# kkahatapitiya/Coarse-Fine-Networks

Measured on AMD Instinct MI355X. Metric: clips/sec (fwd+bwd+SGD) x3d_fine X3D-M T=256x224x224, higher is better.
Workload: dtype f32; 1 GPU; x3d_fine X3D-M train step (fwd+loss+bwd+SGD), 8x3x256x224x224 clips per GPU, random-init weights; clips_per_gpu=8, frames=256, parallelism=dp1, launch=eager

## Files before the change

coarse-fine-networks_amd/cfn_hip/ops.py:

```python
import torch
from torch.autograd import Function
from torch.autograd.function import once_differentiable

import ctypes
import threading

from . import call, call_try, check, query, ACT_NONE, ACT_RELU, ACT_SWISH, ACT_SIGMOID


_scratch_epoch = [0]


class _ZeroArena(object):
    CHUNK = 1 << 20

    def __init__(self):
        self.buf, self.off, self.epoch = {}, {}, _scratch_epoch[0]

    def take(self, numel, dev):
        if self.epoch != _scratch_epoch[0]:
            self.buf, self.off, self.epoch = {}, {}, _scratch_epoch[0]
        numel_al = (numel + 1) & ~1
        key = (dev.type, dev.index)
        if key not in self.buf or self.off[key] + numel_al > self.buf[key].numel():
            self.buf[key] = torch.zeros(max(self.CHUNK, numel_al), dtype=torch.float64, device=dev)
            self.off[key] = 0
        o = self.off[key]
        self.off[key] = o + numel_al
        return self.buf[key][o:o + numel]


class _GradCast(object):

    def __init__(self):
        self._reset()
        self.last_total = 0

    def _reset(self):
        self.cur, self.live, self.scheduled, self.seen, self.task = {}, [], False, set(), None

    def begin(self):
        tid = torch._C._current_graph_task_id()
        if tid != self.task:
            if self.live:
                self.flush()
            self._reset()
            self.task = tid

    def first_use(self, w):
        if id(w) in self.seen:
            return False
        self.seen.add(id(w))
        return True

    def take(self, numel, shape, dev):
        al = (numel + 3) & ~3
        key = (dev.type, dev.index)
        ch = self.cur.get(key)
        if ch is None or ch['off'] + al > ch['f64'].numel():
            size = max(int(self.last_total * 1.05) + 1024, al, 1 << 16)
            ch = {'f64': torch.zeros(size, dtype=torch.float64, device=dev),
                  'f32': torch.empty(size, dtype=torch.float32, device=dev), 'off': 0, 'done': 0}
            self.cur[key] = ch
            self.live.append(ch)
        o = ch['off']
        ch['off'] = o + al
        if not self.scheduled:
            torch.autograd.Variable._execution_engine.queue_callback(self._end_of_backward)
            self.scheduled = True
        return ch['f64'][o:o + numel], ch['f32'][o:o + numel].view(shape)

    def flush(self):
        for ch in self.live:
            if ch['off'] > ch['done']:
                ch['f32'][ch['done']:ch['off']].copy_(ch['f64'][ch['done']:ch['off']])
                ch['done'] = ch['off']

    def _end_of_backward(self):
        self.flush()
        self.last_total = max(sum(ch['off'] for ch in self.live), 1)
        self._reset()


class _PerThread(threading.local):

    def __init__(self):
        self.arena = _ZeroArena()
        self.gradcast = _GradCast()


_tls = _PerThread()
LAZY_GRAD_CAST = True


def _f64(n, c, dev):
    return _tls.arena.take(n * c, dev).view(n, c)


def _f64pair(n, c, dev):
    t = _tls.arena.take(2 * n * c, dev).view(2, n, c)
    return t, t[0], t[1]


def reset_scratch():
    _scratch_epoch[0] += 1


def flush_grad_casts():
    _tls.gradcast.flush()


def allow_lazy_grad_cast(params, ok=True):
    for p in params:
        p._cfn_lazy_grad_ok = bool(ok)


def _lazy_ok(w):
    if not LAZY_GRAD_CAST or w is None or not w.is_leaf or w.grad is not None or torch.is_grad_enabled():
        return False
    if not getattr(w, '_cfn_lazy_grad_ok', False):
        return False
    if w._backward_hooks:
        return False
    hooks = getattr(w, '_post_accumulate_grad_hooks', None)
    if hooks:
        from .dist import _BucketHook
        if not all(isinstance(h, _BucketHook) for h in hooks.values()):
            return False
    return True


def _lazy_ok_probe(w):
    with torch.no_grad():
        return _lazy_ok(w)


def _grad_owner(w):
    if w is not None and not w.is_leaf and w._is_view():
        base = w._base
        if base is not None and base.is_leaf and base.numel() == w.numel() and w.is_contiguous() and base.is_contiguous():
            return base
    return w


def _gw_buffers(w, rows, cols, dev):
    gc = _tls.gradcast
    owner = _grad_owner(w)
    if _lazy_ok(owner):
        gc.begin()
        if gc.first_use(owner):
            g64, g32 = gc.take(rows * cols, tuple(w.shape), dev)
            return g64.view(rows, cols), (lambda: g32)
        gc.flush()
    g64 = _f64(rows, cols, dev)
    return g64, (lambda: g64.float().view(tuple(w.shape)))


def _opt(t):
    return None if t is None else t.contiguous()


def _coef(t, rows=None, cols=None):
    if t is None:
        return None
    if rows is not None and t.numel() != rows * cols:
        raise RuntimeError('per-sample coefficients of %d x %d channels expected, got a tensor of shape %s' % (rows, cols, tuple(t.shape)))
    return t.to(torch.float64).contiguous()


class ShortcutToken(object):

    def __init__(self):
        self.acc, self.acc_stride, self.main_done = None, 1, False


class TailLink(object):

    def __init__(self):
        self.y_scale = self.res_scale = None
        self.done = False


def _bf(t):
    return t is not None and t.dtype in (torch.bfloat16, torch.float16)


def subsample_hw(x, s):
    N, C, T, H, W = x.shape
    out = torch.empty(N, C, T, (H - 1) // s + 1, (W - 1) // s + 1, dtype=x.dtype, device=x.device)
    call('cfn_subsample_hw' + _sfx(x), x, out, N * C * T, H, W, s)
    return out


class _PwConv(Function):

    @staticmethod
    def forward(ctx, x, A, B, w, act, stride, want_stats, token, role, tail=None, tail_role=None):
        x = check(x).contiguous()
        N, Cin, T, H, W = x.shape
        Cout = w.shape[0]
        Ho, Wo = (H - 1) // stride + 1, (W - 1) // stride + 1
        y = torch.empty(N, Cout, T, Ho, Wo, dtype=x.dtype, device=x.device)
        s = q = None
        if want_stats:
            s, q = _f64(N, Cout, x.device), _f64(N, Cout, x.device)
        w2 = w.reshape(Cout, Cin).contiguous()
        A, B = _coef(A, N, Cin), _coef(B, N, Cin)
        xs = None
        if _bf(x):
            xs = subsample_hw(x, stride) if stride > 1 else x
            call('cfn_pwconv_fwd' + _sfx(x), xs, A, B, act, w2, y, s, q, N, Cin, Cout, T * Ho * Wo)
        else:
            call('cfn_pwconv_fwd', x, A, B, act, w2, y, s, q, N, Cin, Cout, T, H, W, stride)
        ctx.save_for_backward(x, A, B, w2, y, xs if stride > 1 else None)
        ctx.meta = (act, stride, tuple(w.shape))
        ctx.wparam = w
        ctx.token, ctx.role = token, role
        ctx.tail, ctx.tail_role = tail, tail_role
        if not want_stats:
            return y, None, None
        return y, s, q

    @staticmethod
    @once_differentiable
    def backward(ctx, gy, gs, gq):
        x, A, B, w2, y, xs = ctx.saved_tensors
        act, stride, wshape = ctx.meta
        token, role = ctx.token, ctx.role
        N, Cin, T, H, W = x.shape
        Cout = w2.shape[0]
        gy = torch.zeros_like(y) if gy is None else gy.contiguous()
        gs, gq = _opt(gs), _opt(gq)
        gsc = None
        if ctx.tail is not None and ctx.tail.done:
            gsc = ctx.tail.y_scale if ctx.tail_role == 'y' else ctx.tail.res_scale
        if _bf(x):
            return _PwConv._backward_bf16(ctx, gy, gs, gq, gsc)
        gx = gA = gB = gw = None
        g64 = fin = None
        fused = False
        if ctx.needs_input_grad[0] or (A is not None and ctx.needs_input_grad[1]):
            if token is not None and role == 'short' and stride > 1 and not token.main_done:
                Ho, Wo = y.shape[3], y.shape[4]
                da = torch.empty(N, Cin, T, Ho, Wo, dtype=torch.float32, device=x.device)
                if ctx.needs_input_grad[3]:
                    g64, fin = _gw_buffers(ctx.wparam, Cout, Cin, x.device)
                    fused = call_try('cfn_pwconv_short_bwd', gy, y, gs, gq, gsc, w2, x, A, B, act, da, g64, N, Cin, Cout, T, H, W,
                                     stride)
                if not fused:
                    call('cfn_pwconv_bwd_data_acc', gy, y, gs, gq, w2, None, None, None, ACT_NONE, da, None, None, N, Cin, Cout, T,
                         Ho, Wo, 1, None, 1, gsc)
                token.acc, token.acc_stride = da, stride
            else:
                gx = torch.zeros_like(x) if stride != 1 else torch.empty_like(x)
                ab = a64 = b64 = None
                if A is not None:
                    ab, a64, b64 = _f64pair(N, Cin, x.device)
                acc, acc_stride = None, 1
                if token is not None and role == 'main':
                    if token.acc is not None:
                        acc, acc_stride, token.acc = token.acc, token.acc_stride, None
                    else:
                        token.main_done = True
                if stride == 1 and ctx.needs_input_grad[3]:
                    g64, fin = _gw_buffers(ctx.wparam, Cout, Cin, x.device)
                    fused = call_try('cfn_pwconv_bwd_fused', gy, y, gs, gq, w2, x, A, B, act, gx, a64, b64, g64, N, Cin, Cout,
                                     T, H, W, acc, acc_stride, gsc)
                if not fused:
                    call('cfn_pwconv_bwd_data_acc', gy, y, gs, gq, w2, x, A, B, act, gx, a64, b64, N, Cin, Cout, T, H, W, stride,
                         acc, acc_stride, gsc)
                if A is not None:
                    gA, gB = ab[0], ab[1]
        if ctx.needs_input_grad[3]:
            if g64 is None:
                g64, fin = _gw_buffers(ctx.wparam, Cout, Cin, x.device)
            if not fused:
                call('cfn_pwconv_bwd_weight', gy, y, gs, gq, x, A, B, act, g64, N, Cin, Cout, T, H, W, stride, gsc)
            gw = fin()
        return gx, gA, gB, gw, None, None, None, None, None, None, None

    @staticmethod
    def _backward_bf16(ctx, gy, gs, gq, gsc):
        x, A, B, w2, y, xs = ctx.saved_tensors
        act, stride, wshape = ctx.meta
        token, role = ctx.token, ctx.role
        N, Cin, T, H, W = x.shape
        Cout = w2.shape[0]
        Ho, Wo = y.shape[3], y.shape[4]
        xin = xs if stride > 1 else x
        gx = gA = gB = gw = None
        if ctx.needs_input_grad[0] or (A is not None and ctx.needs_input_grad[1]):
            if token is not None and role == 'short' and stride > 1 and not token.main_done:
                da = torch.empty(N, Cin, T, Ho, Wo, dtype=x.dtype, device=x.device)
                call('cfn_pwconv_bwd_data' + _sfx(gy), gy, y, gs, gq, w2, None, None, None, ACT_NONE, da, None, None, N, Cin, Cout, T,
                     Ho, Wo, None, 1, gsc)
                token.acc, token.acc_stride = da, stride
            else:
                ab = a64 = b64 = None
                if A is not None:
                    ab, a64, b64 = _f64pair(N, Cin, x.device)
                acc, acc_stride = None, 1
                if token is not None and role == 'main':
                    if token.acc is not None:
                        acc, acc_stride, token.acc = token.acc, token.acc_stride, None
                    else:
                        token.main_done = True
                gxc = torch.empty_like(xin)
                call('cfn_pwconv_bwd_data' + _sfx(gy), gy, y, gs, gq, w2, xin, A, B, act, gxc, a64, b64, N, Cin, Cout, T, Ho, Wo,
                     acc, acc_stride, gsc)
                if stride > 1:
                    gx = torch.zeros_like(x)
                    gx[:, :, :, ::stride, ::stride] = gxc
                else:
                    gx = gxc
                if A is not None:
                    gA, gB = ab[0], ab[1]
        if ctx.needs_input_grad[3]:
            g64, fin = _gw_buffers(ctx.wparam, Cout, Cin, x.device)
            call('cfn_pwconv_bwd_weight' + _sfx(gy), gy, y, gs, gq, xin, A, B, act, g64, N, Cin, Cout, T * Ho * Wo, gsc)
            gw = fin()
        return gx, gA, gB, gw, None, None, None, None, None, None, None


def pwconv(x, w, A=None, B=None, act=ACT_NONE, stride=1, stats=True, token=None, role=None, tail=None, tail_role=None):
    N, Cin, T, H, W = x.shape
    Ho, Wo = (H - 1) // stride + 1, (W - 1) // stride + 1
    es = x.element_size()
    lim = (1 << 31) if es == 4 else (1 << 30)
    span = max(Cin * H * W, w.shape[0] * H * W, w.shape[0] * Ho * Wo, Cin * Ho * Wo) * es
    needs_grad = torch.is_grad_enabled() and any(t is not None and t.requires_grad for t in (x, w, A, B))
    if span * T < lim or needs_grad or T == 1:
        return _PwConv.apply(x, A, B, w, act, stride, stats, token, role, tail, tail_role)
    step = max((lim - 1) // span, 1)
    odd_plane = es == 2 and (Ho * Wo) % 2 == 1
    if odd_plane:
        if 2 * span >= lim:
            raise RuntimeError('pwconv: two frames of %d x %d x %d bf16 elements exceed the 1 GiB buffer range the frame-range '
                               'chunking has to respect (odd plane: frames travel in pairs)' % (max(Cin, w.shape[0]), H, W))
        step = max(step & ~1, 2)
    y = torch.empty(N, w.shape[0], T, Ho, Wo, dtype=x.dtype, device=x.device)
    s = q = None
    t0 = 0
    while t0 < T:
        t1 = min(t0 + step, T)
        if odd_plane and (t1 - t0) % 2 and t1 - t0 > 1:
            t1 -= 1
        pad = odd_plane and (t1 - t0) % 2 == 1
        xc = x[:, :, t0:t1].contiguous()
        if pad:
            xc = torch.cat([xc, torch.zeros_like(xc)], 2)
        yc, sc, qc = _PwConv.apply(xc, A, B, w, act, stride, False if pad else stats, None, None)
        if pad:
            yc = yc[:, :, :1]
            if stats:
                sc, qc = yc.double().sum((2, 3, 4)), (yc.double() ** 2).sum((2, 3, 4))
        y[:, :, t0:t1] = yc
        if stats:
            s, q = (sc, qc) if s is None else (s + sc, q + qc)
        t0 = t1
    return y, s, q


def _sfx(t):
    return '_bf16' if t.dtype == torch.bfloat16 else ('_f16' if t.dtype == torch.float16 else '')


class _DwConv3d(Function):

    @staticmethod
    def forward(ctx, x, A, B, w, act, stride, want_stats):
        x = check(x).contiguous()
        N, C, T, H, W = x.shape
        Ho, Wo = (H + 2 - 3) // stride + 1, (W + 2 - 3) // stride + 1
        y = torch.empty(N, C, T, Ho, Wo, dtype=x.dtype, device=x.device)
        s = q = None
        if want_stats:
            s, q = _f64(N, C, x.device), _f64(N, C, x.device)
        w2 = w.reshape(C, 27).contiguous()
        A, B = _coef(A, N, C), _coef(B, N, C)
        call('cfn_dwconv3d_fwd' + _sfx(x), x, A, B, act, w2, y, s, q, N, C, T, H, W, stride)
        ctx.save_for_backward(x, A, B, w2, y)
        ctx.meta = (act, stride, tuple(w.shape))
        ctx.wparam = w
        if not want_stats:
            return y, None, None
        return y, s, q

    @staticmethod
    @once_differentiable
    def backward(ctx, gy, gs, gq):
        x, A, B, w2, y = ctx.saved_tensors
        act, stride, wshape = ctx.meta
        N, C, T, H, W = x.shape
        gy = torch.zeros_like(y) if gy is None else gy.contiguous()
        gs, gq = _opt(gs), _opt(gq)
        gx = gA = gB = gw = None
        want_x = ctx.needs_input_grad[0] or (A is not None and ctx.needs_input_grad[1])
        want_w = ctx.needs_input_grad[3]
        ab = a64 = b64 = g64 = fin = None
        if want_x:
            gx = torch.empty_like(x)
            if A is not None:
                ab, a64, b64 = _f64pair(N, C, x.device)
        if want_w:
            g64, fin = _gw_buffers(ctx.wparam, C, 27, x.device)
        sfx = _sfx(x)
        fused = want_x and want_w and stride == 1 and call_try('cfn_dwconv3d_bwd_fused' + sfx, gy, y, gs, gq, w2, x, A, B, act,
                                                             gx, a64, b64, g64, N, C, T, H, W)
        if not fused and want_x and want_w and stride == 2:
            fused = call_try('cfn_dwconv3d_bwd_fused_s2' + sfx, gy, y, gs, gq, w2, x, A, B, act, gx, a64, b64, g64, N, C, T, H, W)
        if not fused:
            if want_x:
                call('cfn_dwconv3d_bwd_data' + sfx, gy, y, gs, gq, w2, x, A, B, act, gx, a64, b64, N, C, T, H, W, stride)
            if want_w:
                call('cfn_dwconv3d_bwd_weight' + sfx, gy, y, gs, gq, x, A, B, act, g64, N, C, T, H, W, stride)
        if want_x and A is not None:
            gA, gB = ab[0], ab[1]
        if want_w:
            gw = fin()
        return gx, gA, gB, gw, None, None, None


def dwconv3d(x, w, A=None, B=None, act=ACT_NONE, stride=1, stats=True):
    return _DwConv3d.apply(x, A, B, w, act, stride, stats)


class _DwConvT5(Function):

    @staticmethod
    def forward(ctx, x, w, want_stats, out_dtype=None):
        x = check(x, torch.float32).contiguous()
        N, C, T, H, W = x.shape
        y = torch.empty_like(x, dtype=out_dtype or x.dtype)
        s = q = None
        if want_stats:
            s, q = _f64(N, C, x.device), _f64(N, C, x.device)
        w2 = w.reshape(C, 5).contiguous()
        call('cfn_dwconv_t5_fwd' + _sfx(y), x, w2, y, s, q, N, C, T, H * W)
        ctx.save_for_backward(x, w2, y)
        ctx.wshape = tuple(w.shape)
        ctx.wparam = w
        if not want_stats:
            return y, None, None
        return y, s, q

    @staticmethod
    @once_differentiable
    def backward(ctx, gy, gs, gq):
        x, w2, y = ctx.saved_tensors
        N, C, T, H, W = x.shape
        gy = torch.zeros_like(y) if gy is None else gy.contiguous()
        gs, gq = _opt(gs), _opt(gq)
        gx = gw = None
        want_x, want_w = ctx.needs_input_grad[0], ctx.needs_input_grad[1]
        if want_x:
            gx = torch.empty_like(x)
        if want_w:
            g64, fin = _gw_buffers(ctx.wparam, C, 5, x.device)
        fused = want_x and want_w and call_try('cfn_dwconv_t5_bwd_fused' + _sfx(y), gy, y, gs, gq, w2, x, gx, g64, N, C, T, H * W)
        if not fused:
            if want_x:
                call('cfn_dwconv_t5_bwd_data' + _sfx(y), gy, y, gs, gq, w2, gx, N, C, T, H * W)
            if want_w:
                call('cfn_dwconv_t5_bwd_weight' + _sfx(y), gy, y, gs, gq, x, g64, N, C, T, H * W)
        if want_w:
            gw = fin()
        return gx, gw, None, None


def dwconv_t5(x, w, stats=True, out_dtype=None):
    return _DwConvT5.apply(x, w, stats, out_dtype)


class _StemConv(Function):

    @staticmethod
    def forward(ctx, x, w):
        x = check(x).contiguous()
        N, Ci, T, H, W = x.shape
        Co = w.shape[0]
        Ho, Wo = (H + 2 - 3) // 2 + 1, (W + 2 - 3) // 2 + 1
        y = torch.empty(N, Co, T, Ho, Wo, dtype=torch.float32, device=x.device)
        w2 = w.reshape(Co, Ci * 9).contiguous()
        call('cfn_stem_conv_fwd', x, w2, y, N, Ci, Co, T, H, W)
        ctx.save_for_backward(x)
        ctx.wshape = tuple(w.shape)
        ctx.wparam = w
        return y

    @staticmethod
    @once_differentiable
    def backward(ctx, gy):
        (x,) = ctx.saved_tensors
        N, Ci, T, H, W = x.shape
        Co = ctx.wshape[0]
        gw = None
        if ctx.needs_input_grad[1]:
            g64, fin = _gw_buffers(ctx.wparam, Co, Ci * 9, x.device)
            call('cfn_stem_conv_bwd_weight', gy.contiguous(), x, g64, N, Ci, Co, T, H, W)
            gw = fin()
        return None, gw


def stem_conv(x, w):
    return _StemConv.apply(x, w)


from .u8clips import clip_lut


def _u8_args(frames, lengths, lut):
    if frames.dtype != torch.uint8 or frames.dim() != 5 or frames.shape[4] != 3:
        raise RuntimeError('uint8 frames of shape (N, T, H, W, 3) expected, got %s %s' % (frames.dtype, tuple(frames.shape)))
    if lut.dtype != torch.float32 or lut.numel() != 3 * 256:
        raise RuntimeError('a (3, 256) fp32 table expected (ops.clip_lut), got %s %s' % (lut.dtype, tuple(lut.shape)))
    if lengths is not None:
        if lengths.numel() != frames.shape[0]:
            raise RuntimeError('one length per clip expected: %d clips, lengths %s' % (frames.shape[0], tuple(lengths.shape)))
        lengths = lengths.to(torch.int32).contiguous()
    return frames.contiguous(), lengths, lut.contiguous()


def clip_u8_to_f32(frames, lut, lengths=None):
    frames, lengths, lut = _u8_args(frames, lengths, lut)
    N, T, H, W, _ = frames.shape
    x = torch.empty(N, 3, T, H, W, dtype=torch.float32, device=frames.device)
    call('cfn_clip_u8_to_f32', frames, lut, lengths, x, N, T, H, W)
    return x


class _StemConvU8(Function):

    @staticmethod
    def forward(ctx, frames, lengths, lut, w):
        frames, lengths, lut = _u8_args(frames, lengths, lut)
        N, T, H, W, Ci = frames.shape
        Co = w.shape[0]
        Ho, Wo = (H + 2 - 3) // 2 + 1, (W + 2 - 3) // 2 + 1
        y = torch.empty(N, Co, T, Ho, Wo, dtype=torch.float32, device=frames.device)
        w2 = w.reshape(Co, Ci * 9).contiguous()
        if not call_try('cfn_stem_conv_u8_fwd', frames, lut, lengths, w2, y, N, Ci, Co, T, H, W):
            call('cfn_stem_conv_fwd', clip_u8_to_f32(frames, lut, lengths), w2, y, N, Ci, Co, T, H, W)
        ctx.save_for_backward(frames, lengths, lut)
        ctx.wshape = tuple(w.shape)
        ctx.wparam = w
        return y

    @staticmethod
    @once_differentiable
    def backward(ctx, gy):
        frames, lengths, lut = ctx.saved_tensors
        N, T, H, W, Ci = frames.shape
        Co = ctx.wshape[0]
        gw = None
        if ctx.needs_input_grad[3]:
            g64, fin = _gw_buffers(ctx.wparam, Co, Ci * 9, frames.device)
            gy = gy.contiguous()
            if not call_try('cfn_stem_conv_u8_bwd_weight', gy, frames, lut, lengths, g64, N, Ci, Co, T, H, W):
                call('cfn_stem_conv_bwd_weight', gy, clip_u8_to_f32(frames, lut, lengths), g64, N, Ci, Co, T, H, W)
            gw = fin()
        return None, None, None, gw


def stem_conv_u8(frames, lengths, lut, w):
    return _StemConvU8.apply(frames, lengths, lut, w)


from . import u8aug

_AUG_TABLES = {}
_AUG_TABLES_MAX = 256


def aug_tables(box, size, device):
    cs = tuple(int(v) for v in box.detach().reshape(-1, 4)[:, 2].cpu().tolist())
    device = torch.device(device)
    key = (cs, int(size), device.type, device.index)
    hit = _AUG_TABLES.get(key)
    if hit is None:
        if any(c <= 0 or c > 4 * int(size) for c in cs):
            raise RuntimeError('crop_resize_flip_u8: crop extents %s into %d: 1 <= c <= 4 * size expected (the kernel takes tables of up '
                               'to %d taps; there is no CPU fallback)' % (sorted(set(cs)), size, u8aug.MAX_TAPS))
        bounds, coef = u8aug.batch_tables(cs, size)
        hit = (bounds.to(device), coef.to(device))
        if len(_AUG_TABLES) >= _AUG_TABLES_MAX:
            _AUG_TABLES.clear()
        _AUG_TABLES[key] = hit
    return hit


def crop_resize_flip_u8(frames, lengths, box, size, out=None, tables=None):
    if frames.dtype != torch.uint8 or frames.dim() != 5 or frames.shape[4] != 3:
        raise RuntimeError('uint8 frames of shape (N, T, Hs, Ws, 3) expected, got %s %s' % (frames.dtype, tuple(frames.shape)))
    N, T, Hs, Ws, _ = frames.shape
    S = int(size)
    if box.numel() != 4 * N:
        raise RuntimeError('one box (x1, y1, c, flip) per clip expected: %d clips, box %s' % (N, tuple(box.shape)))
    if lengths is not None:
        if lengths.numel() != N:
            raise RuntimeError('one length per clip expected: %d clips, lengths %s' % (N, tuple(lengths.shape)))
        lengths = lengths.to(torch.int32).contiguous()
    bounds, coef = tables if tables is not None else aug_tables(box, S, frames.device)
    if tuple(bounds.shape) != (N, S, 2) or coef.dim() != 3 or tuple(coef.shape[:2]) != (N, S):
        raise RuntimeError('tables of %d clips into %d expected, got bounds %s coef %s' % (N, S, tuple(bounds.shape), tuple(coef.shape)))
    box = box.reshape(N, 4).to(device=frames.device, dtype=torch.int32).contiguous()
    if out is None:
        out = torch.empty(N, T, S, S, 3, dtype=torch.uint8, device=frames.device)
    elif out.dtype != torch.uint8 or tuple(out.shape) != (N, T, S, S, 3) or not out.is_contiguous():
        raise RuntimeError('out: a contiguous uint8 tensor of shape %s expected, got %s %s' % ((N, T, S, S, 3), out.dtype, tuple(out.shape)))
    if not call_try('cfn_crop_resize_flip_u8', frames.contiguous(), lengths, box, bounds.contiguous(), coef.contiguous(), out, N, T, Hs, Ws,
                    S, int(coef.shape[2])):
        raise RuntimeError('crop_resize_flip_u8: %d taps into size %d is beyond what the kernel was built for (c <= 4 * size, size <= 312 '
                           'at 9 taps); there is no CPU fallback' % (int(coef.shape[2]), S))
    return out


AP_SORT_TILE = 8192
AP_FLAG_NONBINARY, AP_FLAG_OVERFLOW = 1, 2


def _ap_stores(scores, targets, count, what):
    for name, x in (('scores', scores), ('targets', targets), ('count', count)):
        if not torch.is_tensor(x) or not x.is_cuda:
            raise RuntimeError('%s: %s must be a device tensor; there is no CPU path' % (what, name))
    if scores.dtype != torch.float32 or scores.dim() != 2 or targets.dtype != torch.uint8 or tuple(targets.shape) != tuple(scores.shape):
        raise RuntimeError('%s: class-major stores expected, scores (K, cap) fp32 and targets (K, cap) uint8; got %s %s, %s %s'
                           % (what, scores.dtype, tuple(scores.shape), targets.dtype, tuple(targets.shape)))
    if count.dtype != torch.int32 or count.numel() != 1:
        raise RuntimeError('%s: count must be one int32 on the device, got %s %s' % (what, count.dtype, tuple(count.shape)))
    if scores.shape[0] < 1 or scores.shape[1] < 1:
        raise RuntimeError('%s: empty stores %s' % (what, tuple(scores.shape)))
    return int(scores.shape[0]), int(scores.shape[1])


def ap_append(probs, labels, valid, scores, targets, count, flags):
    K, cap = _ap_stores(scores, targets, count, 'ap_append')
    for name, x in (('probs', probs), ('labels', labels), ('flags', flags)):
        if not torch.is_tensor(x) or not x.is_cuda:
            raise RuntimeError('ap_append: %s must be a device tensor; there is no CPU path' % name)
    if probs.dim() != 3 or probs.shape[1] != K or tuple(labels.shape) != tuple(probs.shape):
        raise RuntimeError('ap_append: probs and labels (B, %d, TL) expected, got %s and %s' % (K, tuple(probs.shape), tuple(labels.shape)))
    if flags.dtype != torch.int32 or flags.numel() != 1:
        raise RuntimeError('ap_append: flags must be one int32 on the device')
    B, _, TL = probs.shape
    if valid is not None:
        if valid.numel() != B:
            raise RuntimeError('ap_append: one valid length per video expected: %d videos, valid %s' % (B, tuple(valid.shape)))
        valid = valid.to(torch.int32).contiguous()
    call('cfn_ap_append', probs.float().contiguous(), labels.float().contiguous(), valid, scores, targets, count, flags, B, K, TL, cap)


def ap_sort(scores, targets, count, out=None):
    K, cap = _ap_stores(scores, targets, count, 'ap_sort')
    if out is None:
        out = (torch.empty_like(scores), torch.empty_like(targets), torch.empty(K, cap, dtype=torch.int32, device=scores.device),
               torch.empty_like(targets))
    ss, st, tk, tt = out
    for x, ref, dt in ((ss, scores, torch.float32), (st, targets, torch.uint8), (tk, scores, torch.int32), (tt, targets, torch.uint8)):
        if tuple(x.shape) != tuple(ref.shape) or x.dtype != dt or x.device != ref.device:
            raise RuntimeError('ap_sort: out buffers of shape %s (fp32, uint8, int32, uint8) on %s expected' % (tuple(ref.shape), ref.device))
    call('cfn_ap_sort', scores, targets, count, ss, st, tk, tt, K, cap)
    return ss, st


def ap_reduce(sorted_targets, count):
    if not sorted_targets.is_cuda or not count.is_cuda:
        raise RuntimeError('ap_reduce: device tensors only; there is no CPU path')
    if sorted_targets.dtype != torch.uint8 or sorted_targets.dim() != 2 or count.dtype != torch.int32 or count.numel() != 1:
        raise RuntimeError('ap_reduce: sorted targets (K, cap) uint8 and one int32 count expected')
    K, cap = sorted_targets.shape
    ap = torch.empty(K, dtype=torch.float32, device=sorted_targets.device)
    call('cfn_ap_reduce', sorted_targets, count, ap, K, cap)
    return ap


def average_precision(scores, targets, count, out=None):
    _, st = ap_sort(scores, targets, count, out=out)
    return ap_reduce(st, count)


class _BnFold(Function):

    @staticmethod
    def forward(ctx, s, q, gamma, beta, w1, b1, w2, b2, bufs, cfg):
        training, N, C, S, count, eps, momentum, pool_count = cfg
        run_mean, run_var, nbt = bufs
        dev = run_mean.device
        Wd = w1.shape[0] if w1 is not None else 0
        Se = S if training else 1
        A = torch.empty(N, C, dtype=torch.float64, device=dev)
        B = torch.empty_like(A)
        mean = torch.empty(Se, C, dtype=torch.float64, device=dev)
        rstd = torch.empty_like(mean)
        A0 = B0 = gate = hbuf = pooled = None
        w1c = w2c = None
        if Wd:
            A0, B0, gate, pooled = (torch.empty(N, C, dtype=torch.float32, device=dev) for _ in range(4))
            hbuf = torch.empty(N, Wd, dtype=torch.float32, device=dev)
            w1c, w2c = w1.reshape(Wd, C).contiguous(), w2.reshape(C, Wd).contiguous()
        s, q = _opt(s), _opt(q)
        call('cfn_bn_fold_fwd', s, q, gamma, beta, run_mean, run_var, nbt if training else None, int(training), N, C, S,
             float(count), float(eps), float(momentum), w1c, b1, w2c, b2, Wd, float(pool_count), A, B, mean, rstd,
             A0, B0, gate, hbuf, pooled)
        ctx.save_for_backward(s, gamma, mean, rstd, A0, B0, gate, hbuf, pooled, w1c, w2c)
        ctx.cfg = (training, N, C, S, Wd, count, pool_count, None if w1 is None else tuple(w1.shape),
                   None if w2 is None else tuple(w2.shape))
        return A, B

    @staticmethod
    @once_differentiable
    def backward(ctx, gA, gB):
        s, gamma, mean, rstd, A0, B0, gate, hbuf, pooled, w1c, w2c = ctx.saved_tensors
        training, N, C, S, Wd, count, pool_count, w1s, w2s = ctx.cfg
        dev = mean.device
        gA = torch.zeros(N, C, dtype=torch.float64, device=dev) if gA is None else gA.contiguous()
        gB = torch.zeros(N, C, dtype=torch.float64, device=dev) if gB is None else gB.contiguous()
        gs = gq = None
        if training:
            gs = torch.empty(N, C, dtype=torch.float64, device=dev)
            gq = torch.empty_like(gs)
        elif Wd:
            gs = torch.empty(N, C, dtype=torch.float64, device=dev)
        gg = gbt = None
        if gamma is not None:
            gg, gbt = torch.empty(C, device=dev), torch.empty(C, device=dev)
        gw1 = gb1 = gw2 = gb2 = tA = tB = None
        if Wd:
            gw1, gb1 = torch.empty(Wd, C, device=dev), torch.empty(Wd, device=dev)
            gw2, gb2 = torch.empty(C, Wd, device=dev), torch.empty(C, device=dev)
            tA, tB = (torch.empty(N, C, dtype=torch.float64, device=dev) for _ in range(2))
        call('cfn_bn_fold_bwd', gA, gB, s, gamma, mean, rstd, A0, B0, gate, hbuf, pooled, w1c, w2c, int(training), N, C, S,
             Wd, float(count), float(pool_count), gs, gq, gg, gbt, gw1, gb1, gw2, gb2, tA, tB)
        if Wd:
            gw1, gw2 = gw1.view(w1s), gw2.view(w2s)
        return gs, gq, gg, gbt, gw1, gb1, gw2, gb2, None, None


def bn_fold(s, q, gamma, beta, bufs, training, N, C, S, count, eps, momentum, se=None, pool_count=1.0):
    w1, b1, w2, b2 = se if se is not None else (None, None, None, None)
    return _BnFold.apply(s, q, gamma, beta, w1, b1, w2, b2, bufs, (training, N, C, S, count, eps, momentum, pool_count))


class _BnAddRelu(Function):

    @staticmethod
    def forward(ctx, y, A, B, res, Ar, Br, split, link):
        y, res = check(y).contiguous(), check(res).contiguous()
        N, C = y.shape[:2]
        vol = y[0, 0].numel()
        if tuple(res.shape) != tuple(y.shape):
            raise RuntimeError('bn_add_relu: residual %s does not match y %s' % (tuple(res.shape), tuple(y.shape)))
        out = torch.empty_like(y)
        A, B, Ar, Br = _coef(A, N, C), _coef(B, N, C), _coef(Ar, N, C), _coef(Br, N, C)
        mask = None
        sfx = _sfx(y)
        if link is not None:
            words = query('cfn_bn_add_relu_mask_words' + sfx, N * C, vol)
            if words > 0:
                mask = torch.empty(words, dtype=torch.int32, device=y.device)
        call('cfn_bn_add_relu_fwd' + sfx, y, A, B, res, Ar, Br, out, mask, N * C, vol)
        ctx.link, ctx.has_mask = link, mask is not None
        ctx.save_for_backward(y, A, res, Ar, mask if mask is not None else out)
        if not split:
            return out
        alias = torch.empty(0, dtype=out.dtype, device=out.device).set_(out.untyped_storage(), out.storage_offset(),
                                                                         out.shape, out.stride())
        return out, alias

    @staticmethod
    @once_differentiable
    def backward(ctx, gout, gout2=None):
        y, A, res, Ar, out = ctx.saved_tensors
        N, C = y.shape[:2]
        vol = y[0, 0].numel()
        if gout is None:
            gout, gout2 = gout2, None
        if gout is None:
            gout = torch.zeros_like(y)
        gout2 = None if gout2 is None else gout2.contiguous()
        t3 = _tls.arena.take(3 * N * C, y.device).view(3, N, C)
        gA, gB = t3[0], t3[1]
        gAr = t3[2] if Ar is not None else None
        gBr = gB if Ar is not None else None
        link = ctx.link
        if link is not None:
            g = torch.empty_like(y)
            mask = out if ctx.has_mask else None
            call('cfn_bn_add_relu_bwd_g' + _sfx(y), gout.contiguous(), gout2, None if ctx.has_mask else out, mask, y,
                 res if Ar is not None else None, g, gA, gB, gAr, N * C, vol)
            link.y_scale, link.res_scale, link.done = A.detach(), (None if Ar is None else Ar.detach()), True
            g2 = torch.empty(0, dtype=g.dtype, device=g.device).set_(g.untyped_storage(), g.storage_offset(), g.shape, g.stride())
            return g, gA, gB, g2, gAr, gBr, None, None
        if _bf(y):
            g = torch.empty_like(y)
            call('cfn_bn_add_relu_bwd_g' + _sfx(y), gout.contiguous(), gout2, out, None, y, res if Ar is not None else None, g, gA, gB,
                 gAr, N * C, vol)
            shp = (N, C) + (1,) * (y.dim() - 2)
            gres = g if Ar is None else (g.float() * Ar.float().view(shp)).to(y.dtype)
            return (g.float() * A.float().view(shp)).to(y.dtype), gA, gB, gres, gAr, gBr, None, None
        gy, gres = torch.empty_like(y), torch.empty_like(res)
        call('cfn_bn_add_relu_bwd', gout.contiguous(), gout2, out, y, A, res, Ar, gy, gres, gA, gB, gAr, N * C, vol)
        return gy, gA, gB, gres, gAr, gBr, None, None


def bn_add_relu(y, A, B, res, Ar=None, Br=None, split=False, link=None):
    return _BnAddRelu.apply(y, A, B, res, Ar, Br, split, link)


class _AffineAct(Function):
    @staticmethod
    def forward(ctx, x, A, B, act):
        x = check(x).contiguous()
        N, C = x.shape[:2]
        out = torch.empty_like(x)
        A, B = _coef(A, N, C), _coef(B, N, C)
        call('cfn_affine_act_fwd', x, A, B, act, out, N * C, x[0, 0].numel())
        ctx.save_for_backward(x, A, B)
        ctx.act = act
        return out

    @staticmethod
    @once_differentiable
    def backward(ctx, gout):
        x, A, B = ctx.saved_tensors
        N, C = x.shape[:2]
        gx = torch.empty_like(x)
        a64, b64 = _f64(N, C, x.device), _f64(N, C, x.device)
        call('cfn_affine_act_bwd', gout.contiguous(), x, A, B, ctx.act, gx, a64, b64, N * C, x[0, 0].numel())
        return gx, a64, b64, None


def affine_act(x, A, B, act=ACT_NONE):
    return _AffineAct.apply(x, A, B, act)


class _ChannelStats(Function):

    @staticmethod
    def forward(ctx, x):
        x = check(x).contiguous()
        N, C = x.shape[:2]
        s, q = _f64(N, C, x.device), _f64(N, C, x.device)
        call('cfn_channel_stats', x, s, q, N * C, x[0, 0].numel())
        ctx.save_for_backward(x)
        return s, q

    @staticmethod
    @once_differentiable
    def backward(ctx, gs, gq):
        (x,) = ctx.saved_tensors
        N, C = x.shape[:2]
        gx = torch.zeros_like(x)
        shp = (N, C) + (1,) * (x.dim() - 2)
        if gs is not None:
            gx = gx + gs.float().view(shp)
        if gq is not None:
            gx = gx + 2.0 * gq.float().view(shp) * x
        return gx


def channel_stats(x):
    return _ChannelStats.apply(x)


class _PoolHW(Function):

    @staticmethod
    def forward(ctx, x, A, B, act, OH, OW):
        x = check(x).contiguous()
        N, C, T, H, W = x.shape
        out = torch.empty(N, C, T, OH, OW, dtype=torch.float32, device=x.device)
        A, B = _coef(A, N, C), _coef(B, N, C)
        call('cfn_pool_hw_fwd' + _sfx(x), x, A, B, act, out, N * C, T, H, W, OH, OW)
        ctx.save_for_backward(x, A, B)
        ctx.meta = (act, OH, OW)
        return out

    @staticmethod
    @once_differentiable
    def backward(ctx, gout):
        x, A, B = ctx.saved_tensors
        act, OH, OW = ctx.meta
        N, C, T, H, W = x.shape
        gx = torch.empty_like(x)
        a64 = b64 = None
        if A is not None:
            a64, b64 = _f64(N, C, x.device), _f64(N, C, x.device)
        call('cfn_pool_hw_bwd' + _sfx(x), gout.contiguous(), x, A, B, act, gx, a64, b64, N * C, T, H, W, OH, OW)
        if A is None:
            return gx, None, None, None, None, None
        return gx, a64, b64, None, None, None


def pool_hw(x, OH, OW, A=None, B=None, act=ACT_NONE):
    return _PoolHW.apply(x, A, B, act, OH, OW)


class _Film(Function):

    @staticmethod
    def forward(ctx, x, m, c, f):
        x, m, c = check(x).contiguous(), check(m).contiguous(), check(c).contiguous()
        N, C, T, H, W = x.shape
        want = (N, C, T, H // f if f > 0 else -1, W // f if f > 0 else -1)
        if f <= 0 or H % f or W % f or tuple(m.shape) != want or tuple(c.shape) != want:
            raise RuntimeError('film: coefficients %s / %s do not tile x %s with %d x %d blocks (expected %s)'
                               % (tuple(m.shape), tuple(c.shape), tuple(x.shape), f, f, want))
        out = torch.empty_like(x)
        call('cfn_film_fwd', x, m, c, out, N * C, T, H, W, f)
        ctx.save_for_backward(x, m)
        ctx.f = f
        return out

    @staticmethod
    @once_differentiable
    def backward(ctx, g):
        x, m = ctx.saved_tensors
        N, C, T, H, W = x.shape
        gx, gm, gc = torch.empty_like(x), torch.empty_like(m), torch.empty_like(m)
        call('cfn_film_bwd', g.contiguous(), x, m, gx, gm, gc, N * C, T, H, W, ctx.f)
        return gx, gm, gc, None


def film(x, m, c, f):
    return _Film.apply(x, m, c, f)


class _TimeSample(Function):

    @staticmethod
    def forward(ctx, x, cdf):
        x, cdf = check(x).contiguous(), check(cdf).contiguous()
        B, C, Tin = x.shape[:3]
        K = cdf.shape[1]
        P = x[0, 0, 0].numel()
        out = torch.empty((B, C, K) + tuple(x.shape[3:]), dtype=torch.float32, device=x.device)
        call('cfn_time_sample_fwd', x, cdf, out, B, C, Tin, K, P)
        ctx.save_for_backward(x, cdf)
        return out

    @staticmethod
    @once_differentiable
    def backward(ctx, g):
        x, cdf = ctx.saved_tensors
        B, C, Tin = x.shape[:3]
        K = cdf.shape[1]
        P = x[0, 0, 0].numel()
        gx = torch.empty_like(x) if ctx.needs_input_grad[0] else None
        g64 = torch.zeros(B, K, dtype=torch.float64, device=x.device) if ctx.needs_input_grad[1] else None
        call('cfn_time_sample_bwd', g.contiguous(), x, cdf, gx, g64, B, C, Tin, K, P)
        return gx, (g64.float() if g64 is not None else None)


def time_sample(x, cdf):
    return _TimeSample.apply(x, cdf)


class _TimePool(Function):

    @staticmethod
    def forward(ctx, x, mode, R):
        x = check(x, torch.float32).contiguous()
        B, C, T = x.shape[:3]
        P = x[0, 0, 0].numel()
        out = torch.empty((B, C, T // R) + tuple(x.shape[3:]), dtype=torch.float32, device=x.device)
        call('cfn_time_pool_fwd', x, out, mode, B * C, T, R, P)
        ctx.save_for_backward(x)
        ctx.meta = (mode, R)
        return out

    @staticmethod
    @once_differentiable
    def backward(ctx, g):
        (x,) = ctx.saved_tensors
        mode, R = ctx.meta
        B, C, T = x.shape[:3]
        gx = torch.empty_like(x)
        call('cfn_time_pool_bwd', g.contiguous(), x, gx, mode, B * C, T, R, x[0, 0, 0].numel())
        return gx, None, None


def time_pool(x, mode, R=4):
    return _TimePool.apply(x, {'avg': 0, 'max': 1}[mode], R)


def grid_time_index(cdf, Tin):
    cdf = check(cdf).contiguous()
    i0 = torch.empty(cdf.shape, dtype=torch.int32, device=cdf.device)
    w1 = torch.empty(cdf.shape, dtype=torch.float32, device=cdf.device)
    call('cfn_grid_time_index', cdf, cdf.numel(), Tin, i0, w1)
    return i0, w1


class _Interp1d(Function):
    @staticmethod
    def forward(ctx, x, y, xnew):
        x, y, xnew = check(x).contiguous(), check(y).contiguous(), check(xnew).contiguous()
        B = max(x.shape[0], y.shape[0], xnew.shape[0])
        N, Pq = x.shape[1], xnew.shape[1]
        rows = (int(x.shape[0] > 1), int(y.shape[0] > 1), int(xnew.shape[0] > 1))
        ynew = torch.empty(B, Pq, dtype=torch.float32, device=x.device)
        ind = torch.empty(B, Pq, dtype=torch.int64, device=x.device)
        call('cfn_interp1d_fwd', x, y, xnew, ynew, ind, B, N, Pq, *rows)
        ctx.save_for_backward(x, y, xnew, ind)
        ctx.rows = rows
        ctx.mark_non_differentiable(ind)
        return ynew, ind

    @staticmethod
    @once_differentiable
    def backward(ctx, g, _gind):
        x, y, xnew, ind = ctx.saved_tensors
        B, Pq = ind.shape
        N = x.shape[1]
        gx = torch.zeros_like(x) if ctx.needs_input_grad[0] else None
        gy = torch.zeros_like(y) if ctx.needs_input_grad[1] else None
        gq = torch.zeros_like(xnew) if ctx.needs_input_grad[2] else None
        call('cfn_interp1d_bwd', g.contiguous(), x, y, xnew, ind, gx, gy, gq, B, N, Pq, *ctx.rows)
        return gx, gy, gq


def interp1d(x, y, xnew):
    return _Interp1d.apply(x, y, xnew)


class _TimeResize(Function):

    @staticmethod
    def forward(ctx, x, L, align_corners):
        x = check(x).contiguous()
        BC = x.shape[0] * x.shape[1]
        Kin = x.shape[2]
        P = x[0, 0, 0].numel()
        out = torch.empty(tuple(x.shape[:2]) + (L,) + tuple(x.shape[3:]), dtype=torch.float32, device=x.device)
        call('cfn_time_resize_fwd', x, out, BC, Kin, L, P, int(bool(align_corners)))
        ctx.meta = (tuple(x.shape), L, int(bool(align_corners)))
        return out

    @staticmethod
    @once_differentiable
    def backward(ctx, g):
        shape, L, ac = ctx.meta
        gx = torch.empty(shape, dtype=torch.float32, device=g.device)
        P = 1
        for d in shape[3:]:
            P *= d
        call('cfn_time_resize_bwd', g.contiguous(), gx, shape[0] * shape[1], shape[2], L, P, ac)
        return gx, None, None


def time_resize(x, L, align_corners=True):
    return _TimeResize.apply(x, L, align_corners)


def _detloss_args(logits, labels, masks, crops):
    for name, v in (('logits', logits), ('labels', labels), ('masks', masks)):
        if not v.is_cuda or v.dtype != torch.float32:
            raise RuntimeError('detection_loss: %s must be a device fp32 tensor, got %s on %s (there is no CPU path)' % (name, v.dtype, v.device))
        if v.device != logits.device:
            raise RuntimeError('detection_loss: %s lives on %s, the logits on %s' % (name, v.device, logits.device))
    crops = int(crops)
    if logits.dim() != 3 or labels.dim() != 3 or masks.dim() != 2 or crops < 1:
        raise RuntimeError('detection_loss: logits (B*crops, C, T), labels (B, C, TL), masks (B, TL), crops >= 1')
    B, C, TL = labels.shape
    if logits.shape[0] != B * crops or logits.shape[1] != C or tuple(masks.shape) != (B, TL) or 0 in logits.shape or 0 in labels.shape:
        raise RuntimeError('detection_loss: logits %s, labels %s, masks %s do not belong together at %d crop(s)'
                           % (tuple(logits.shape), tuple(labels.shape), tuple(masks.shape), crops))
    return logits.contiguous(), labels.contiguous(), masks.contiguous(), B, C, logits.shape[2], TL


def detection_loss_fwd(logits, labels, masks, align_corners=True, crops=1, norm=None, world=1.0, want_probs=True):
    logits, labels, masks, B, C, T, TL = _detloss_args(logits, labels, masks, crops)
    dev = logits.device
    if norm is not None:
        if not norm.is_cuda or norm.device != dev or norm.numel() != 1:
            raise RuntimeError('detection_loss: norm must be a one-element tensor on the device of the logits')
        norm = norm.detach().to(torch.float32).reshape(1)
    cls = torch.empty((), dtype=torch.float32, device=dev)
    loc = torch.empty((), dtype=torch.float32, device=dev)
    probs = torch.empty(B, C, TL, dtype=torch.float32, device=dev) if want_probs else None
    jstar = torch.empty(B * C, dtype=torch.int32, device=dev)
    ymax = torch.empty(B * C, dtype=torch.float32, device=dev)
    rows = torch.empty(2 * B * C, dtype=torch.float64, device=dev)
    norm_used = torch.empty(1, dtype=torch.float64, device=dev)
    call('cfn_detloss_fwd', logits, labels, masks, norm, float(world), probs, cls, loc, jstar, ymax, rows, norm_used, B, C, T, TL, int(crops),
         int(bool(align_corners)))
    return cls, loc, probs, jstar, ymax, norm_used


def detection_loss_bwd(g_cls, g_loc, logits, labels, masks, jstar, ymax, norm_used, align_corners=True, crops=1, world=1.0):
    logits, labels, masks, B, C, T, TL = _detloss_args(logits, labels, masks, crops)
    if jstar.numel() != B * C or ymax.numel() != B * C or norm_used.numel() != 1:
        raise RuntimeError('detection_loss_bwd: jstar / ymax / norm_used are not the ones the forward returned for these shapes')
    g_cls, g_loc = (g.detach().to(torch.float32).reshape(1) for g in (g_cls, g_loc))
    gx = torch.empty_like(logits)
    call('cfn_detloss_bwd', g_cls, g_loc, logits, labels, masks, jstar.contiguous(), ymax.contiguous(), norm_used, float(world), gx, B, C, T, TL,
         int(crops), int(bool(align_corners)))
    return gx


class _DetectionLoss(Function):

    @staticmethod
    def forward(ctx, logits, labels, masks, align_corners, crops, norm, world, want_probs):
        cls, loc, probs, jstar, ymax, norm_used = detection_loss_fwd(logits, labels, masks, align_corners, crops, norm, world, want_probs)
        ctx.save_for_backward(logits, labels, masks, jstar, ymax, norm_used)
        ctx.meta = (bool(align_corners), int(crops), float(world))
        if probs is not None:
            ctx.mark_non_differentiable(probs)
# ... 305 lines not shown
```

coarse-fine-networks_amd/csrc/pw_common.h:

```cpp
#pragma once
#include "cfn_common.h"

typedef float __attribute__((ext_vector_type(16))) f16v;
typedef float __attribute__((ext_vector_type(4))) f4v;

enum { PW_FWD = 0, PW_DGRAD = 1 };
#define PW_KC 32
#define PW_RED_PITCH 33

struct PwArgs {
    const float* src;
    const float* src2;
    const double* pa;
    const double* pb;
    const double* gs;
    const double* gq;
    const double* gsc;
    const float* w;
    float* dst;
    const float* ex;
    const double* ea;
    const double* eb;
    const float* acc; int acc_s, acc_Ho, acc_Wo;
    double* s1;
    double* s2;
    int N, M, K, Q, Pin, Hi, Wi, Ho, Wo, stride, act;
    int Cin;
    int mtiles, nstrips, tpb, kres, Kpad;
    int stem, Cimg, kT, kH, kW, sT, sH, sW, pT, pH, pW, Ti, To;
};

#define PW_UNIT 8
#define PW_KRES_MAX 512

__device__ __forceinline__ float pw_bload(__amdgpu_buffer_rsrc_t r, int voff, int soff) {
    return __builtin_bit_cast(float, __builtin_amdgcn_raw_buffer_load_b32(r, voff, soff, 0));
}


int pwd_try_launch(PwArgs& a, int mode, bool stats, hipStream_t st);

int pws_try_launch(PwArgs& a, int mode, bool stats, hipStream_t st);
int pwk_try_launch(PwArgs& a, int mode, bool stats, hipStream_t st);
int pwt_try_launch(PwArgs& a, int mode, bool stats, hipStream_t st);
int pws_terms_now();
int pws_wgrad_try_launch(const float* gy, const float* y, const double* gs, const double* gq, const double* gsc, const float* x,
                         const double* pa, const double* pb, int act, double* gw, int N, int M, int K, int Q, hipStream_t st);

int pwss_wgrad_try_bf16(const uint16_t* gy, const uint16_t* y, const double* gs, const double* gq, const double* gsc, const uint16_t* x,
                        const double* pa, const double* pb, int act, double* gw, int N, int M, int K, int Q, hipStream_t st);

int pwd_wgrad_try_launch(const float* gy, const float* y, const double* gs, const double* gq, const double* gsc, const float* x,
                         const double* pa, const double* pb, int act, double* gw, int N, int M, int K, int Q, hipStream_t st);
int pwd_wgrad_try_strided(const float* gy, const float* y, const double* gs, const double* gq, const double* gsc, const float* x,
                          const double* pa, const double* pb, int act, double* gw, int N, int M, int K, int T, int Hi, int Wi,
                          int stride, hipStream_t st);
int pwd_wgrad_try_dense(const float* gy, const float* y, const double* gs, const double* gq, const float* x, const double* pa,
                        const double* pb, int act, double* gw, int N, int M, int Cimg, int T, int Hi, int Wi, const int* g,
                        hipStream_t st);

int stem_fwd_try_launch(const float* x, const float* w, float* y, int N, int Cimg, int Cout, int T, int Hi, int Wi, hipStream_t st);
int stem_wgrad_try_launch(const float* gy, const float* x, double* gw, int N, int Cimg, int Cout, int T, int Hi, int Wi, hipStream_t st, bool probe);

int sal_fwd_try_launch(const float* x, const double* A, const double* B, int act, const float* w, float* y, double* sum,
                       double* sumsq, int N, int Cin, int Cout, int T, int Hi, int Wi, const int* g, hipStream_t st);
int pwfs_try_launch(const float* gy, const float* y, const double* gsum, const double* gsumsq, const float* w, const float* x, const double* A,
                    const double* B, int act, float* gx, double* gA, double* gB, double* gw, int N, int Cin, int Cout, int T, int Hi, int Wi,
                    const float* acc, int acc_stride, const double* gscale, hipStream_t st);
int salb_fwd_try_launch(const float* x, const double* A, const double* B, int act, const float* w, float* y, double* sum,
                        double* sumsq, int N, int Cin, int Cout, int T, int Hi, int Wi, const int* g, hipStream_t st);
int sal_wgrad_try_launch(const float* gy, const float* y, const double* gs, const double* gq, const float* x, const double* A,
                         const double* B, int act, double* gw, int N, int Cin, int Cout, int T, int Hi, int Wi, const int* g,
                         hipStream_t st);
```

coarse-fine-networks_amd/csrc/pwfused.hip:

```cpp
#include "cfn_common.h"
#include <stdlib.h>

#include "pw_common.h"

typedef float __attribute__((ext_vector_type(4))) pf4;

#define PF_PT 64
#define PF_PITCH 65

struct PfArgs {
    const float* gy; const float* y; const double* gs; const double* gq; const double* gsc;
    const float* w;
    const float* x; const double* pa; const double* pb;
    float* gx; double* gA; double* gB; double* gw;
    const float* acc; int acc_s, acc_Ho, acc_Wo, Hi, Wi, T;
    int N, M, K, Q, nstrips, stages;
};

template <int MTW, int NTW, int ACT>
__global__ __launch_bounds__(256, ACT < 0 ? 3 : 2) void pw_bwd_fused_kernel(const PfArgs a) {
    extern __shared__ __attribute__((aligned(16))) float smem[];
    constexpr bool EPI = ACT >= 0;
    constexpr int ACTV = EPI ? ACT : CFN_ACT_NONE;
    constexpr int BM = 32 * MTW, BN = 32 * NTW;
    constexpr int NG = BM / 16, NX = BN / 16;
    constexpr int NT16 = BN / 16, KS = BM / 4;
    const int tid = threadIdx.x, wave = tid >> 6, lane = tid & 63, half = lane >> 5, col = lane & 31;
    const int m16 = lane & 15, kq = lane >> 4;
    unsigned L = cfn_xcd_remap(blockIdx.x, gridDim.x);
    const int strip = L % a.nstrips;
    const int n = L / a.nstrips;
    const int M = a.M, K = a.K, Q = a.Q;

    constexpr int IMG = (BM + BN) * PF_PITCH;
    float* img0 = smem;
    float* sCg = smem + 2 * IMG;
    float* sCz = sCg + 2 * BM;
    float* sCx = sCz + BM;
    float* sSt = sCx + 2 * BN;
    for (int m = tid; m < BM; m += 256) {
        const bool ok = m < M;
        sCg[2 * m] = (ok && a.gs) ? (float)a.gs[(long)n * M + m] : 0.0f;
        sCg[2 * m + 1] = (ok && a.gq && a.y) ? 2.0f * (float)a.gq[(long)n * M + m] : 0.0f;
        sCz[m] = (ok && a.gsc) ? (float)a.gsc[(long)n * M + m] : 1.0f;
    }
    for (int k = tid; k < BN; k += 256) {
        const bool ok = EPI && k < K;
        sCx[2 * k] = ok ? (float)a.pa[(long)n * K + k] : 1.0f;
        sCx[2 * k + 1] = ok ? (float)a.pb[(long)n * K + k] : 0.0f;
    }
    float wq[NT16][KS];
#pragma unroll
    for (int t = 0; t < NT16; ++t)
#pragma unroll
        for (int s = 0; s < KS; ++s) {
            const int ci = t * 16 + m16, co = 4 * s + kq;
            wq[t][s] = (ci < K && co < M) ? a.w[(long)co * K + ci] : 0.0f;
        }
    float ca[NTW], cb[NTW];
#pragma unroll
    for (int j = 0; j < NTW; ++j) {
        const int k = j * 32 + col;
        const bool ok = EPI && k < K;
        ca[j] = ok ? (float)a.pa[(long)n * K + k] : 1.0f;
        cb[j] = ok ? (float)a.pb[(long)n * K + k] : 0.0f;
    }
    f16v acc[MTW][NTW];
#pragma unroll
    for (int i = 0; i < MTW; ++i)
#pragma unroll
        for (int j = 0; j < NTW; ++j)
#pragma unroll
            for (int r = 0; r < 16; ++r) acc[i][j][r] = 0.0f;
    float sa[NT16][4], sb[NT16][4];
#pragma unroll
    for (int t = 0; t < NT16; ++t)
#pragma unroll
        for (int r = 0; r < 4; ++r) { sa[t][r] = 0.0f; sb[t][r] = 0.0f; }
    __syncthreads();

    const int lrow = tid >> 4, c4 = (tid & 15) * 4;
    constexpr int OOB = 0x7ffffff0;
    __amdgpu_buffer_rsrc_t rg = cfn_rsrc(const_cast<float*>(a.gy + (long)n * M * Q), (unsigned)((long)M * Q * 4));
    __amdgpu_buffer_rsrc_t ry = cfn_rsrc(const_cast<float*>((a.y ? a.y : a.gy) + (long)n * M * Q), a.y ? (unsigned)((long)M * Q * 4) : 0u);
    __amdgpu_buffer_rsrc_t rx = cfn_rsrc(const_cast<float*>(a.x + (long)n * K * Q), (unsigned)((long)K * Q * 4));
    __amdgpu_buffer_rsrc_t rd = cfn_rsrc(a.gx + (long)n * K * Q, (unsigned)((long)K * Q * 4));
    pf4 pg[NG], py[NG], px[NX];
    int vog[NG], vox[NX];
#pragma unroll
    for (int it = 0; it < NG; ++it) vog[it] = (it * 16 + lrow) < M ? ((it * 16 + lrow) * Q + c4) * 4 : OOB;
#pragma unroll
    for (int it = 0; it < NX; ++it) vox[it] = (it * 16 + lrow) < K ? ((it * 16 + lrow) * Q + c4) * 4 : OOB;
    auto prefetch = [&](int q0) {
        const bool inq = q0 + c4 < Q;
#pragma unroll
        for (int it = 0; it < NG; ++it) {
            const int vo = inq ? vog[it] : OOB;
            pg[it] = __builtin_bit_cast(pf4, __builtin_amdgcn_raw_buffer_load_b128(rg, vo, q0 * 4, 0));
            py[it] = __builtin_bit_cast(pf4, __builtin_amdgcn_raw_buffer_load_b128(ry, vo, q0 * 4, 0));
        }
#pragma unroll
        for (int it = 0; it < NX; ++it)
            px[it] = __builtin_bit_cast(pf4, __builtin_amdgcn_raw_buffer_load_b128(rx, inq ? vox[it] : OOB, q0 * 4, 0));
    };
    auto stage = [&](int q0, float* sG, float* sX) {
        const bool inq = q0 + c4 < Q;
#pragma unroll
        for (int it = 0; it < NG; ++it) {
            const int row = it * 16 + lrow;
            const float cs = cfn_settle(sCg[2 * row]), cq = cfn_settle(sCg[2 * row + 1]), cz = cfn_settle(sCz[row]);
            const bool ok = inq && (row < M);
            float* d = sG + row * PF_PITCH + c4;
            d[0] = ok ? fmaf(py[it].x, cq, fmaf(pg[it].x, cz, cs)) : 0.0f;
            d[1] = ok ? fmaf(py[it].y, cq, fmaf(pg[it].y, cz, cs)) : 0.0f;
            d[2] = ok ? fmaf(py[it].z, cq, fmaf(pg[it].z, cz, cs)) : 0.0f;
            d[3] = ok ? fmaf(py[it].w, cq, fmaf(pg[it].w, cz, cs)) : 0.0f;
        }
#pragma unroll
        for (int it = 0; it < NX; ++it) {
            const int row = it * 16 + lrow;
            float* d = sX + row * PF_PITCH + c4;
            d[0] = px[it].x; d[1] = px[it].y; d[2] = px[it].z; d[3] = px[it].w;
        }
    };

    const int qbeg = strip * a.stages * PF_PT;
    const int nst = min(a.stages, (Q - qbeg + PF_PT - 1) / PF_PT);
    if (nst > 0) {
        prefetch(qbeg);
        stage(qbeg, img0, img0 + BM * PF_PITCH);
        if (nst > 1) prefetch(qbeg + PF_PT);
    }
    __syncthreads();
    const int pbase = wave * (PF_PT / 4);
    const int hw = a.Hi * a.Wi;
    const int acc_pitch4 = a.T * a.acc_Ho * a.acc_Wo * 4;
    __amdgpu_buffer_rsrc_t racc = cfn_rsrc(const_cast<float*>(a.acc ? a.acc + (long)n * K * (acc_pitch4 / 4) : a.gy), a.acc ? (unsigned)((long)K * acc_pitch4) : 0u);
    for (int st = 0; st < nst; ++st) {
        const int q0 = qbeg + st * PF_PT;
        float* cur = img0 + (st & 1) * IMG;
        float* nxt = img0 + ((st + 1) & 1) * IMG;
        if (st + 1 < nst) {
            stage(q0 + PF_PT, nxt, nxt + BM * PF_PITCH);
            if (st + 2 < nst) prefetch(q0 + 2 * PF_PT);
        }
        const float* sG = cur;
        const float* sX = cur + BM * PF_PITCH;
#pragma unroll
        for (int s = 0; s < PF_PT / 8; ++s) {
            const int p = pbase + 2 * s + half;
            float av[MTW], bv[NTW];
#pragma unroll
            for (int i = 0; i < MTW; ++i) av[i] = sG[(i * 32 + col) * PF_PITCH + p];
#pragma unroll
            for (int j = 0; j < NTW; ++j) {
                const float xr = sX[(j * 32 + col) * PF_PITCH + p];
                bv[j] = EPI ? cfn_act<ACTV>(fmaf(xr, ca[j], cb[j])) : xr;
            }
#pragma unroll
            for (int i = 0; i < MTW; ++i)
#pragma unroll
                for (int j = 0; j < NTW; ++j) acc[i][j] = __builtin_amdgcn_mfma_f32_32x32x2f32(av[i], bv[j], acc[i][j], 0, 0, 0);
        }
        pf4 da[NT16];
#pragma unroll
        for (int t = 0; t < NT16; ++t) da[t] = (pf4){0.f, 0.f, 0.f, 0.f};
#pragma unroll
        for (int s = 0; s < KS; ++s) {
            const float b = sG[(4 * s + kq) * PF_PITCH + pbase + m16];
#pragma unroll
            for (int t = 0; t < NT16; ++t) da[t] = __builtin_amdgcn_mfma_f32_16x16x4f32(wq[t][s], b, da[t], 0, 0, 0);
        }
        const int q = q0 + pbase + m16;
        const bool qv = q < Q;
        int aoff = OOB;
        if (a.acc && qv) {
            const int tq = q / hw, rq = q - tq * hw;
            const int hq = rq / a.Wi, wq_ = rq - hq * a.Wi;
            if (hq % a.acc_s == 0 && wq_ % a.acc_s == 0) aoff = (((tq * a.acc_Ho + hq / a.acc_s) * a.acc_Wo + wq_ / a.acc_s)) * 4;
        }
        float av4[NT16][4];
#pragma unroll
        for (int t = 0; t < NT16; ++t)
#pragma unroll
            for (int r = 0; r < 4; ++r) av4[t][r] = 0.0f;
        if (a.acc) {
            const unsigned arow = (unsigned)aoff + (unsigned)(4 * kq) * (unsigned)acc_pitch4;
#pragma unroll
            for (int t = 0; t < NT16; ++t)
#pragma unroll
                for (int r = 0; r < 4; ++r)
                    av4[t][r] = __builtin_bit_cast(float, __builtin_amdgcn_raw_buffer_load_b32(
                        racc, (int)(aoff == OOB ? (unsigned)OOB : arow + (unsigned)r * (unsigned)acc_pitch4), t * 16 * acc_pitch4, 0));
        }
#pragma unroll
        for (int t = 0; t < NT16; ++t) {
#pragma unroll
            for (int r = 0; r < 4; ++r) {
                const int ci = t * 16 + 4 * kq + r;
                const bool ok = qv && ci < K;
                float v = da[t][r] + av4[t][r];
                if (EPI) {
                    const float xr = sX[ci * PF_PITCH + pbase + m16];
                    const float pa = sCx[2 * ci], pb = sCx[2 * ci + 1];
                    const float dz = ok ? v * cfn_act_grad<ACTV>(fmaf(xr, pa, pb)) : 0.0f;
                    sa[t][r] = fmaf(dz, xr, sa[t][r]);
                    sb[t][r] += dz;
                    v = dz * pa;
                }
                __builtin_amdgcn_raw_buffer_store_b32(__builtin_bit_cast(unsigned, v), rd, ok ? (ci * Q + pbase + m16) * 4 : OOB, q0 * 4, 0);
            }
        }
        __syncthreads();
    }

    if (EPI) {
#pragma unroll
        for (int t = 0; t < NT16; ++t)
#pragma unroll
            for (int r = 0; r < 4; ++r) {
                float u = sa[t][r], v = sb[t][r];
#pragma unroll
                for (int o = 1; o < 16; o <<= 1) { u += __shfl_xor(u, o, 64); v += __shfl_xor(v, o, 64); }
                if (m16 == 0) {
                    const int ci = t * 16 + 4 * kq + r;
                    sSt[(wave * BN + ci) * 2] = u;
                    sSt[(wave * BN + ci) * 2 + 1] = v;
                }
            }
    }
    constexpr int CWP = BN + 1;
    float* cw = smem + wave * (BM * CWP);
#pragma unroll
    for (int i = 0; i < MTW; ++i)
#pragma unroll
        for (int j = 0; j < NTW; ++j)
#pragma unroll
            for (int r = 0; r < 16; ++r) {
                const int ml = i * 32 + (r & 3) + 8 * (r >> 2) + 4 * half;
                cw[ml * CWP + j * 32 + col] = acc[i][j][r];
            }
    __syncthreads();
    for (int e = tid; e < BM * BN; e += 256) {
        const int ml = e / BN, kl = e - ml * BN;
        const int o = ml * CWP + kl;
        const float v = (smem[o] + smem[BM * CWP + o]) + (smem[2 * BM * CWP + o] + smem[3 * BM * CWP + o]);
        if (ml < M && kl < K) cfn_add64(&a.gw[(long)ml * K + kl], (double)v);
    }
    if (EPI && tid < K) {
        const float u = (sSt[2 * tid] + sSt[(BN + tid) * 2]) + (sSt[(2 * BN + tid) * 2] + sSt[(3 * BN + tid) * 2]);
        const float v = (sSt[2 * tid + 1] + sSt[(BN + tid) * 2 + 1]) + (sSt[(2 * BN + tid) * 2 + 1] + sSt[(3 * BN + tid) * 2 + 1]);
        cfn_add64(&a.gA[(long)n * K + tid], (double)u);
        cfn_add64(&a.gB[(long)n * K + tid], (double)v);
    }
}

template <int MTW, int NTW>
static int pf_launch(const PfArgs& a, int act, bool epi, unsigned blocks, hipStream_t st) {
    constexpr int BM = 32 * MTW, BN = 32 * NTW;
    size_t lds = ((size_t)2 * (BM + BN) * PF_PITCH + 3 * BM + 10 * BN) * sizeof(float);
    const size_t lds_cw = (size_t)4 * BM * (BN + 1) * sizeof(float);
    if (lds_cw > lds) lds = lds_cw;
#define CFN_PF_GO(ACTV)                                                                                         \
    do {                                                                                                        \
        auto k = pw_bwd_fused_kernel<MTW, NTW, ACTV>;                                                           \
        if (lds > 48 * 1024) (void)hipFuncSetAttribute((const void*)k, hipFuncAttributeMaxDynamicSharedMemorySize, (int)lds); \
        hipLaunchKernelGGL(k, dim3(blocks), dim3(256), lds, st, a);                                             \
    } while (0)
    if (!epi) CFN_PF_GO(-1);
    else if (act == CFN_ACT_RELU) CFN_PF_GO(CFN_ACT_RELU);
    else if (act == CFN_ACT_SWISH) CFN_PF_GO(CFN_ACT_SWISH);
    else CFN_PF_GO(CFN_ACT_NONE);
#undef CFN_PF_GO
    return cfn_check_launch("pwconv_bwd_fused");
}

extern "C" int cfn_pwconv_bwd_fused(const float* gy, const float* y, const double* gsum, const double* gsumsq, const float* w,
                                    const float* x, const double* A, const double* B, int act, float* gx, double* gA, double* gB,
                                    double* gw, int N, int Cin, int Cout, int T, int Hi, int Wi, const float* acc, int acc_stride,
                                    const double* gscale, void* stream) {
    CFN_REQUIRE(gy && w && x && gx && gw, "cfn_pwconv_bwd_fused: null tensor");
    CFN_REQUIRE((A == nullptr) == (B == nullptr), "cfn_pwconv_bwd_fused: A/B mismatch");
    CFN_REQUIRE(A == nullptr || (gA && gB), "cfn_pwconv_bwd_fused: prologue needs gA, gB");
    CFN_REQUIRE(gsumsq == nullptr || y != nullptr, "cfn_pwconv_bwd_fused: gsumsq needs y");
    CFN_REQUIRE(acc == nullptr || acc_stride >= 1, "cfn_pwconv_bwd_fused: bad acc_stride");
    {
        const int rs = pwfs_try_launch(gy, y, gsum, gsumsq, w, x, A, B, act, gx, gA, gB, gw, N, Cin, Cout, T, Hi, Wi, acc, acc_stride, gscale, (hipStream_t)stream);
        if (rs != -1) return rs;
    }
    const long Ql = (long)T * Hi * Wi;
    if (Cin > 64 || Cout > 64 || (Cin > 32 && Cout > 32) || Ql % 4 != 0 || Ql >= (1L << 30)) return -1;
    if ((long)Cout * Ql * 4 >= 0x7ffffff0L || (long)Cin * Ql * 4 >= 0x7ffffff0L) return -1;
    if (A && act != CFN_ACT_NONE && act != CFN_ACT_RELU && act != CFN_ACT_SWISH) return -1;
    if ((((uintptr_t)gy | (uintptr_t)x | (uintptr_t)(y ? y : gy)) & 15) != 0) return -1;
    PfArgs a = {};
    a.gy = gy; a.y = gsumsq ? y : nullptr; a.gs = gsum; a.gq = gsumsq; a.gsc = gscale; a.w = w; a.x = x; a.pa = A; a.pb = B;
    a.gx = gx; a.gA = gA; a.gB = gB; a.gw = gw;
    a.acc = acc; a.acc_s = acc ? acc_stride : 1; a.Hi = Hi; a.Wi = Wi; a.T = T;
    a.acc_Ho = (Hi - 1) / a.acc_s + 1; a.acc_Wo = (Wi - 1) / a.acc_s + 1;
    a.N = N; a.M = Cout; a.K = Cin; a.Q = (int)Ql;
    const long nst = cfn_cdiv(Ql, PF_PT);
    const bool epi = A != nullptr;
    long want = (epi ? 1024 : 1536) / N;
    if (want < 1) want = 1;
    long stages = cfn_cdiv(nst, want);
    if (stages < 4) stages = 4;
    a.stages = (int)stages;
    a.nstrips = (int)cfn_cdiv(nst, stages);
    const unsigned blocks = (unsigned)((long)N * a.nstrips);
    hipStream_t st = (hipStream_t)stream;
    CfnProfScope prof(CFN_K_PWCONV_BWD, st, 4.0 * N * ((double)Cout * Ql * (a.y ? 2 : 1) + (double)Cin * Ql * 2));
    if (Cout > 32) return pf_launch<2, 1>(a, act, epi, blocks, st);
    if (Cin > 32) return pf_launch<1, 2>(a, act, epi, blocks, st);
    return pf_launch<1, 1>(a, act, epi, blocks, st);
}
```

coarse-fine-networks_amd/csrc/pwfuseds.hip:

```cpp
#include "cfn_common.h"
#include <stdlib.h>
#include <map>
#include <mutex>

#include "pw_common.h"

typedef float __attribute__((ext_vector_type(4))) pf4;
typedef __bf16 pfs_bf8 __attribute__((ext_vector_type(8)));
typedef __bf16 pfs_bf2 __attribute__((ext_vector_type(2)));
typedef float pfs_f2 __attribute__((ext_vector_type(2)));
typedef unsigned pfs_u4 __attribute__((ext_vector_type(4)));

#define PFS_PT 64
#define PFS_PITCH 65

__device__ __forceinline__ float pfs_lo(unsigned u) { return __builtin_bit_cast(float, u << 16); }
__device__ __forceinline__ float pfs_hi(unsigned u) { return __builtin_bit_cast(float, u & 0xffff0000u); }
__device__ __forceinline__ unsigned pfs_pack(float lo, float hi) {
    const pfs_bf2 b = __builtin_convertvector((pfs_f2){lo, hi}, pfs_bf2);
    return __builtin_bit_cast(unsigned, b);
}
__device__ __forceinline__ void pfs_split3(float v0, float v1, unsigned (&p)[3]) {
    p[0] = pfs_pack(v0, v1);
    v0 -= pfs_lo(p[0]); v1 -= pfs_hi(p[0]);
    p[1] = pfs_pack(v0, v1);
    v0 -= pfs_lo(p[1]); v1 -= pfs_hi(p[1]);
    p[2] = pfs_pack(v0, v1);
}
#define PFS_TERMS(F) F(2, 0) F(0, 2) F(1, 1) F(1, 0) F(0, 1) F(0, 0)

struct PfsArgs {
    const float* gy; const float* y; const double* gs; const double* gq; const double* gsc;
    const float* w;
    const float* x; const double* pa; const double* pb;
    float* gx; double* gA; double* gB; double* gw;
    const float* acc; int acc_s, acc_Ho, acc_Wo, Hi, Wi, T;
    int N, M, K, Q, nstrips, stages;
    int dbg;
};

template <int MTW, int NTW, int ACT>
__global__ __launch_bounds__(512, 1) void pw_bwd_fused_split_kernel(const PfsArgs a) {
    extern __shared__ __attribute__((aligned(16))) float smem[];
    constexpr bool EPI = ACT >= 0;
    constexpr int ACTV = EPI ? ACT : CFN_ACT_NONE;
    constexpr int BM = 32 * MTW, BN = 32 * NTW;
    constexpr int NG = BM / 16, NX = BN / 16;
    constexpr int NT16 = BN / 16, KS = BM / 32;
    constexpr bool ROWSPLIT = MTW >= NTW;
    constexpr int MI = ROWSPLIT ? MTW / 2 : MTW, NJ = ROWSPLIT ? NTW : NTW / 2;
    constexpr int BMP = BM + 8;
    const int tid = threadIdx.x, wave = cfn_uni((int)(tid >> 6)), lane = tid & 63, half = lane >> 5, col = lane & 31;
    const int m16 = lane & 15, kq = lane >> 4;
    unsigned L = cfn_xcd_remap(blockIdx.x, gridDim.x);
    const int strip = L % a.nstrips;
    const int n = L / a.nstrips;
    const int M = a.M, K = a.K, Q = a.Q;

    constexpr int IMG = (BM + BN) * PFS_PITCH;
    float* img0 = smem;
    float* sCx = smem + 2 * IMG + 3 * BM;
    float* sSt = sCx + 2 * BN;
    unsigned* sW = reinterpret_cast<unsigned*>(sSt + 8 * BN);
    for (int k = tid; k < BN; k += 512) {
        const bool ok = EPI && k < K;
        sCx[2 * k] = ok ? (float)a.pa[(long)n * K + k] : 1.0f;
        sCx[2 * k + 1] = ok ? (float)a.pb[(long)n * K + k] : 0.0f;
    }
    for (int e = tid; e < BN * (BM / 2); e += 512) {
        const int ci = e / (BM / 2), mp = e - ci * (BM / 2), co = 2 * mp;
        const float w0 = (ci < K && co < M) ? a.w[(long)co * K + ci] : 0.0f;
        const float w1 = (ci < K && co + 1 < M) ? a.w[(long)(co + 1) * K + ci] : 0.0f;
        unsigned p[3];
        pfs_split3(w0, w1, p);
#pragma unroll
        for (int s = 0; s < 3; ++s) sW[(s * BN + ci) * (BMP / 2) + mp] = p[s];
    }
    __syncthreads();

    const int lrow = 4 * ((tid & 255) >> 6) + ((lane >> 3) & 3), c4 = ((lane & 7) + 8 * (lane >> 5)) * 4;
    constexpr int OOB = 0x7ffffff0;
    __amdgpu_buffer_rsrc_t rg = cfn_rsrc(const_cast<float*>(a.gy + (long)n * M * Q), (unsigned)((long)M * Q * 4));
    __amdgpu_buffer_rsrc_t ry = cfn_rsrc(const_cast<float*>((a.y ? a.y : a.gy) + (long)n * M * Q), a.y ? (unsigned)((long)M * Q * 4) : 0u);
    __amdgpu_buffer_rsrc_t rx = cfn_rsrc(const_cast<float*>(a.x + (long)n * K * Q), (unsigned)((long)K * Q * 4));
    __amdgpu_buffer_rsrc_t rd = cfn_rsrc(a.gx + (long)n * K * Q, (unsigned)((long)K * Q * 4));
    pf4 pg[NG], py[NG], px[NX];
    int vog[NG], vox[NX];
    float rcs[NG], rcq[NG], rcz[NG];
#pragma unroll
    for (int it = 0; it < NG; ++it) {
        const int row = it * 16 + lrow;
        const bool ok = row < M;
        rcs[it] = (ok && a.gs) ? (float)a.gs[(long)n * M + row] : 0.0f;
        rcq[it] = (ok && a.gq && a.y) ? 2.0f * (float)a.gq[(long)n * M + row] : 0.0f;
        rcz[it] = (ok && a.gsc) ? (float)a.gsc[(long)n * M + row] : 1.0f;
    }
#pragma unroll
    for (int it = 0; it < NG; ++it) vog[it] = (it * 16 + lrow) < M ? ((it * 16 + lrow) * Q + c4) * 4 : OOB;
#pragma unroll
    for (int it = 0; it < NX; ++it) vox[it] = (it * 16 + lrow) < K ? ((it * 16 + lrow) * Q + c4) * 4 : OOB;
    auto prefetch = [&](int q0) {
        const bool inq = q0 + c4 < Q;
#pragma unroll
        for (int it = 0; it < NG; ++it) {
            const int vo = inq ? vog[it] : OOB;
            pg[it] = __builtin_bit_cast(pf4, __builtin_amdgcn_raw_buffer_load_b128(rg, vo, q0 * 4, 0));
            py[it] = __builtin_bit_cast(pf4, __builtin_amdgcn_raw_buffer_load_b128(ry, vo, q0 * 4, 0));
        }
#pragma unroll
        for (int it = 0; it < NX; ++it)
            px[it] = __builtin_bit_cast(pf4, __builtin_amdgcn_raw_buffer_load_b128(rx, inq ? vox[it] : OOB, q0 * 4, 0));
    };
    auto stage = [&](int q0, float* sG, float* sX) {
        const bool inq = q0 + c4 < Q;
#pragma unroll
        for (int it = 0; it < NG; ++it) {
            const int row = it * 16 + lrow;
            const float cs = rcs[it], cq = rcq[it], cz = rcz[it];
            const bool ok = inq && (row < M);
            float* d = sG + row * PFS_PITCH + c4;
            d[0] = ok ? fmaf(py[it].x, cq, fmaf(pg[it].x, cz, cs)) : 0.0f;
            d[1] = ok ? fmaf(py[it].y, cq, fmaf(pg[it].y, cz, cs)) : 0.0f;
            d[2] = ok ? fmaf(py[it].z, cq, fmaf(pg[it].z, cz, cs)) : 0.0f;
            d[3] = ok ? fmaf(py[it].w, cq, fmaf(pg[it].w, cz, cs)) : 0.0f;
        }
#pragma unroll
        for (int it = 0; it < NX; ++it) {
            const int row = it * 16 + lrow;
            float* d = sX + row * PFS_PITCH + c4;
            d[0] = px[it].x; d[1] = px[it].y; d[2] = px[it].z; d[3] = px[it].w;
        }
    };

    const int qbeg = strip * a.stages * PFS_PT;
    const int nst = min(a.stages, (Q - qbeg + PFS_PT - 1) / PFS_PT);
    if (nst > 0 && wave < 4) {
        prefetch(qbeg);
        stage(qbeg, img0, img0 + BM * PFS_PITCH);
        if (nst > 1) prefetch(qbeg + PFS_PT);
    }
    __syncthreads();
    const int pbase = (wave & 3) * (PFS_PT / 4);
    constexpr int CWP = 33, CWT = 32 * CWP;

    if (wave < 4) {
        const int th = wave & 1, ph = wave >> 1;
        const int i0 = ROWSPLIT ? th * MI : 0, j0 = ROWSPLIT ? 0 : th * NJ;
        float ca[NJ], cb[NJ];
#pragma unroll
        for (int j = 0; j < NJ; ++j) {
            const int k = (j0 + j) * 32 + col;
            const bool ok = EPI && k < K;
            ca[j] = ok ? (float)a.pa[(long)n * K + k] : 1.0f;
            cb[j] = ok ? (float)a.pb[(long)n * K + k] : 0.0f;
        }
        f16v acc[MI][NJ];
#pragma unroll
        for (int i = 0; i < MI; ++i)
#pragma unroll
            for (int j = 0; j < NJ; ++j)
#pragma unroll
                for (int r = 0; r < 16; ++r) acc[i][j][r] = 0.0f;
        for (int st = 0; st < nst; ++st) {
            const int q0 = qbeg + st * PFS_PT;
            float* cur = img0 + (st & 1) * IMG;
            float* nxt = img0 + ((st + 1) & 1) * IMG;
            if (st + 1 < nst) {
                stage(q0 + PFS_PT, nxt, nxt + BM * PFS_PITCH);
                if (st + 2 < nst) prefetch(q0 + 2 * PFS_PT);
            }
            const float* sG = cur;
            const float* sX = cur + BM * PFS_PITCH;
            if (!(a.dbg & 1))
#pragma unroll
            for (int kb = 0; kb < 2; ++kb) {
                const int p0 = 32 * ph + 16 * kb + 8 * half;
                pfs_u4 Bf[NJ][3];
#pragma unroll
                for (int j = 0; j < NJ; ++j) {
                    const float* r = sX + ((j0 + j) * 32 + col) * PFS_PITCH + p0;
#pragma unroll
                    for (int h = 0; h < 4; ++h) {
                        float x0 = r[2 * h], x1 = r[2 * h + 1];
                        if (EPI) { x0 = cfn_act<ACTV>(fmaf(x0, ca[j], cb[j])); x1 = cfn_act<ACTV>(fmaf(x1, ca[j], cb[j])); }
                        unsigned p[3];
                        pfs_split3(x0, x1, p);
#pragma unroll
                        for (int s = 0; s < 3; ++s) Bf[j][s][h] = p[s];
                    }
                }
#pragma unroll
                for (int i = 0; i < MI; ++i) {
                    const float* r = sG + ((i0 + i) * 32 + col) * PFS_PITCH + p0;
                    pfs_u4 Af[3];
#pragma unroll
                    for (int h = 0; h < 4; ++h) {
                        unsigned p[3];
                        pfs_split3(r[2 * h], r[2 * h + 1], p);
#pragma unroll
                        for (int s = 0; s < 3; ++s) Af[s][h] = p[s];
                    }
#define PFS_WG(SA, SB) acc[i][j] = __builtin_amdgcn_mfma_f32_32x32x16_bf16(__builtin_bit_cast(pfs_bf8, Af[SA]), __builtin_bit_cast(pfs_bf8, Bf[j][SB]), acc[i][j], 0, 0, 0);
#pragma unroll
                    for (int j = 0; j < NJ; ++j) { PFS_TERMS(PFS_WG) }
#undef PFS_WG
                }
            }
            __syncthreads();
        }
        __syncthreads();
        __syncthreads();
        float* cw = smem + wave * (MI * NJ * CWT);
#pragma unroll
        for (int i = 0; i < MI; ++i)
#pragma unroll
            for (int j = 0; j < NJ; ++j)
#pragma unroll
                for (int r = 0; r < 16; ++r) cw[(i * NJ + j) * CWT + ((r & 3) + 8 * (r >> 2) + 4 * half) * CWP + col] = acc[i][j][r];
    } else {
        float sa[NT16][4], sb[NT16][4];
#pragma unroll
        for (int t = 0; t < NT16; ++t)
#pragma unroll
            for (int r = 0; r < 4; ++r) { sa[t][r] = 0.0f; sb[t][r] = 0.0f; }
        const int hw = a.Hi * a.Wi;
        const int acc_pitch4 = a.T * a.acc_Ho * a.acc_Wo * 4;
        __amdgpu_buffer_rsrc_t racc = cfn_rsrc(const_cast<float*>(a.acc ? a.acc + (long)n * K * (acc_pitch4 / 4) : a.gy), a.acc ? (unsigned)((long)K * acc_pitch4) : 0u);
        for (int st = 0; st < nst; ++st) {
            const int q0 = qbeg + st * PFS_PT;
            float* cur = img0 + (st & 1) * IMG;
            const float* sG = cur;
            const float* sX = cur + BM * PFS_PITCH;
            pf4 da[NT16];
#pragma unroll
            for (int t = 0; t < NT16; ++t) da[t] = (pf4){0.f, 0.f, 0.f, 0.f};
            if (!(a.dbg & 2))
#pragma unroll
            for (int s = 0; s < KS; ++s) {
                const float* r = sG + (32 * s + 8 * kq) * PFS_PITCH + pbase + m16;
                pfs_u4 Gf[3];
#pragma unroll
                for (int h = 0; h < 4; ++h) {
                    unsigned p[3];
                    pfs_split3(r[(2 * h) * PFS_PITCH], r[(2 * h + 1) * PFS_PITCH], p);
#pragma unroll
                    for (int u = 0; u < 3; ++u) Gf[u][h] = p[u];
                }
#pragma unroll
                for (int t = 0; t < NT16; ++t) {
                    const unsigned* wr = sW + ((t * 16 + m16) * BMP + 32 * s + 8 * kq) / 2;
                    pfs_u4 Wf[3];
#pragma unroll
                    for (int u = 0; u < 3; ++u) Wf[u] = *reinterpret_cast<const pfs_u4*>(wr + u * BN * (BMP / 2));
#define PFS_DG(SA, SB) da[t] = __builtin_amdgcn_mfma_f32_16x16x32_bf16(__builtin_bit_cast(pfs_bf8, Wf[SA]), __builtin_bit_cast(pfs_bf8, Gf[SB]), da[t], 0, 0, 0);
                    PFS_TERMS(PFS_DG)
#undef PFS_DG
                    if (NT16 > 4 && (t & 1)) __builtin_amdgcn_sched_barrier(0);
                }
            }
            const int q = q0 + pbase + m16;
            const bool qv = q < Q;
            const int gvo = (qv && !(a.dbg & 8)) ? (4 * kq * Q + pbase + m16) * 4 : OOB;
            int aoff = OOB;
            if (a.acc && qv) {
                const int tq = q / hw, rq = q - tq * hw;
                const int hq = rq / a.Wi, wq_ = rq - hq * a.Wi;
                if (hq % a.acc_s == 0 && wq_ % a.acc_s == 0) aoff = (((tq * a.acc_Ho + hq / a.acc_s) * a.acc_Wo + wq_ / a.acc_s)) * 4;
            }
            const unsigned arow = (unsigned)aoff + (unsigned)(4 * kq) * (unsigned)acc_pitch4;
            constexpr bool AV_UPFRONT = NT16 <= 4;
            float av4[AV_UPFRONT ? NT16 : 1][4];
            if (AV_UPFRONT) {
#pragma unroll
                for (int t = 0; t < NT16; ++t)
#pragma unroll
                    for (int r = 0; r < 4; ++r) av4[AV_UPFRONT ? t : 0][r] = 0.0f;
                if (a.acc) {
#pragma unroll
                    for (int t = 0; t < NT16; ++t)
#pragma unroll
                        for (int r = 0; r < 4; ++r)
                            av4[AV_UPFRONT ? t : 0][r] = __builtin_bit_cast(float, __builtin_amdgcn_raw_buffer_load_b32(
                                racc, (int)(aoff == OOB ? (unsigned)OOB : arow + (unsigned)r * (unsigned)acc_pitch4), t * 16 * acc_pitch4, 0));
                }
            }
#pragma unroll
            for (int t = 0; t < NT16; ++t) {
#pragma unroll
                for (int r = 0; r < 4; ++r) {
                    const int ci = t * 16 + 4 * kq + r;
                    float v = da[t][r];
                    if (AV_UPFRONT) v += av4[AV_UPFRONT ? t : 0][r];
                    else if (a.acc)
                        v += __builtin_bit_cast(float, __builtin_amdgcn_raw_buffer_load_b32(
                            racc, (int)(aoff == OOB ? (unsigned)OOB : arow + (unsigned)r * (unsigned)acc_pitch4), t * 16 * acc_pitch4, 0));
                    if (EPI && !(a.dbg & 4)) {
                        const float xr = sX[ci * PFS_PITCH + pbase + m16];
                        const float2 pab = cfn_settle(*reinterpret_cast<const float2*>(sCx + 2 * ci));
                        const float pa = pab.x, pb = pab.y;
                        const float dz = v * cfn_act_grad<ACTV>(fmaf(xr, pa, pb));
                        sa[t][r] = fmaf(dz, xr, sa[t][r]);
                        sb[t][r] += dz;
                        v = dz * pa;
                    }
                    __builtin_amdgcn_raw_buffer_store_b32(__builtin_bit_cast(unsigned, v), rd, gvo, (q0 + (t * 16 + r) * Q) * 4, 0);
                }
                if (NT16 > 4) __builtin_amdgcn_sched_barrier(0);
            }
            __syncthreads();
        }
        if (EPI) {
#pragma unroll
            for (int t = 0; t < NT16; ++t)
#pragma unroll
                for (int r = 0; r < 4; ++r) {
                    float u = sa[t][r], v = sb[t][r];
#pragma unroll
                    for (int o = 1; o < 16; o <<= 1) { u += __shfl_xor(u, o, 64); v += __shfl_xor(v, o, 64); }
                    if (m16 == 0) {
                        const int ci = t * 16 + 4 * kq + r;
                        sSt[((wave & 3) * BN + ci) * 2] = u;
                        sSt[((wave & 3) * BN + ci) * 2 + 1] = v;
                    }
                }
        }
        __syncthreads();
        const int t2 = tid - 256;
        if (EPI && t2 < K) {
            const float u = (sSt[2 * t2] + sSt[(BN + t2) * 2]) + (sSt[(2 * BN + t2) * 2] + sSt[(3 * BN + t2) * 2]);
            const float v = (sSt[2 * t2 + 1] + sSt[(BN + t2) * 2 + 1]) + (sSt[(2 * BN + t2) * 2 + 1] + sSt[(3 * BN + t2) * 2 + 1]);
            cfn_add64(&a.gA[(long)n * K + t2], (double)u);
            cfn_add64(&a.gB[(long)n * K + t2], (double)v);
        }
        __syncthreads();
    }
    __syncthreads();
    constexpr int WT = MI * NJ;
    for (int e = tid; e < 2 * WT * 1024; e += 512) {
        const int th = e / (WT * 1024), tile = (e >> 10) % WT, ml = (e >> 5) & 31, kl = e & 31, o = tile * CWT + ml * CWP + kl;
        const float v = smem[th * (WT * CWT) + o] + smem[(2 + th) * (WT * CWT) + o];
        const int i = tile / NJ, j = tile - i * NJ;
        const int gm = ((ROWSPLIT ? th * MI : 0) + i) * 32 + ml, gk = ((ROWSPLIT ? 0 : th * NJ) + j) * 32 + kl;
        if (gm < M && gk < K) cfn_add64(&a.gw[(long)gm * K + gk], (double)v);
    }
}

template <int MTW, int NTW>
static int pfs_launch(const PfsArgs& a, int act, bool epi, unsigned blocks, hipStream_t st) {
    constexpr int BM = 32 * MTW, BN = 32 * NTW, BMP = BM + 8;
    size_t lds = ((size_t)2 * (BM + BN) * PFS_PITCH + 3 * BM + 10 * BN) * sizeof(float) + (size_t)3 * BN * BMP * 2;
    const size_t lds_cw = (size_t)4 * (MTW * NTW / 2) * 32 * 33 * sizeof(float);
    if (lds_cw > lds) lds = lds_cw;
#define CFN_PFS_GO(ACTV)                                                                                        \
    do {                                                                                                        \
        auto k = pw_bwd_fused_split_kernel<MTW, NTW, ACTV>;                                                     \
        (void)hipFuncSetAttribute((const void*)k, hipFuncAttributeMaxDynamicSharedMemorySize, (int)lds);        \
        hipLaunchKernelGGL(k, dim3(blocks), dim3(512), lds, st, a);                                             \
    } while (0)
    if (!epi) CFN_PFS_GO(-1);
    else if (act == CFN_ACT_RELU) CFN_PFS_GO(CFN_ACT_RELU);
    else if (act == CFN_ACT_SWISH) CFN_PFS_GO(CFN_ACT_SWISH);
    else CFN_PFS_GO(CFN_ACT_NONE);
#undef CFN_PFS_GO
    return cfn_check_launch("pwconv_bwd_fused (split bf16)");
}

#define PF3_PT 32
#define PF3_PITCH 33
#define PF3_TP 36

struct Pf3Args {
    const float* gy; const float* y; const double* gs; const double* gq; const double* gsc;
    const float* x; const unsigned* wsplit;
    float* gx; double* gw;
    const float* acc; int acc_s, acc_Ho, acc_Wo, Hi, Wi, T;
    int N, M, K, Q, nstrips, stages;
    int dbg;
};

template <int MT, int NT>
__global__ __launch_bounds__(256) void pf3_presplit_kernel(const float* w, int M, int K, unsigned* ws) {
    constexpr int BM = 32 * MT, BN = 32 * NT, BMP = BM + 8;
    const int e = blockIdx.x * 256 + threadIdx.x;
    if (e >= BN * (BMP / 2)) return;
    const int ci = e / (BMP / 2), mp = e - ci * (BMP / 2), co = 2 * mp;
    const float w0 = (ci < K && co < M) ? w[(long)co * K + ci] : 0.0f;
    const float w1 = (ci < K && co + 1 < M) ? w[(long)(co + 1) * K + ci] : 0.0f;
    unsigned p[3];
    pfs_split3(w0, w1, p);
#pragma unroll
    for (int s = 0; s < 3; ++s) ws[(s * BN + ci) * (BMP / 2) + mp] = p[s];
}

template <int MT, int NT>
__global__ __launch_bounds__(512, 1) void pw_bwd_fused_split3_kernel(const Pf3Args a) {
    extern __shared__ __attribute__((aligned(16))) float smem[];
    constexpr int BM = 32 * MT, BN = 32 * NT, BMP = BM + 8;
    constexpr int NG = BM / 32, NX = BN / 32;
    constexpr int NT16 = BN / 16, KS = BM / 32;
    constexpr int NR = (MT + 3) / 4;
    constexpr int NDW = NT16 / 2;
    static_assert(NT16 % 2 == 0 && NDW <= 3, "at most three data-gradient waves beside the staging wave");
    const int tid = threadIdx.x, wave = cfn_uni((int)(tid >> 6)), lane = tid & 63, half = lane >> 5, col = lane & 31;
    const int m16 = lane & 15, kq = lane >> 4;
    unsigned L = cfn_xcd_remap(blockIdx.x, gridDim.x);
    const int strip = L % a.nstrips;
    const int n = L / a.nstrips;
    const int M = a.M, K = a.K, Q = a.Q;
    constexpr int IMG = (BM + BN) * PF3_PITCH;
    float* img0 = smem;
    constexpr int OOB = 0x7ffffff0;
    const int qbeg = strip * a.stages * PF3_PT;
    const int nst = min(a.stages, (Q - qbeg + PF3_PT - 1) / PF3_PT);
    const int lrow = (tid & 255) >> 3, c4 = (tid & 7) * 4;

    if (wave < 4) {
        __amdgpu_buffer_rsrc_t rg = cfn_rsrc(const_cast<float*>(a.gy + (long)n * M * Q), (unsigned)((long)M * Q * 4));
        __amdgpu_buffer_rsrc_t ry = cfn_rsrc(const_cast<float*>((a.y ? a.y : a.gy) + (long)n * M * Q), a.y ? (unsigned)((long)M * Q * 4) : 0u);
        pf4 pg[NG], py[NG];
        int vog[NG];
        float rcs[NG], rcq[NG], rcz[NG];
#pragma unroll
        for (int it = 0; it < NG; ++it) {
            const int row = it * 32 + lrow;
            const bool ok = row < M;
            rcs[it] = (ok && a.gs) ? (float)a.gs[(long)n * M + row] : 0.0f;
            rcq[it] = (ok && a.gq && a.y) ? 2.0f * (float)a.gq[(long)n * M + row] : 0.0f;
            rcz[it] = (ok && a.gsc) ? (float)a.gsc[(long)n * M + row] : 1.0f;
            vog[it] = ok ? (row * Q + c4) * 4 : OOB;
        }
        auto prefetch = [&](int q0) {
            const bool inq = q0 + c4 < Q;
#pragma unroll
            for (int it = 0; it < NG; ++it) {
                const int vo = inq ? vog[it] : OOB;
                pg[it] = __builtin_bit_cast(pf4, __builtin_amdgcn_raw_buffer_load_b128(rg, vo, q0 * 4, 0));
                py[it] = __builtin_bit_cast(pf4, __builtin_amdgcn_raw_buffer_load_b128(ry, vo, q0 * 4, 0));
            }
        };
        auto stage = [&](int q0, float* sG) {
            const bool inq = q0 + c4 < Q;
#pragma unroll
            for (int it = 0; it < NG; ++it) {
                const int row = it * 32 + lrow;
                const float cs = rcs[it], cq = rcq[it], cz = rcz[it];
                const bool ok = inq && (row < M);
                float* d = sG + row * PF3_PITCH + c4;
                d[0] = ok ? fmaf(py[it].x, cq, fmaf(pg[it].x, cz, cs)) : 0.0f;
                d[1] = ok ? fmaf(py[it].y, cq, fmaf(pg[it].y, cz, cs)) : 0.0f;
                d[2] = ok ? fmaf(py[it].z, cq, fmaf(pg[it].z, cz, cs)) : 0.0f;
                d[3] = ok ? fmaf(py[it].w, cq, fmaf(pg[it].w, cz, cs)) : 0.0f;
            }
        };
        if (nst > 0) {
            prefetch(qbeg);
            stage(qbeg, img0);
            if (nst > 1) prefetch(qbeg + PF3_PT);
        }
        __syncthreads();
        f16v acc[NR][NT];
#pragma unroll
        for (int t = 0; t < NR; ++t)
#pragma unroll
            for (int j = 0; j < NT; ++j)
#pragma unroll
                for (int r = 0; r < 16; ++r) acc[t][j][r] = 0.0f;
        for (int st = 0; st < nst; ++st) {
            const int q0 = qbeg + st * PF3_PT;
            float* cur = img0 + (st & 1) * IMG;
            float* nxt = img0 + ((st + 1) & 1) * IMG;
            if (st + 1 < nst) {
                stage(q0 + PF3_PT, nxt);
                if (st + 2 < nst) prefetch(q0 + 2 * PF3_PT);
            }
            const float* sG = cur;
            const float* sX = cur + BM * PF3_PITCH;
            if (!(a.dbg & 1))
#pragma unroll
            for (int kb = 0; kb < 2; ++kb) {
                const int p0 = 16 * kb + 8 * half;
                pfs_u4 Af[NR][3];
#pragma unroll
                for (int t = 0; t < NR; ++t) {
                    const int i = wave + 4 * t;
                    if (i < MT) {
                        const float* r = sG + (i * 32 + col) * PF3_PITCH + p0;
#pragma unroll
                        for (int h = 0; h < 4; ++h) {
                            unsigned p[3];
                            pfs_split3(r[2 * h], r[2 * h + 1], p);
#pragma unroll
                            for (int s = 0; s < 3; ++s) Af[t][s][h] = p[s];
                        }
                    }
                }
#pragma unroll
                for (int j = 0; j < NT; ++j) {
                    pfs_u4 Bf[3];
                    const float* r = sX + (j * 32 + col) * PF3_PITCH + p0;
#pragma unroll
                    for (int h = 0; h < 4; ++h) {
                        unsigned p[3];
                        pfs_split3(r[2 * h], r[2 * h + 1], p);
#pragma unroll
                        for (int s = 0; s < 3; ++s) Bf[s][h] = p[s];
                    }
#define PF3_WG(SA, SB)                                                                                                                         \
                    _Pragma("unroll") for (int t = 0; t < NR; ++t)                                                                              \
                        if (wave + 4 * t < MT)                                                                                                  \
                            acc[t][j] = __builtin_amdgcn_mfma_f32_32x32x16_bf16(__builtin_bit_cast(pfs_bf8, Af[t][SA]), __builtin_bit_cast(pfs_bf8, Bf[SB]), acc[t][j], 0, 0, 0);
                    PFS_TERMS(PF3_WG)
#undef PF3_WG
                }
            }
            __syncthreads();
        }
#pragma unroll
        for (int t = 0; t < NR; ++t) {
            const int i = wave + 4 * t;
            if (i < MT) {
#pragma unroll
                for (int j = 0; j < NT; ++j)
#pragma unroll
                    for (int r = 0; r < 16; ++r) {
                        const int gm = i * 32 + (r & 3) + 8 * (r >> 2) + 4 * half, gk = j * 32 + col;
                        const float v = acc[t][j][r];
                        if (gm < M && gk < K) cfn_add64(&a.gw[(long)gm * K + gk], (double)v);
                    }
            }
        }
    } else if (wave < 4 + NDW) {
        const int d = wave - 4;
        __amdgpu_buffer_rsrc_t rd = cfn_rsrc(a.gx + (long)n * K * Q, (unsigned)((long)K * Q * 4));
        __amdgpu_buffer_rsrc_t rw = cfn_rsrc(const_cast<unsigned*>(a.wsplit), (unsigned)((size_t)3 * BN * (BMP / 2) * 4));
        const int wlane = ((m16 * BMP + 8 * kq) / 2) * 4;
        pfs_u4 Wr[2][KS][3];
#pragma unroll
        for (int t = 0; t < 2; ++t)
#pragma unroll
            for (int s = 0; s < KS; ++s)
#pragma unroll
                for (int u = 0; u < 3; ++u)
                    Wr[t][s][u] = __builtin_bit_cast(pfs_u4, __builtin_amdgcn_raw_buffer_load_b128(rw, wlane, (((u * BN + (2 * d + t) * 16) * BMP + 32 * s) / 2) * 4, 0));
        const int hw = a.Hi * a.Wi;
        const int acc_pitch4 = a.T * a.acc_Ho * a.acc_Wo * 4;
        __amdgpu_buffer_rsrc_t racc = cfn_rsrc(const_cast<float*>(a.acc ? a.acc + (long)n * K * (acc_pitch4 / 4) : a.gy), a.acc ? (unsigned)((long)K * acc_pitch4) : 0u);
        __syncthreads();
        for (int st = 0; st < nst; ++st) {
            const int q0 = qbeg + st * PF3_PT;
            const float* sG = img0 + (st & 1) * IMG;
            float av[2][2][4];
#pragma unroll
            for (int pb = 0; pb < 2; ++pb)
#pragma unroll
                for (int t = 0; t < 2; ++t)
#pragma unroll
                    for (int r = 0; r < 4; ++r) av[pb][t][r] = 0.0f;
            if (a.acc) {
#pragma unroll
                for (int pb = 0; pb < 2; ++pb) {
                    const int q = q0 + 16 * pb + m16;
                    int aoff = OOB;
                    if (q < Q) {
                        const int tq = q / hw, rq = q - tq * hw;
                        const int hq = rq / a.Wi, wq_ = rq - hq * a.Wi;
                        if (hq % a.acc_s == 0 && wq_ % a.acc_s == 0) aoff = (((tq * a.acc_Ho + hq / a.acc_s) * a.acc_Wo + wq_ / a.acc_s)) * 4;
                    }
                    const unsigned arow = (unsigned)aoff + (unsigned)(4 * kq) * (unsigned)acc_pitch4;
#pragma unroll
                    for (int t = 0; t < 2; ++t)
#pragma unroll
                        for (int r = 0; r < 4; ++r)
                            av[pb][t][r] = __builtin_bit_cast(float, __builtin_amdgcn_raw_buffer_load_b32(
                                racc, (int)(aoff == OOB ? (unsigned)OOB : arow + (unsigned)r * (unsigned)acc_pitch4), (2 * d + t) * 16 * acc_pitch4, 0));
                }
            }
            pf4 da[2][2];
#pragma unroll
            for (int pb = 0; pb < 2; ++pb)
#pragma unroll
                for (int t = 0; t < 2; ++t) da[pb][t] = (pf4){0.f, 0.f, 0.f, 0.f};
            if (!(a.dbg & 2))
#pragma unroll
            for (int s = 0; s < KS; ++s) {
#pragma unroll
                for (int pb = 0; pb < 2; ++pb) {
                    const float* r = sG + (32 * s + 8 * kq) * PF3_PITCH + 16 * pb + m16;
                    pfs_u4 Gf[3];
#pragma unroll
                    for (int h = 0; h < 4; ++h) {
                        unsigned p[3];
                        pfs_split3(r[(2 * h) * PF3_PITCH], r[(2 * h + 1) * PF3_PITCH], p);
#pragma unroll
                        for (int u = 0; u < 3; ++u) Gf[u][h] = p[u];
                    }
#define PF3_DG(SA, SB)                                                                                                                         \
                    _Pragma("unroll") for (int t = 0; t < 2; ++t)                                                                               \
                        da[pb][t] = __builtin_amdgcn_mfma_f32_16x16x32_bf16(__builtin_bit_cast(pfs_bf8, Wr[t][s][SA]), __builtin_bit_cast(pfs_bf8, Gf[SB]), da[pb][t], 0, 0, 0);
                    PFS_TERMS(PF3_DG)
#undef PF3_DG
                }
            }
            float* tile = smem + 2 * IMG + d * (32 * PF3_TP);
#pragma unroll
            for (int pb = 0; pb < 2; ++pb)
#pragma unroll
                for (int t = 0; t < 2; ++t)
#pragma unroll
                    for (int r = 0; r < 4; ++r) {
                        const float v = da[pb][t][r] + av[pb][t][r];
                        tile[(t * 16 + 4 * kq + r) * PF3_TP + 16 * pb + m16] = v;
                    }
            __builtin_amdgcn_fence(__ATOMIC_RELEASE, "wavefront");
            __builtin_amdgcn_wave_barrier();
            __builtin_amdgcn_fence(__ATOMIC_ACQUIRE, "wavefront");
            {
                const int seg = lane & 7, r0 = lane >> 3;
                const bool inq = q0 + 4 * seg < Q && !(a.dbg & 8);
#pragma unroll
                for (int ps = 0; ps < 4; ++ps) {
                    const int row = ps * 8 + r0;
                    const pf4 v = *reinterpret_cast<const pf4*>(tile + row * PF3_TP + 4 * seg);
                    __builtin_amdgcn_raw_buffer_store_b128(__builtin_bit_cast(pfs_u4, v), rd, inq ? (r0 * Q + 4 * seg) * 4 : OOB, (q0 + (32 * d + ps * 8) * Q) * 4, 0);
                }
            }
            __syncthreads();
        }
    } else if (wave < 7) {
        __syncthreads();
        for (int st = 0; st < nst; ++st) __syncthreads();
    } else {
        __amdgpu_buffer_rsrc_t rx = cfn_rsrc(const_cast<float*>(a.x + (long)n * K * Q), (unsigned)((long)K * Q * 4));
        constexpr int NP = BN / 8;
        const int xrow = lane >> 3;
        pf4 px[NP];
        int vox[NP];
#pragma unroll
        for (int it = 0; it < NP; ++it) vox[it] = (it * 8 + xrow) < K ? ((it * 8 + xrow) * Q + c4) * 4 : OOB;
        auto prefetch = [&](int q0) {
            const bool inq = q0 + c4 < Q;
#pragma unroll
            for (int it = 0; it < NP; ++it)
                px[it] = __builtin_bit_cast(pf4, __builtin_amdgcn_raw_buffer_load_b128(rx, inq ? vox[it] : OOB, q0 * 4, 0));
        };
        auto stage = [&](float* sX) {
#pragma unroll
            for (int it = 0; it < NP; ++it) {
                float* dd = sX + (it * 8 + xrow) * PF3_PITCH + c4;
                dd[0] = px[it].x; dd[1] = px[it].y; dd[2] = px[it].z; dd[3] = px[it].w;
            }
        };
        if (nst > 0) {
            prefetch(qbeg);
            stage(img0 + BM * PF3_PITCH);
            if (nst > 1) prefetch(qbeg + PF3_PT);
        }
        __syncthreads();
        for (int st = 0; st < nst; ++st) {
            const int q0 = qbeg + st * PF3_PT;
            float* nxt = img0 + ((st + 1) & 1) * IMG;
            if (st + 1 < nst) {
                stage(nxt + BM * PF3_PITCH);
                if (st + 2 < nst) prefetch(q0 + 2 * PF3_PT);
            }
            __syncthreads();
        }
    }
// ... 39 lines not shown
        __amdgpu_buffer_rsrc_t ry = cfn_rsrc(const_cast<float*>((a.y ? a.y : a.gy) + (long)n * M * Q), a.y ? (unsigned)((long)M * Q * 4) : 0u);
        __amdgpu_buffer_rsrc_t rx = cfn_rsrc(const_cast<float*>(a.x + (long)n * K * Q), (unsigned)((long)K * Q * 4));
        pf4 pg[NG], py[NG], px[NX];
        int vog[NG], vox[NX];
        float rcs[NG], rcq[NG], rcz[NG];
#pragma unroll
        for (int it = 0; it < NG; ++it) {
            const int row = it * 32 + lrow;
            const bool ok = row < M;
            rcs[it] = (ok && a.gs) ? (float)a.gs[(long)n * M + row] : 0.0f;
            rcq[it] = (ok && a.gq && a.y) ? 2.0f * (float)a.gq[(long)n * M + row] : 0.0f;
            rcz[it] = (ok && a.gsc) ? (float)a.gsc[(long)n * M + row] : 1.0f;
            vog[it] = ok ? (row * Q + c4) * 4 : OOB;
        }
#pragma unroll
        for (int it = 0; it < NX; ++it) vox[it] = (it * 32 + lrow) < K ? ((it * 32 + lrow) * Q + c4) * 4 : OOB;
        auto prefetch = [&](int q0) {
            const bool inq = q0 + c4 < Q;
#pragma unroll
            for (int it = 0; it < NG; ++it) {
                const int vo = inq ? vog[it] : OOB;
                pg[it] = __builtin_bit_cast(pf4, __builtin_amdgcn_raw_buffer_load_b128(rg, vo, q0 * 4, 0));
                py[it] = __builtin_bit_cast(pf4, __builtin_amdgcn_raw_buffer_load_b128(ry, vo, q0 * 4, 0));
            }
#pragma unroll
            for (int it = 0; it < NX; ++it)
                px[it] = __builtin_bit_cast(pf4, __builtin_amdgcn_raw_buffer_load_b128(rx, inq ? vox[it] : OOB, q0 * 4, 0));
        };
        auto stage = [&](int q0, float* sG, float* sX) {
            const bool inq = q0 + c4 < Q;
#pragma unroll
            for (int it = 0; it < NG; ++it) {
                const int row = it * 32 + lrow;
                const float cs = rcs[it], cq = rcq[it], cz = rcz[it];
                const bool ok = inq && (row < M);
                float* d = sG + row * PF3_PITCH + c4;
                d[0] = ok ? fmaf(py[it].x, cq, fmaf(pg[it].x, cz, cs)) : 0.0f;
                d[1] = ok ? fmaf(py[it].y, cq, fmaf(pg[it].y, cz, cs)) : 0.0f;
                d[2] = ok ? fmaf(py[it].z, cq, fmaf(pg[it].z, cz, cs)) : 0.0f;
                d[3] = ok ? fmaf(py[it].w, cq, fmaf(pg[it].w, cz, cs)) : 0.0f;
            }
#pragma unroll
            for (int it = 0; it < NX; ++it) {
                float* d = sX + (it * 32 + lrow) * PF3_PITCH + c4;
                d[0] = px[it].x; d[1] = px[it].y; d[2] = px[it].z; d[3] = px[it].w;
            }
        };
        if (nst > 0) {
            prefetch(qbeg);
            stage(qbeg, img0, img0 + BM * PF3_PITCH);
            if (nst > 1) prefetch(qbeg + PF3_PT);
        }
        float ca[NC], cb[NC];
#pragma unroll
        for (int c = 0; c < NC; ++c) {
            const int k = (wave + 4 * c) * 32 + col;
            const bool ok = k < K;
            ca[c] = ok ? (float)a.pa[(long)n * K + k] : 1.0f;
            cb[c] = ok ? (float)a.pb[(long)n * K + k] : 0.0f;
        }
        __syncthreads();
        f16v acc[NC][MT];
#pragma unroll
        for (int c = 0; c < NC; ++c)
#pragma unroll
            for (int i = 0; i < MT; ++i)
#pragma unroll
                for (int r = 0; r < 16; ++r) acc[c][i][r] = 0.0f;
        for (int st = 0; st < nst; ++st) {
            const int q0 = qbeg + st * PF3_PT;
            float* cur = img0 + (st & 1) * IMG;
            float* nxt = img0 + ((st + 1) & 1) * IMG;
            if (st + 1 < nst) {
                stage(q0 + PF3_PT, nxt, nxt + BM * PF3_PITCH);
                if (st + 2 < nst) prefetch(q0 + 2 * PF3_PT);
            }
            const float* sG = cur;
            const float* sX = cur + BM * PF3_PITCH;
#pragma unroll
            for (int kb = 0; kb < 2; ++kb) {
                const int p0 = 16 * kb + 8 * half;
                pfs_u4 Bf[NC][3];
#pragma unroll
                for (int c = 0; c < NC; ++c) {
                    const int j = wave + 4 * c;
                    if (j < NT) {
                        const float* r = sX + (j * 32 + col) * PF3_PITCH + p0;
#pragma unroll
                        for (int h = 0; h < 4; ++h) {
                            const float x0 = cfn_act<ACT>(fmaf(r[2 * h], ca[c], cb[c])), x1 = cfn_act<ACT>(fmaf(r[2 * h + 1], ca[c], cb[c]));
                            unsigned p[3];
                            pfs_split3(x0, x1, p);
#pragma unroll
                            for (int s = 0; s < 3; ++s) Bf[c][s][h] = p[s];
                        }
                    }
                }
#pragma unroll
                for (int i = 0; i < MT; ++i) {
                    pfs_u4 Af[3];
                    const float* r = sG + (i * 32 + col) * PF3_PITCH + p0;
#pragma unroll
                    for (int h = 0; h < 4; ++h) {
                        unsigned p[3];
                        pfs_split3(r[2 * h], r[2 * h + 1], p);
#pragma unroll
                        for (int s = 0; s < 3; ++s) Af[s][h] = p[s];
                    }
#define PF3E_WG(SA, SB)                                                                                                                        \
                    _Pragma("unroll") for (int c = 0; c < NC; ++c)                                                                              \
                        if (wave + 4 * c < NT)                                                                                                  \
                            acc[c][i] = __builtin_amdgcn_mfma_f32_32x32x16_bf16(__builtin_bit_cast(pfs_bf8, Af[SA]), __builtin_bit_cast(pfs_bf8, Bf[c][SB]), acc[c][i], 0, 0, 0);
                    PFS_TERMS(PF3E_WG)
#undef PF3E_WG
                }
            }
            __syncthreads();
        }
#pragma unroll
        for (int c = 0; c < NC; ++c) {
            const int j = wave + 4 * c;
            if (j < NT) {
#pragma unroll
                for (int i = 0; i < MT; ++i)
#pragma unroll
                    for (int r = 0; r < 16; ++r) {
                        const int gm = i * 32 + (r & 3) + 8 * (r >> 2) + 4 * half, gk = j * 32 + col;
                        const float v = acc[c][i][r];
                        if (gm < M && gk < K) cfn_add64(&a.gw[(long)gm * K + gk], (double)v);
                    }
            }
        }
    } else {
        const int d = wave - 4;
        const int tb = ND * d, tn = ND;
        __amdgpu_buffer_rsrc_t rd = cfn_rsrc(a.gx + (long)n * K * Q, (unsigned)((long)K * Q * 4));
        __amdgpu_buffer_rsrc_t rw = cfn_rsrc(const_cast<unsigned*>(a.wsplit), (unsigned)((size_t)3 * BN * (BMP / 2) * 4));
        const int wlane = ((m16 * BMP + 8 * kq) / 2) * 4;
        pfs_u4 Wr[ND][KS][3];
#pragma unroll
        for (int t = 0; t < ND; ++t)
#pragma unroll
            for (int s = 0; s < KS; ++s)
#pragma unroll
                for (int u = 0; u < 3; ++u)
                    Wr[t][s][u] = (t < tn && tb + t < NT16) ? __builtin_bit_cast(pfs_u4, __builtin_amdgcn_raw_buffer_load_b128(rw, wlane, cfn_uni((((u * BN + (tb + t) * 16) * BMP + 32 * s) / 2) * 4), 0))
                                                      : (pfs_u4){0u, 0u, 0u, 0u};
        float sa[ND][4], sb[ND][4];
#pragma unroll
        for (int t = 0; t < ND; ++t)
#pragma unroll
            for (int r = 0; r < 4; ++r) { sa[t][r] = 0.0f; sb[t][r] = 0.0f; }
        __syncthreads();
        for (int st = 0; st < nst; ++st) {
            const int q0 = qbeg + st * PF3_PT;
            const float* sG = img0 + (st & 1) * IMG;
            const float* sX = sG + BM * PF3_PITCH;
            pf4 da[2][ND];
#pragma unroll
            for (int pb = 0; pb < 2; ++pb)
#pragma unroll
                for (int t = 0; t < ND; ++t) da[pb][t] = (pf4){0.f, 0.f, 0.f, 0.f};
#pragma unroll
            for (int s = 0; s < KS; ++s) {
#pragma unroll
                for (int pb = 0; pb < 2; ++pb) {
                    const float* r = sG + (32 * s + 8 * kq) * PF3_PITCH + 16 * pb + m16;
                    pfs_u4 Gf[3];
#pragma unroll
                    for (int h = 0; h < 4; ++h) {
                        unsigned p[3];
                        pfs_split3(r[(2 * h) * PF3_PITCH], r[(2 * h + 1) * PF3_PITCH], p);
#pragma unroll
                        for (int u = 0; u < 3; ++u) Gf[u][h] = p[u];
                    }
#define PF3E_DG(SA, SB)                                                                                                                        \
                    _Pragma("unroll") for (int t = 0; t < ND; ++t)                                                                              \
                        da[pb][t] = __builtin_amdgcn_mfma_f32_16x16x32_bf16(__builtin_bit_cast(pfs_bf8, Wr[t][s][SA]), __builtin_bit_cast(pfs_bf8, Gf[SB]), da[pb][t], 0, 0, 0);
                    PFS_TERMS(PF3E_DG)
#undef PF3E_DG
                }
            }
#pragma unroll
            for (int pb = 0; pb < 2; ++pb) {
                const int q = q0 + 16 * pb + m16;
                const int gvo = q < Q ? (4 * kq * Q + 16 * pb + m16) * 4 : OOB;
#pragma unroll
                for (int t = 0; t < ND; ++t) {
#pragma unroll
                    for (int r = 0; r < 4; ++r) {
                        const int ci = (tb + t) * 16 + 4 * kq + r;
                        const float v = da[pb][t][r];
                        const float xr = sX[ci * PF3_PITCH + 16 * pb + m16];
                        const float2 pab = cfn_settle(*reinterpret_cast<const float2*>(sCx + 2 * ci));
                        const float dz = v * cfn_act_grad<ACT>(fmaf(xr, pab.x, pab.y));
                        sa[t][r] = fmaf(dz, xr, sa[t][r]);
                        sb[t][r] += dz;
                        const float o = dz * pab.x;
                        __builtin_amdgcn_raw_buffer_store_b32(__builtin_bit_cast(unsigned, o), rd, gvo, (q0 + ((tb + t) * 16 + r) * Q) * 4, 0);
                    }
                    __builtin_amdgcn_sched_barrier(0);
                }
            }
            __syncthreads();
        }
#pragma unroll
        for (int t = 0; t < ND; ++t)
#pragma unroll
            for (int r = 0; r < 4; ++r) {
                float u = sa[t][r], v = sb[t][r];
#pragma unroll
                for (int o = 1; o < 16; o <<= 1) { u += __shfl_xor(u, o, 64); v += __shfl_xor(v, o, 64); }
                const int ci = (tb + t) * 16 + 4 * kq + r;
                if (m16 == 0 && t < tn && ci < K) {
                    cfn_add64(&a.gA[(long)n * K + ci], (double)u);
                    cfn_add64(&a.gB[(long)n * K + ci], (double)v);
                }
            }
    }
}

static unsigned* pf3_workspace(size_t bytes, hipStream_t st) {
    static std::mutex mu;
    static std::map<std::pair<int, hipStream_t>, std::pair<unsigned*, size_t>> bufs;
    int dev = 0;
    if (hipGetDevice(&dev) != hipSuccess) { (void)hipGetLastError(); return nullptr; }
    std::lock_guard<std::mutex> lk(mu);
    auto& b = bufs[std::make_pair(dev, st)];
    if (b.second >= bytes) return b.first;
    hipStreamCaptureStatus cs = hipStreamCaptureStatusNone;
    if (hipStreamIsCapturing(st, &cs) != hipSuccess || cs != hipStreamCaptureStatusNone) return nullptr;
    unsigned* p = nullptr;
    if (hipMalloc(&p, bytes) != hipSuccess) { (void)hipGetLastError(); return nullptr; }
    b = {p, bytes};
    return p;
}

template <int NT>
static int pf3_launch(const float* gy, const float* y, const double* gsum, const double* gsumsq, const float* w, const float* x, float* gx, double* gw,
                      int N, int Cin, int Cout, int T, int Hi, int Wi, const float* acc, int acc_stride, const double* gscale, hipStream_t st) {
    constexpr int MT = 7, BM = 32 * MT, BN = 32 * NT, BMP = BM + 8;
    const long Ql = (long)T * Hi * Wi;
    const size_t wbytes = (size_t)3 * BN * (BMP / 2) * 4;
    unsigned* ws = pf3_workspace(wbytes, st);
    if (!ws) return -1;
    hipLaunchKernelGGL((pf3_presplit_kernel<MT, NT>), dim3((BN * (BMP / 2) + 255) / 256), dim3(256), 0, st, w, Cout, Cin, ws);
    Pf3Args a = {};
    a.gy = gy; a.y = gsumsq ? y : nullptr; a.gs = gsum; a.gq = gsumsq; a.gsc = gscale; a.x = x; a.wsplit = ws; a.gx = gx; a.gw = gw;
    a.acc = acc; a.acc_s = acc ? acc_stride : 1; a.Hi = Hi; a.Wi = Wi; a.T = T;
    a.acc_Ho = (Hi - 1) / a.acc_s + 1; a.acc_Wo = (Wi - 1) / a.acc_s + 1;
    a.N = N; a.M = Cout; a.K = Cin; a.Q = (int)Ql;
#ifdef CFN_PWFS_KNOCKOUTS
    { const char* e = getenv("CFN_PWFS_DBG"); a.dbg = e ? atoi(e) : 0; }
#endif
    const long nst = cfn_cdiv(Ql, PF3_PT);
    const long wgs = (long)N * nst > 256L * 100 ? 512 : 256;
    long want = wgs / N;
    if (want < 1) want = 1;
    long stages = cfn_cdiv(nst, want);
    if (stages < 4) stages = 4;
    a.stages = (int)stages;
    a.nstrips = (int)cfn_cdiv(nst, stages);
    const unsigned blocks = (unsigned)((long)N * a.nstrips);
    const size_t lds = ((size_t)2 * (BM + BN) * PF3_PITCH + 3 * 32 * PF3_TP) * sizeof(float);
    CfnProfScope prof(CFN_K_PWCONV_BWD, st, 4.0 * N * ((double)Cout * Ql * (a.y ? 2 : 1) + (double)Cin * Ql * 2));
    auto k = pw_bwd_fused_split3_kernel<MT, NT>;
    (void)hipFuncSetAttribute((const void*)k, hipFuncAttributeMaxDynamicSharedMemorySize, (int)lds);
    hipLaunchKernelGGL(k, dim3(blocks), dim3(512), lds, st, a);
    return cfn_check_launch("pwconv_bwd_fused (split bf16, layer 3)");
}

static int pf3e_try_launch(const float* gy, const float* y, const double* gsum, const double* gsumsq, const float* w, const float* x, const double* A, const double* B,
                           int act, float* gx, double* gA, double* gB, double* gw, int N, int Cin, int Cout, long Ql, const double* gscale, hipStream_t st) {
    constexpr int MT = 3, NT = 7, BM = 32 * MT, BN = 32 * NT, BMP = BM + 8;
    const size_t wbytes = (size_t)3 * BN * (BMP / 2) * 4;
    unsigned* ws = pf3_workspace(wbytes, st);
    if (!ws) return -1;
    hipLaunchKernelGGL((pf3_presplit_kernel<MT, NT>), dim3((BN * (BMP / 2) + 255) / 256), dim3(256), 0, st, w, Cout, Cin, ws);
    Pf3eArgs a = {};
    a.gy = gy; a.y = gsumsq ? y : nullptr; a.gs = gsum; a.gq = gsumsq; a.gsc = gscale; a.x = x; a.pa = A; a.pb = B; a.wsplit = ws;
    a.gx = gx; a.gA = gA; a.gB = gB; a.gw = gw;
    a.N = N; a.M = Cout; a.K = Cin; a.Q = (int)Ql;
    const long nst = cfn_cdiv(Ql, PF3_PT);
    long want = 256 / N;
    if (want < 1) want = 1;
    long stages = cfn_cdiv(nst, want);
    if (stages < 4) stages = 4;
    a.stages = (int)stages;
    a.nstrips = (int)cfn_cdiv(nst, stages);
    const unsigned blocks = (unsigned)((long)N * a.nstrips);
    const size_t lds = ((size_t)2 * (BM + BN) * PF3_PITCH + 2 * BN) * sizeof(float);
    CfnProfScope prof(CFN_K_PWCONV_BWD, st, 4.0 * N * ((double)Cout * Ql * (a.y ? 2 : 1) + (double)Cin * Ql * 2));
#define CFN_PF3E_GO(ACTV)                                                                                       \
    do {                                                                                                        \
        auto k = pw_bwd_fused_split3e_kernel<MT, NT, ACTV>;                                                     \
        (void)hipFuncSetAttribute((const void*)k, hipFuncAttributeMaxDynamicSharedMemorySize, (int)lds);        \
        hipLaunchKernelGGL(k, dim3(blocks), dim3(512), lds, st, a);                                             \
    } while (0)
    if (act == CFN_ACT_RELU) CFN_PF3E_GO(CFN_ACT_RELU);
    else if (act == CFN_ACT_SWISH) CFN_PF3E_GO(CFN_ACT_SWISH);
    else CFN_PF3E_GO(CFN_ACT_NONE);
#undef CFN_PF3E_GO
    return cfn_check_launch("pwconv_bwd_fused (split bf16, layer 3 conv3)");
}

int pwfs_try_launch(const float* gy, const float* y, const double* gsum, const double* gsumsq, const float* w, const float* x, const double* A,
                    const double* B, int act, float* gx, double* gA, double* gB, double* gw, int N, int Cin, int Cout, int T, int Hi, int Wi,
                    const float* acc, int acc_stride, const double* gscale, hipStream_t st) {
    const char* env_on = getenv("CFN_PWF_SPLIT");
    const int on = env_on ? atoi(env_on) : 1;
    if (!on || pws_terms_now() != 6) return -1;
    const bool wide_m = Cout > 64 && Cout <= 128 && Cin > 32 && Cin <= 64;
    const bool thin_k = Cout > 64 && Cout <= 128 && Cin >= 16 && Cin <= 32;
    const bool wide_k = Cin > 64 && Cin <= 128 && Cout > 32 && Cout <= 64;
    if (on >= 1 && A == nullptr && Cout > 192 && Cout <= 224 && Cin > 32 && Cin <= 96) {
        const long Ql3 = (long)T * Hi * Wi;
        if (Ql3 % 4 == 0 && Ql3 < (1L << 30) && (long)Cout * Ql3 * 4 < 0x7ffffff0L && ((((uintptr_t)gy | (uintptr_t)x | (uintptr_t)(y ? y : gy)) & 15) == 0) &&
            (acc == nullptr || acc_stride >= 1)) {
            if (Cin > 64) return pf3_launch<3>(gy, y, gsum, gsumsq, w, x, gx, gw, N, Cin, Cout, T, Hi, Wi, acc, acc_stride, gscale, st);
            return pf3_launch<2>(gy, y, gsum, gsumsq, w, x, gx, gw, N, Cin, Cout, T, Hi, Wi, acc, acc_stride, gscale, st);
        }
    }
    const char* env_l3e = getenv("CFN_PWF_L3E");
    const int l3e_on = env_l3e ? atoi(env_l3e) : 0;
    if (on >= 1 && l3e_on && A != nullptr && acc == nullptr && Cout > 64 && Cout <= 96 && Cin > 192 && Cin <= 224) {
        const long Ql3 = (long)T * Hi * Wi;
        if (Ql3 % 4 == 0 && Ql3 < (1L << 30) && (long)Cin * Ql3 * 4 < 0x7ffffff0L && ((((uintptr_t)gy | (uintptr_t)x | (uintptr_t)(y ? y : gy)) & 15) == 0) &&
            (act == CFN_ACT_NONE || act == CFN_ACT_RELU || act == CFN_ACT_SWISH))
            return pf3e_try_launch(gy, y, gsum, gsumsq, w, x, A, B, act, gx, gA, gB, gw, N, Cin, Cout, Ql3, gscale, st);
    }
    if (!wide_m && !wide_k && !thin_k) return -1;
    if (A != nullptr && on < 2) return -1;
    const long Ql = (long)T * Hi * Wi;
    if (Ql % 4 != 0 || Ql >= (1L << 30)) return -1;
    if ((long)Cout * Ql * 4 >= 0x7ffffff0L || (long)Cin * Ql * 4 >= 0x7ffffff0L) return -1;
    if (A && act != CFN_ACT_NONE && act != CFN_ACT_RELU && act != CFN_ACT_SWISH) return -1;
    if ((((uintptr_t)gy | (uintptr_t)x | (uintptr_t)(y ? y : gy)) & 15) != 0) return -1;
    PfsArgs a = {};
    a.gy = gy; a.y = gsumsq ? y : nullptr; a.gs = gsum; a.gq = gsumsq; a.gsc = gscale; a.w = w; a.x = x; a.pa = A; a.pb = B;
    a.gx = gx; a.gA = gA; a.gB = gB; a.gw = gw;
    a.acc = acc; a.acc_s = acc ? acc_stride : 1; a.Hi = Hi; a.Wi = Wi; a.T = T;
    a.acc_Ho = (Hi - 1) / a.acc_s + 1; a.acc_Wo = (Wi - 1) / a.acc_s + 1;
    a.N = N; a.M = Cout; a.K = Cin; a.Q = (int)Ql;
#ifdef CFN_PWFS_KNOCKOUTS
    { const char* e = getenv("CFN_PWFS_DBG"); a.dbg = e ? atoi(e) : 0; }
#endif
    const long nst = cfn_cdiv(Ql, PFS_PT);
    long want = 512 / N;
    if (want < 1) want = 1;
    long stages = cfn_cdiv(nst, want);
    if (stages < 4) stages = 4;
    a.stages = (int)stages;
    a.nstrips = (int)cfn_cdiv(nst, stages);
    const unsigned blocks = (unsigned)((long)N * a.nstrips);
    CfnProfScope prof(CFN_K_PWCONV_BWD, st, 4.0 * N * ((double)Cout * Ql * (a.y ? 2 : 1) + (double)Cin * Ql * 2));
    const bool epi = A != nullptr;
    if (wide_m) return pfs_launch<4, 2>(a, act, epi, blocks, st);
    if (thin_k) return pfs_launch<4, 1>(a, act, epi, blocks, st);
    return pfs_launch<2, 4>(a, act, epi, blocks, st);
}
```

coarse-fine-networks_amd/x3d_fine.py:

```python
import os

import torch
import torch.nn as nn
import torch.nn.functional as F

from cfn_hip import ops, ACT_NONE, ACT_RELU, ACT_SWISH
from cfn_hip.u8clips import U8Clips

USE_TORCH_OPS = os.environ.get('CFN_USE_TORCH_OPS', '0') == '1'


class Deferred(object):
    __slots__ = ('raw', 'A', 'B', 'act')

    def __init__(self, raw, A, B, act):
        self.raw, self.A, self.B, self.act = raw, A, B, act

    @property
    def shape(self):
        return self.raw.shape

    def materialize(self):
        return ops.affine_act(self.raw, self.A, self.B, self.act)


def _unpack(x):
    if isinstance(x, Deferred):
        return x.raw, x.A, x.B, x.act
    return x, None, None, ACT_NONE


class SubBatchNorm3d(nn.Module):

    def __init__(self, num_splits, **args):
        super(SubBatchNorm3d, self).__init__()
        self.num_splits = num_splits
        self.num_features = args['num_features']
        self.eps = args.get('eps', 1e-5)
        self.momentum = args.get('momentum', 0.1)
        if args.get('affine', True):
            self.affine = True
            self.weight = nn.Parameter(torch.ones(self.num_features))
            self.bias = nn.Parameter(torch.zeros(self.num_features))
        else:
            self.affine = False
        self.bn = nn.BatchNorm3d(self.num_features, eps=self.eps, momentum=self.momentum, affine=False)
        self.split_bn = nn.BatchNorm3d(self.num_features * self.num_splits, eps=self.eps, momentum=self.momentum,
                                       affine=False)

    def aggregate_stats(self):
        if self.split_bn.track_running_stats:
            n = self.num_splits
            means = self.split_bn.running_mean.view(n, -1)
            mean = means.sum(0) / n
            var = self.split_bn.running_var.view(n, -1).sum(0) / n + ((means - mean) ** 2).sum(0) / n
            self.bn.running_mean.data = mean.detach()
            self.bn.running_var.data = var.detach()

    def fold(self, s, q, count, n, se=None):
        if self.training:
            bufs = (self.split_bn.running_mean, self.split_bn.running_var, self.split_bn.num_batches_tracked)
        else:
            bufs = (self.bn.running_mean, self.bn.running_var, self.bn.num_batches_tracked)
        gamma, beta = (self.weight, self.bias) if self.affine else (None, None)
        return ops.bn_fold(s, q, gamma, beta, bufs, self.training, n, self.num_features, self.num_splits, count, self.eps,
                           self.momentum, se=se, pool_count=count)

    def fold_op(self, s, q, count, n, se=None):
        tr = self.training
        bn = self.split_bn if tr else self.bn
        gamma, beta = (self.weight, self.bias) if self.affine else (None, None)
        w1, b1, w2, b2 = se if se is not None else (None, None, None, None)
        out = torch.ops.cfn.bn_fold(s, q, gamma, beta, bn.running_mean, bn.running_var, bn.num_batches_tracked, tr, n,
                                    self.num_features, self.num_splits, float(count), self.eps, self.momentum, w1, b1, w2, b2, float(count))
        if tr:
            with torch.no_grad():
                bn.running_mean.copy_(out[9])
                bn.running_var.copy_(out[10])
                bn.num_batches_tracked.copy_(out[11])
        return out[0], out[1]

    def forward(self, x):
        n = x.shape[0]
        s = q = None
        if self.training:
            s, q = ops.channel_stats(x)
        A, B = self.fold(s, q, x[0, 0].numel(), n)
        return ops.affine_act(x, A, B, ACT_NONE)


class Swish(nn.Module):

    def forward(self, x):
        n, c = x.shape[:2]
        one = torch.ones(n, c, device=x.device)
        return ops.affine_act(x, one, torch.zeros_like(one), ACT_SWISH)


def conv3x3x3(in_planes, out_planes, stride=1, t_downsample=False):
    return nn.Conv3d(in_planes, out_planes, kernel_size=3, stride=stride if t_downsample else (1, stride, stride), padding=1,
                     bias=False, groups=in_planes)


def conv1x1x1(in_planes, out_planes, stride=1, t_downsample=False):
    return nn.Conv3d(in_planes, out_planes, kernel_size=1, stride=stride if t_downsample else (1, stride, stride), bias=False)


def _every(x, s):
    return x if s == 1 else x[:, :, ::s].contiguous()


def _count(y):
    return y.shape[2] * y.shape[3] * y.shape[4]


class Bottleneck(nn.Module):

    def __init__(self, in_planes, planes, stride=1, downsample=None, index=0, base_bn_splits=8, t_downsample=False):
        super(Bottleneck, self).__init__()
        self.index = index
        self.base_bn_splits = base_bn_splits
        self.conv1 = conv1x1x1(in_planes, planes[0])
        self.bn1 = SubBatchNorm3d(num_splits=base_bn_splits, num_features=planes[0], affine=True)
        self.conv2 = conv3x3x3(planes[0], planes[0], stride, t_downsample=t_downsample)
        self.bn2 = SubBatchNorm3d(num_splits=base_bn_splits, num_features=planes[0], affine=True)
        self.conv3 = conv1x1x1(planes[0], planes[1], t_downsample=t_downsample)
        self.bn3 = SubBatchNorm3d(num_splits=base_bn_splits, num_features=planes[1], affine=True)
        self.swish = Swish()
        self.relu = nn.ReLU(inplace=True)
        if self.index % 2 == 0:
            width = self.round_width(planes[0])
            self.global_pool = nn.AdaptiveAvgPool3d((1, 1, 1))
            self.fc1 = nn.Conv3d(planes[0], width, kernel_size=1, stride=1)
            self.fc2 = nn.Conv3d(width, planes[0], kernel_size=1, stride=1)
            self.sigmoid = nn.Sigmoid()
        self.downsample = downsample
        self.stride = stride
        self.t_stride = stride if t_downsample else 1
        self.split_out = False

    def round_width(self, width, multiplier=0.0625, min_width=8, divisor=8):
        if not multiplier:
            return width
        width *= multiplier
        min_width = min_width or divisor
        width_out = max(min_width, int(width + divisor / 2) // divisor * divisor)
        if width_out < 0.9 * width:
            width_out += divisor
        return int(width_out)

    def _forward_torch_ops(self, x):
        import cfn_hip.torchlib
        T = torch.ops.cfn
        if isinstance(x, tuple):
            x = x[0]
        if isinstance(x, Deferred):
            x = x.materialize()
        if self.t_stride != 1 or (self.downsample is not None and not isinstance(self.downsample, nn.Sequential)):
            raise NotImplementedError('CFN_USE_TORCH_OPS: t_downsample / shortcut type A run on the default path only')
        n = x.shape[0]
        has_se = self.index % 2 == 0
        y1, s1, q1 = T.pwconv(x, self.conv1.weight, None, None, ACT_NONE, 1)
        A1, B1 = self.bn1.fold_op(s1, q1, _count(y1), n)
        y2, s2, q2 = T.dwconv3d(y1, self.conv2.weight, A1, B1, ACT_RELU, self.stride)
        se = (self.fc1.weight, self.fc1.bias, self.fc2.weight, self.fc2.bias) if has_se else None
        A2, B2 = self.bn2.fold_op(s2, q2, _count(y2), n, se=se)
        y3, s3, q3 = T.pwconv(y2, self.conv3.weight, A2, B2, ACT_SWISH, 1)
        A3, B3 = self.bn3.fold_op(s3, q3, _count(y3), n)
        if self.downsample is not None:
            yd, sd, qd = T.pwconv(x, self.downsample[0].weight, None, None, ACT_NONE, self.stride)
            Ad, Bd = self.downsample[1].fold_op(sd, qd, _count(yd), n)
            return T.bn_add_relu(y3, A3, B3, yd, Ad, Bd)
        return T.bn_add_relu(y3, A3, B3, x)

    def forward(self, x):
        if USE_TORCH_OPS:
            return self._forward_torch_ops(x)
        x, x_res = x if isinstance(x, tuple) else (x, x)
        xr, xa, xb, xact = _unpack(x)
        n = xr.shape[0]
        tr = self.training
        has_se = self.index % 2 == 0

        ts = self.t_stride
        tok = ops.ShortcutToken() if (isinstance(self.downsample, nn.Sequential) and self.stride > 1 and ts == 1) else None
        y1, s1, q1 = ops.pwconv(xr, self.conv1.weight, xa, xb, xact, 1, stats=tr, token=tok, role='main')
        A1, B1 = self.bn1.fold(s1, q1, _count(y1), n)
        if ts == 1:
            y2, s2, q2 = ops.dwconv3d(y1, self.conv2.weight, A1, B1, ACT_RELU, self.stride, stats=tr or has_se)
        else:
            y2f, _, _ = ops.dwconv3d(y1, self.conv2.weight, A1, B1, ACT_RELU, self.stride, stats=False)
            y2 = _every(y2f, ts)
            s2, q2 = ops.channel_stats(y2) if (tr or has_se) else (None, None)
        se = (self.fc1.weight, self.fc1.bias, self.fc2.weight, self.fc2.bias) if has_se else None
        A2, B2 = self.bn2.fold(s2, q2, _count(y2), n, se=se)
        link = ops.TailLink() if torch.is_grad_enabled() else None
        y3, s3, q3 = ops.pwconv(y2, self.conv3.weight, A2, B2, ACT_SWISH, 1, stats=tr, tail=link, tail_role='y')
        A3, B3 = self.bn3.fold(s3, q3, _count(y3), n)

        if self.downsample is not None:
            if not isinstance(self.downsample, nn.Sequential):
                _, planes_out, s_ = self.downsample
                xm = x_res.materialize() if isinstance(x_res, Deferred) else x_res
                res = xm.detach()[:, :, ::s_, ::s_, ::s_]
                if planes_out > res.shape[1]:
                    res = torch.cat([res, res.new_zeros((res.shape[0], planes_out - res.shape[1]) + tuple(res.shape[2:]))], dim=1)
                return ops.bn_add_relu(y3, A3, B3, res.contiguous(), split=self.split_out, link=link)
            yd, sd, qd = ops.pwconv(_every(xr, ts), self.downsample[0].weight, xa, xb, xact, self.stride, stats=tr, token=tok, role='short',
                                    tail=link, tail_role='res')
            Ad, Bd = self.downsample[1].fold(sd, qd, _count(yd), n)
            return ops.bn_add_relu(y3, A3, B3, yd, Ad, Bd, split=self.split_out, link=link)
        res = x_res.materialize() if isinstance(x_res, Deferred) else x_res
        return ops.bn_add_relu(y3, A3, B3, res, split=self.split_out, link=link)


class ResNet(nn.Module):

    def __init__(self, block, layers, block_inplanes, n_input_channels=3, conv1_t_size=7, conv1_t_stride=1,
                 shortcut_type='B', widen_factor=1.0, dropout=0.5, n_classes=400, base_bn_splits=8, task='class',
                 extract_feat=False, global_tower=False, t_downsample=False, aux_losses=None, _skip_module_init=False,
                 act_dtype=None):
        if not _skip_module_init:
            super(ResNet, self).__init__()
        block_inplanes = [(int(x * widen_factor), int(y * widen_factor)) for x, y in block_inplanes]
        self.index = 0
        self.base_bn_splits = base_bn_splits
        self.task = task
        self.extract_feat = extract_feat
        self.global_tower = global_tower
        self.t_downsample = t_downsample
        self.act_dtype = {None: torch.float32, 'f32': torch.float32, 'fp32': torch.float32, torch.float32: torch.float32,
                          'bf16': torch.bfloat16, torch.bfloat16: torch.bfloat16,
                          'fp16': torch.float16, 'f16': torch.float16, torch.float16: torch.float16}[act_dtype]
        self.in_planes = block_inplanes[0][1]

        self.conv1_s = nn.Conv3d(n_input_channels, self.in_planes, kernel_size=(1, 3, 3), stride=(1, 2, 2),
                                 padding=(0, 1, 1), bias=False)
        self.conv1_t = nn.Conv3d(self.in_planes, self.in_planes, kernel_size=(5, 1, 1), stride=(1, 1, 1),
                                 padding=(2, 0, 0), bias=False, groups=self.in_planes)
        self.bn1 = SubBatchNorm3d(num_splits=base_bn_splits, num_features=self.in_planes, affine=True)
        self.relu = nn.ReLU(inplace=True)
        self.layer1 = self._make_layer(block, block_inplanes[0], layers[0], shortcut_type, stride=2)
        self.layer2 = self._make_layer(block, block_inplanes[1], layers[1], shortcut_type, stride=2)
        self.layer3 = self._make_layer(block, block_inplanes[2], layers[2], shortcut_type, stride=2)
        self.layer4 = self._make_layer(block, block_inplanes[3], layers[3], shortcut_type, stride=2)
        self.conv5 = nn.Conv3d(block_inplanes[3][1], block_inplanes[3][0], kernel_size=(1, 1, 1), stride=(1, 1, 1),
                               padding=(0, 0, 0), bias=False)
        self.bn5 = SubBatchNorm3d(num_splits=base_bn_splits, num_features=block_inplanes[3][0], affine=True)
        if task == 'class':
            self.avgpool = nn.AdaptiveAvgPool3d((1, 1, 1))
        elif task == 'loc':
            self.avgpool = nn.AdaptiveAvgPool3d((None, 1, 1))
        self.fc1 = nn.Conv3d(block_inplanes[3][0], 2048, bias=False, kernel_size=1, stride=1)
        self.fc2 = nn.Linear(2048, n_classes)
        self.dropout = nn.Dropout(dropout)

        for m in self.modules():
            if isinstance(m, nn.Conv3d):
                nn.init.kaiming_normal_(m.weight, mode='fan_out', nonlinearity='relu')

    def _make_layer(self, block, planes, blocks, shortcut_type, stride=1):
        downsample = None
        if stride != 1 or self.in_planes != planes[1]:
            if shortcut_type == 'A':
                downsample = ('A', planes[1], stride)
            else:
                downsample = nn.Sequential(
                    conv1x1x1(self.in_planes, planes[1], stride, t_downsample=self.t_downsample),
                    SubBatchNorm3d(num_splits=self.base_bn_splits, num_features=planes[1], affine=True))
        layers = [block(in_planes=self.in_planes, planes=planes, stride=stride, downsample=downsample,
                        index=self.index, base_bn_splits=self.base_bn_splits, t_downsample=self.t_downsample)]
        self.in_planes = planes[1]
        self.index += 1
        for _ in range(1, blocks):
            layers.append(block(self.in_planes, planes, index=self.index, base_bn_splits=self.base_bn_splits,
                                t_downsample=self.t_downsample))
            self.index += 1
        self.index = 0
        for blk in layers[:-1]:
            blk.split_out = True
        return nn.Sequential(*layers)

    def replace_logits(self, n_classes):
        self.fc2 = nn.Linear(2048, n_classes).to(self.fc1.weight.device)

    def update_bn_splits_long_cycle(self, long_cycle_bn_scale):
        for m in self.modules():
            if isinstance(m, SubBatchNorm3d):
                m.num_splits = self.base_bn_splits * long_cycle_bn_scale
                m.split_bn = nn.BatchNorm3d(num_features=m.num_features * m.num_splits, affine=False).to(m.weight.device)
        return self.base_bn_splits * long_cycle_bn_scale

    def aggregate_sub_bn_stats(self):
        count = 0
        for m in self.modules():
            if isinstance(m, SubBatchNorm3d):
                m.aggregate_stats()
                count += 1
        return count

    def set_input_norm(self, mean, std, norm_value=255):
        lut = ops.clip_lut(mean, std, norm_value).to(self.conv1_s.weight.device)
        self.register_buffer('input_lut', lut, persistent=False)
        return self

    def _conv1_s(self, x):
        if not isinstance(x, U8Clips):
            return ops.stem_conv(x, self.conv1_s.weight)
        lut = getattr(self, 'input_lut', None)
        if lut is None:
            raise RuntimeError('the model was handed uint8 frames (U8Clips) but does not know how to normalise them: call '
                               'set_input_norm(mean, std) first (e.g. CHARADES_MEAN / CHARADES_STD)')
        if x.frames.dim() != 5:
            raise RuntimeError('U8Clips of shape (N, T, H, W, 3) expected (flatten_crops() a collated batch), got %s'
                               % (tuple(x.frames.shape),))
        return ops.stem_conv_u8(x.frames, x.lengths, lut, self.conv1_s.weight)

    def _stem(self, x):
        y = self._conv1_s(x)
        y, s, q = ops.dwconv_t5(y, self.conv1_t.weight, stats=self.training, out_dtype=self.act_dtype)
        A, B = self.bn1.fold(s, q, _count(y), y.shape[0])
        return Deferred(y, A, B, ACT_RELU)

    def _head(self, x):
        n = x.shape[0]
        y5, s5, q5 = ops.pwconv(x, self.conv5.weight, stats=self.training)
        A5, B5 = self.bn5.fold(s5, q5, _count(y5), n)
        if self.task == 'class':
            pooled = ops.pool_hw(y5, 1, 1, A5, B5, ACT_RELU).mean(dim=2, keepdim=True)
        else:
            pooled = ops.pool_hw(y5, 1, 1, A5, B5, ACT_RELU)
        if self.extract_feat:
            return pooled
        f1, _, _ = ops.pwconv(pooled, self.fc1.weight, stats=False)
        one = torch.ones(n, f1.shape[1], device=f1.device)
        z = ops.affine_act(f1, one, torch.zeros_like(one), ACT_RELU)
        z = self.dropout(z)
        out, _, _ = ops.pwconv(z, self.fc2.weight.view(self.fc2.weight.shape[0], -1, 1, 1, 1), stats=False)
        out = out.squeeze(4).squeeze(3) + self.fc2.bias.view(1, -1, 1)
        return out

    def forward(self, inp):
        x, masks = inp
        x = self._stem(x)
        feat_g = {}
        for i, layer in enumerate((self.layer1, self.layer2, self.layer3, self.layer4), start=1):
            x = layer(x)
            if self.global_tower:
                feat_g['layer%d' % i] = ops.pool_hw(x, 7, 7)
        if self.global_tower:
            n = x.shape[0]
            y5, s5, q5 = ops.pwconv(x, self.conv5.weight, stats=self.training)
            A5, B5 = self.bn5.fold(s5, q5, _count(y5), n)
            feat_g['conv5'] = ops.pool_hw(y5, 7, 7, A5, B5, ACT_RELU)
            return feat_g, masks
        return self._head(x)


def replace_logits(self, n_classes):
    self.fc2 = nn.Linear(2048, n_classes)


def get_inplanes(version):
    planes = {'S': [(54, 24), (108, 48), (216, 96), (432, 192)],
              'M': [(54, 24), (108, 48), (216, 96), (432, 192)],
              'XL': [(72, 32), (162, 72), (306, 136), (630, 280)]}
    return planes[version]


def get_blocks(version):
    blocks = {'S': [3, 5, 11, 7], 'M': [3, 5, 11, 7], 'XL': [5, 10, 25, 15]}
    return blocks[version]


def generate_model(x3d_version, **kwargs):
    return ResNet(Bottleneck, get_blocks(x3d_version), get_inplanes(x3d_version), **kwargs)
```

include/cfn_hip.h:

```cpp
#ifndef CFN_HIP_H
#define CFN_HIP_H
#ifdef __cplusplus
extern "C" {
#endif

const char* cfn_last_error(void);
const char* cfn_version(void);
int cfn_device_info(int* cus, int* lds_per_cu, char* name, int name_len);

int cfn_prof_enable(int family, int on);
int cfn_prof_collect(int family, double* total_ms, long* launches, double* total_bytes);

int cfn_dwconv3d_fwd(const float* x, const double* A, const double* B, int act, const float* w, float* y, double* sum,
                     double* sumsq, int N, int C, int T, int Hi, int Wi, int stride, void* stream);
int cfn_dwconv3d_bwd_data(const float* gy, const float* y, const double* gsum, const double* gsumsq, const float* w,
                          const float* x, const double* A, const double* B, int act, float* gx, double* gA, double* gB,
                          int N, int C, int T, int Hi, int Wi, int stride, void* stream);
int cfn_dwconv3d_bwd_weight(const float* gy, const float* y, const double* gsum, const double* gsumsq, const float* x,
                            const double* A, const double* B, int act, double* gw, int N, int C, int T, int Hi, int Wi,
                            int stride, void* stream);
int cfn_dwconv3d_bwd_fused(const float* gy, const float* y, const double* gsum, const double* gsumsq, const float* w,
                           const float* x, const double* A, const double* B, int act, float* gx, double* gA, double* gB,
                           double* gw, int N, int C, int T, int H, int W, void* stream);
int cfn_dwconv3d_bwd_fused_s2(const float* gy, const float* y, const double* gsum, const double* gsumsq, const float* w,
                              const float* x, const double* A, const double* B, int act, float* gx, double* gA, double* gB,
                              double* gw, int N, int C, int T, int H, int W, void* stream);

int cfn_dwconv_t5_fwd(const float* x, const float* w, float* y, double* sum, double* sumsq, int N, int C, int T,
                      long plane, void* stream);
int cfn_dwconv_t5_bwd_data(const float* gy, const float* y, const double* gsum, const double* gsumsq, const float* w,
                           float* gx, int N, int C, int T, long plane, void* stream);
int cfn_dwconv_t5_bwd_weight(const float* gy, const float* y, const double* gsum, const double* gsumsq, const float* x,
                             double* gw, int N, int C, int T, long plane, void* stream);
int cfn_dwconv_t5_bwd_fused(const float* gy, const float* y, const double* gsum, const double* gsumsq, const float* w,
                            const float* x, float* gx, double* gw, int N, int C, int T, long plane, void* stream);

int cfn_pwconv_fwd(const float* x, const double* A, const double* B, int act, const float* w, float* y, double* sum,
                   double* sumsq, int N, int Cin, int Cout, int T, int Hi, int Wi, int stride, void* stream);
int cfn_pwconv_bwd_data(const float* gy, const float* y, const double* gsum, const double* gsumsq, const float* w,
                        const float* x, const double* A, const double* B, int act, float* gx, double* gA, double* gB, int N,
                        int Cin, int Cout, int T, int Hi, int Wi, int stride, void* stream);
int cfn_pwconv_bwd_data_acc(const float* gy, const float* y, const double* gsum, const double* gsumsq, const float* w,
                        const float* x, const double* A, const double* B, int act, float* gx, double* gA, double* gB, int N,
                        int Cin, int Cout, int T, int Hi, int Wi, int stride, const float* acc, int acc_stride,
                        const double* gscale, void* stream);
int cfn_pwconv_bwd_weight(const float* gy, const float* y, const double* gsum, const double* gsumsq, const float* x,
                          const double* A, const double* B, int act, double* gw, int N, int Cin, int Cout, int T, int Hi,
                          int Wi, int stride, const double* gscale, void* stream);

int cfn_pw_split_terms(int terms);

int cfn_deterministic(int on);

int cfn_pwconv_bwd_fused(const float* gy, const float* y, const double* gsum, const double* gsumsq, const float* w,
                         const float* x, const double* A, const double* B, int act, float* gx, double* gA, double* gB,
                         double* gw, int N, int Cin, int Cout, int T, int Hi, int Wi, const float* acc, int acc_stride,
                         const double* gscale, void* stream);

int cfn_pwconv_short_bwd(const float* gy, const float* y, const double* gsum, const double* gsumsq, const double* gscale,
                         const float* w, const float* x, const double* A, const double* B, int act, float* da, double* gw,
                         int N, int Cin, int Cout, int T, int Hi, int Wi, int stride, void* stream);

int cfn_stem_conv_fwd(const float* x, const float* w, float* y, int N, int Cimg, int Cout, int T, int Hi, int Wi,
                      void* stream);
int cfn_stem_conv_bwd_weight(const float* gy, const float* x, double* gw, int N, int Cimg, int Cout, int T, int Hi, int Wi,
                             void* stream);

int cfn_clip_u8_to_f32(const unsigned char* frames, const float* lut, const int* lengths, float* x, int N, int T, int H, int W,
                       void* stream);
int cfn_stem_conv_u8_fwd(const unsigned char* frames, const float* lut, const int* lengths, const float* w, float* y, int N,
                         int Cimg, int Cout, int T, int Hi, int Wi, void* stream);
int cfn_stem_conv_u8_bwd_weight(const float* gy, const unsigned char* frames, const float* lut, const int* lengths, double* gw,
                                int N, int Cimg, int Cout, int T, int Hi, int Wi, void* stream);

int cfn_bn_fold_fwd(const double* s, const double* q, const float* gamma, const float* beta, float* run_mean, float* run_var,
                    long* nbt, int training, int N, int C, int S, double count, double eps, double momentum, const float* w1,
                    const float* b1, const float* w2, const float* b2, int Wd, double pool_count, double* A, double* B,
                    double* mean, double* rstd, float* A0, float* B0, float* gate, float* hbuf, float* pooled, void* stream);
int cfn_bn_fold_bwd(const double* gA, const double* gB, const double* s, const float* gamma, const double* mean,
                    const double* rstd, const float* A0, const float* B0, const float* gate, const float* hbuf,
                    const float* pooled, const float* w1, const float* w2, int training, int N, int C, int S, int Wd,
                    double count, double pool_count, double* gs, double* gq, float* ggamma, float* gbeta, float* gw1,
                    float* gb1, float* gw2, float* gb2, double* tA, double* tB, void* stream);

int cfn_conv3d_dense_fwd(const float* x, const double* A, const double* B, int act, const float* w, float* y, double* sum,
                         double* sumsq, int N, int Cin, int Cout, int T, int Hi, int Wi, const int* geom, void* stream);
int cfn_conv3d_dense_bwd_data(const float* gy, const float* y, const double* gsum, const double* gsumsq, const float* w,
                              const float* x, const double* A, const double* B, int act, float* gx, double* gA, double* gB,
                              int N, int Cin, int Cout, int T, int Hi, int Wi, const int* geom, void* stream);
int cfn_conv3d_dense_bwd_weight(const float* gy, const float* y, const double* gsum, const double* gsumsq, const float* x,
                                const double* A, const double* B, int act, double* gw, int N, int Cin, int Cout, int T, int Hi,
                                int Wi, const int* geom, void* stream);

int cfn_gauss_align_fwd(const long* meta, const float* mask, const float* gx, double tx, double ratio, float* GX, int B, int crops,
                        int Tf, int K, void* stream);
int cfn_gauss_align_bwd(const float* gGX, const long* meta, const float* mask, const float* gx, double tx, double ratio,
                        float* ggx, int B, int crops, int Tf, int K, void* stream);

int cfn_fusion_gather_fwd(const float* x, const float* at_raw, const float* at_bias, const float* GX, const float* mask, float* z,
                          float* den, int B, int crops, int C, int Tf, int K, int P, void* stream);
int cfn_fusion_gather_bwd(const float* gz, const float* z, const float* den, const float* x, const float* at_raw,
                          const float* at_bias, const float* GX, const float* mask, float* gx, float* gat, float* gGX, float* dw,
                          int B, int crops, int C, int Tf, int K, int P, void* stream);

int cfn_bn_add_relu_fwd(const float* y, const double* A, const double* B, const float* res, const double* Ar, const double* Br,
                        float* out, int* mask, long NC, long vol, void* stream);
int cfn_bn_add_relu_bwd(const float* gout, const float* gout2, const float* out, const float* y, const double* A, const float* res,
                        const double* Ar, float* gy, float* gres, double* gA, double* gB, double* gAr, long NC, long vol,
                        void* stream);
long cfn_bn_add_relu_mask_words(long NC, long vol);
int cfn_bn_add_relu_bwd_g(const float* gout, const float* gout2, const float* out, const int* mask, const float* y,
                          const float* res, float* g, double* gA, double* gB, double* gAr, long NC, long vol, void* stream);

int cfn_affine_act_fwd(const float* x, const double* A, const double* B, int act, float* out, long NC, long vol, void* stream);
int cfn_affine_act_bwd(const float* gout, const float* x, const double* A, const double* B, int act, float* gx, double* gA,
                       double* gB, long NC, long vol, void* stream);
int cfn_channel_stats(const float* x, double* sum, double* sumsq, long NC, long vol, void* stream);

int cfn_pool_hw_fwd(const float* x, const double* A, const double* B, int act, float* out, long NC, int T, int H, int W, int OH,
                    int OW, void* stream);
int cfn_pool_hw_bwd(const float* gout, const float* x, const double* A, const double* B, int act, float* gx, double* gA,
                    double* gB, long NC, int T, int H, int W, int OH, int OW, void* stream);

int cfn_film_fwd(const float* x, const float* m, const float* c, float* out, long NC, int T, int H, int W, int f,
                 void* stream);
int cfn_film_bwd(const float* g, const float* x, const float* m, float* gx, float* gm, float* gc, long NC, int T, int H,
                 int W, int f, void* stream);

int cfn_grid_time_index(const float* cdf, int n, int Tin, int* i0, float* w1, void* stream);
int cfn_grid_cdf_fwd(const float* g, const float* bias, float* cdf, int B, int Kin, void* stream);
int cfn_grid_cdf_bwd(const float* gcdf, const float* g, const float* bias, float* gg, int B, int Kin, void* stream);
int cfn_time_sample_fwd(const float* x, const float* cdf, float* out, int B, int C, int Tin, int K, long P, void* stream);
int cfn_time_sample_bwd(const float* g, const float* x, const float* cdf, float* gx, double* gcdf, int B, int C, int Tin,
                        int K, long P, void* stream);

int cfn_time_pool_fwd(const float* x, float* out, int mode, long BC, int Tin, int R, long P, void* stream);
int cfn_time_pool_bwd(const float* g, const float* x, float* gx, int mode, long BC, int Tin, int R, long P, void* stream);

int cfn_interp1d_fwd(const float* x, const float* y, const float* xnew, float* ynew, long* ind, int B, int N, int Pq,
                     int xrow, int yrow, int qrow, void* stream);
int cfn_interp1d_bwd(const float* g, const float* x, const float* y, const float* xnew, const long* ind, float* gx, float* gy,
                     float* gq, int B, int N, int Pq, int xrow, int yrow, int qrow, void* stream);

int cfn_time_resize_fwd(const float* x, float* out, long BC, int Kin, int Lout, long P, int align_corners, void* stream);
int cfn_time_resize_bwd(const float* g, float* gx, long BC, int Kin, int Lout, long P, int align_corners, void* stream);

int cfn_detloss_fwd(const float* logits, const float* labels, const float* masks, const float* norm, double world, float* probs,
                    float* cls, float* loc, int* jstar, float* ymax, double* rows, double* norm_used, int B, int C, int T, int TL,
                    int n, int align_corners, void* stream);
int cfn_detloss_bwd(const float* g_cls, const float* g_loc, const float* logits, const float* labels, const float* masks,
                    const int* jstar, const float* ymax, const double* norm_used, double world, float* gx, int B, int C, int T,
                    int TL, int n, int align_corners, void* stream);

int cfn_pwconv_fwd_bf16(const unsigned short* x, const double* A, const double* B, int act, const float* w, unsigned short* y,
                        double* sum, double* sumsq, int N, int Cin, int Cout, long Q, void* stream);
int cfn_pwconv_bwd_data_bf16(const unsigned short* gy, const unsigned short* y, const double* gsum, const double* gsumsq,
                             const float* w, const unsigned short* x, const double* A, const double* B, int act,
                             unsigned short* gx, double* gA, double* gB, int N, int Cin, int Cout, int T, int H, int W,
                             const unsigned short* acc, int acc_stride, const double* gscale, void* stream);
int cfn_pwconv_bwd_weight_bf16(const unsigned short* gy, const unsigned short* y, const double* gsum, const double* gsumsq,
                               const unsigned short* x, const double* A, const double* B, int act, double* gw, int N, int Cin,
                               int Cout, long Q, const double* gscale, void* stream);
int cfn_subsample_hw_bf16(const unsigned short* x, unsigned short* out, long planes, int H, int W, int s, void* stream);

int cfn_dwconv3d_fwd_bf16(const unsigned short* x, const double* A, const double* B, int act, const float* w, unsigned short* y,
                          double* sum, double* sumsq, int N, int C, int T, int Hi, int Wi, int stride, void* stream);
int cfn_dwconv3d_bwd_data_bf16(const unsigned short* gy, const unsigned short* y, const double* gsum, const double* gsumsq,
                               const float* w, const unsigned short* x, const double* A, const double* B, int act,
                               unsigned short* gx, double* gA, double* gB, int N, int C, int T, int Hi, int Wi, int stride,
                               void* stream);
int cfn_dwconv3d_bwd_weight_bf16(const unsigned short* gy, const unsigned short* y, const double* gsum, const double* gsumsq,
                                 const unsigned short* x, const double* A, const double* B, int act, double* gw, int N, int C,
                                 int T, int Hi, int Wi, int stride, void* stream);
int cfn_dwconv3d_bwd_fused_bf16(const unsigned short* gy, const unsigned short* y, const double* gsum, const double* gsumsq,
                                const float* w, const unsigned short* x, const double* A, const double* B, int act,
                                unsigned short* gx, double* gA, double* gB, double* gw, int N, int C, int T, int H, int W,
                                void* stream);
int cfn_dwconv3d_bwd_fused_s2_bf16(const unsigned short* gy, const unsigned short* y, const double* gsum, const double* gsumsq,
                                   const float* w, const unsigned short* x, const double* A, const double* B, int act,
                                   unsigned short* gx, double* gA, double* gB, double* gw, int N, int C, int T, int H, int W,
                                   void* stream);

int cfn_dwconv_t5_fwd_bf16(const float* x, const float* w, unsigned short* y, double* sum, double* sumsq, int N, int C, int T,
                           long plane, void* stream);
int cfn_dwconv_t5_bwd_data_bf16(const unsigned short* gy, const unsigned short* y, const double* gsum, const double* gsumsq,
                                const float* w, float* gx, int N, int C, int T, long plane, void* stream);
int cfn_dwconv_t5_bwd_weight_bf16(const unsigned short* gy, const unsigned short* y, const double* gsum, const double* gsumsq,
                                  const float* x, double* gw, int N, int C, int T, long plane, void* stream);
int cfn_dwconv_t5_bwd_fused_bf16(const unsigned short* gy, const unsigned short* y, const double* gsum, const double* gsumsq,
                                 const float* w, const float* x, float* gx, double* gw, int N, int C, int T, long plane,
                                 void* stream);

long cfn_bn_add_relu_mask_words_bf16(long NC, long vol);
int cfn_bn_add_relu_fwd_bf16(const unsigned short* y, const double* A, const double* B, const unsigned short* res,
                             const double* Ar, const double* Br, unsigned short* out, int* mask, long NC, long vol, void* stream);
int cfn_bn_add_relu_bwd_g_bf16(const unsigned short* gout, const unsigned short* gout2, const unsigned short* out, const int* mask,
                               const unsigned short* y, const unsigned short* res, unsigned short* g, double* gA, double* gB,
                               double* gAr, long NC, long vol, void* stream);
int cfn_pool_hw_fwd_bf16(const unsigned short* x, const double* A, const double* B, int act, float* out, long NC, int T, int H,
                         int W, int OH, int OW, void* stream);
int cfn_pool_hw_bwd_bf16(const float* gout, const unsigned short* x, const double* A, const double* B, int act,
                         unsigned short* gx, double* gA, double* gB, long NC, int T, int H, int W, int OH, int OW, void* stream);

int cfn_pwconv_fwd_f16(const unsigned short* x, const double* A, const double* B, int act, const float* w, unsigned short* y,
                        double* sum, double* sumsq, int N, int Cin, int Cout, long Q, void* stream);
int cfn_pwconv_bwd_data_f16(const unsigned short* gy, const unsigned short* y, const double* gsum, const double* gsumsq,
                             const float* w, const unsigned short* x, const double* A, const double* B, int act,
                             unsigned short* gx, double* gA, double* gB, int N, int Cin, int Cout, int T, int H, int W,
                             const unsigned short* acc, int acc_stride, const double* gscale, void* stream);
int cfn_pwconv_bwd_weight_f16(const unsigned short* gy, const unsigned short* y, const double* gsum, const double* gsumsq,
                               const unsigned short* x, const double* A, const double* B, int act, double* gw, int N, int Cin,
                               int Cout, long Q, const double* gscale, void* stream);
int cfn_subsample_hw_f16(const unsigned short* x, unsigned short* out, long planes, int H, int W, int s, void* stream);

int cfn_dwconv3d_fwd_f16(const unsigned short* x, const double* A, const double* B, int act, const float* w, unsigned short* y,
                          double* sum, double* sumsq, int N, int C, int T, int Hi, int Wi, int stride, void* stream);
int cfn_dwconv3d_bwd_data_f16(const unsigned short* gy, const unsigned short* y, const double* gsum, const double* gsumsq,
                               const float* w, const unsigned short* x, const double* A, const double* B, int act,
                               unsigned short* gx, double* gA, double* gB, int N, int C, int T, int Hi, int Wi, int stride,
                               void* stream);
int cfn_dwconv3d_bwd_weight_f16(const unsigned short* gy, const unsigned short* y, const double* gsum, const double* gsumsq,
                                 const unsigned short* x, const double* A, const double* B, int act, double* gw, int N, int C,
                                 int T, int Hi, int Wi, int stride, void* stream);
int cfn_dwconv3d_bwd_fused_f16(const unsigned short* gy, const unsigned short* y, const double* gsum, const double* gsumsq,
                                const float* w, const unsigned short* x, const double* A, const double* B, int act,
                                unsigned short* gx, double* gA, double* gB, double* gw, int N, int C, int T, int H, int W,
                                void* stream);
int cfn_dwconv3d_bwd_fused_s2_f16(const unsigned short* gy, const unsigned short* y, const double* gsum, const double* gsumsq,
                                   const float* w, const unsigned short* x, const double* A, const double* B, int act,
                                   unsigned short* gx, double* gA, double* gB, double* gw, int N, int C, int T, int H, int W,
                                   void* stream);

int cfn_dwconv_t5_fwd_f16(const float* x, const float* w, unsigned short* y, double* sum, double* sumsq, int N, int C, int T,
                           long plane, void* stream);
int cfn_dwconv_t5_bwd_data_f16(const unsigned short* gy, const unsigned short* y, const double* gsum, const double* gsumsq,
                                const float* w, float* gx, int N, int C, int T, long plane, void* stream);
int cfn_dwconv_t5_bwd_weight_f16(const unsigned short* gy, const unsigned short* y, const double* gsum, const double* gsumsq,
                                  const float* x, double* gw, int N, int C, int T, long plane, void* stream);
int cfn_dwconv_t5_bwd_fused_f16(const unsigned short* gy, const unsigned short* y, const double* gsum, const double* gsumsq,
                                 const float* w, const float* x, float* gx, double* gw, int N, int C, int T, long plane,
                                 void* stream);

long cfn_bn_add_relu_mask_words_f16(long NC, long vol);
int cfn_bn_add_relu_fwd_f16(const unsigned short* y, const double* A, const double* B, const unsigned short* res,
                             const double* Ar, const double* Br, unsigned short* out, int* mask, long NC, long vol, void* stream);
int cfn_bn_add_relu_bwd_g_f16(const unsigned short* gout, const unsigned short* gout2, const unsigned short* out, const int* mask,
                               const unsigned short* y, const unsigned short* res, unsigned short* g, double* gA, double* gB,
                               double* gAr, long NC, long vol, void* stream);
int cfn_pool_hw_fwd_f16(const unsigned short* x, const double* A, const double* B, int act, float* out, long NC, int T, int H,
                         int W, int OH, int OW, void* stream);
int cfn_pool_hw_bwd_f16(const float* gout, const unsigned short* x, const double* A, const double* B, int act,
                         unsigned short* gx, double* gA, double* gB, long NC, int T, int H, int W, int OH, int OW, void* stream);

int cfn_crop_resize_flip_u8(const unsigned char* src, const int* lengths, const int* box, const int* bounds, const int* coef,
                            unsigned char* dst, int N, int T, int Hs, int Ws, int S, int K, void* stream);

int cfn_ap_append(const float* probs, const float* labels, const int* valid, float* scores, unsigned char* targets, int* count,
                  int* flags, int B, int K, int TL, long cap, void* stream);
int cfn_ap_sort(const float* scores, const unsigned char* targets, const int* count, float* sorted_scores,
                unsigned char* sorted_targets, int* tmp_keys, unsigned char* tmp_targets, int K, long cap, void* stream);
int cfn_ap_reduce(const unsigned char* sorted_targets, const int* count, float* ap, int K, long cap, void* stream);
int cfn_ap_sort_tile(void);

int cfn_feat_unpack_f16(const unsigned short* data, const long* offsets, const int* lengths, float* out0, float* out1, float* out2,
                        float* out3, float* out4, int B, int t_max, int c0, int c1, int c2, int c3, int c4, long total, void* stream);
int cfn_feat_unpack_bf16(const unsigned short* data, const long* offsets, const int* lengths, float* out0, float* out1, float* out2,
                         float* out3, float* out4, int B, int t_max, int c0, int c1, int c2, int c3, int c4, long total, void* stream);
int cfn_feat_pack_f16(const float* x0, const float* x1, const float* x2, const float* x3, const float* x4, unsigned short* dst, int T,
                      int c0, int c1, int c2, int c3, int c4, void* stream);
int cfn_feat_pack_bf16(const float* x0, const float* x1, const float* x2, const float* x3, const float* x4, unsigned short* dst, int T,
                       int c0, int c1, int c2, int c3, int c4, void* stream);

long cfn_jpeg_workspace_bytes(int rows, long slots, int lanes, int blocks_max);
int cfn_jpeg_decode_u8(const unsigned char* data, const int* frames, const int* tables, const int* geom, const int* lengths,
                       unsigned char* out, int* status, void* ws, long ws_bytes, long data_bytes, int rows, int sets, int N,
                       int Tmax, int Hmax, int Wmax, int lanes, int blocks_max, void* stream);

int cfn_seg_labels(const double* seg, const int* offsets, const double* fps, const int* window, float* labels, float* mask,
                   int* valid_t, int B, int C, int t_max, long n_seg, void* stream);

#ifdef __cplusplus
}
#endif
#endif
```

Before: 107.0 clips/s.

## Fold previous block's bn-add-relu backward into next block's conv1 fused backward

Adds a tail-fold path where the next block's conv1 fused backward kernel also applies the previous block's relu mask, adds the skip gradient and accumulates the BN scale/shift (and residual scale) gradients. The previous block's bn_add_relu backward then reuses that result instead of launching its own kernel. This is meant to remove a full read/write pass over the block-output gradient per residual block. In exchange it adds extra loads and registers to the fused kernel, plus fragile cross-autograd state that raises an error if the block output has other consumers.

Result: no change. 107.9 clips/s, median of 6 (+0.8%).

```diff
diff --git a/coarse-fine-networks_amd/cfn_hip/ops.py b/coarse-fine-networks_amd/cfn_hip/ops.py
--- a/coarse-fine-networks_amd/cfn_hip/ops.py
+++ b/coarse-fine-networks_amd/cfn_hip/ops.py
@@ -181,6 +181,16 @@
         self.done = False
 
 
+TAIL_FOLD = True
+
+
+class TailFold(object):
+
+    def __init__(self):
+        self.y = self.res = self.g2 = self.out = None
+        self.folded = 0
+
+
 def _bf(t):
     return t is not None and t.dtype in (torch.bfloat16, torch.float16)
 
@@ -195,7 +205,7 @@
 class _PwConv(Function):
 
     @staticmethod
-    def forward(ctx, x, A, B, w, act, stride, want_stats, token, role, tail=None, tail_role=None):
+    def forward(ctx, x, A, B, w, act, stride, want_stats, token, role, tail=None, tail_role=None, fold=None):
         x = check(x).contiguous()
         N, Cin, T, H, W = x.shape
         Cout = w.shape[0]
@@ -217,6 +227,7 @@
         ctx.wparam = w
         ctx.token, ctx.role = token, role
         ctx.tail, ctx.tail_role = tail, tail_role
+        ctx.fold = fold
         if not want_stats:
             return y, None, None
         return y, s, q
@@ -264,8 +275,20 @@
                         token.main_done = True
                 if stride == 1 and ctx.needs_input_grad[3]:
                     g64, fin = _gw_buffers(ctx.wparam, Cout, Cin, x.device)
-                    fused = call_try('cfn_pwconv_bwd_fused', gy, y, gs, gq, w2, x, A, B, act, gx, a64, b64, g64, N, Cin, Cout,
-                                     T, H, W, acc, acc_stride, gsc)
+                    fold = ctx.fold
+                    if (fold is not None and TAIL_FOLD and fold.out is None and fold.y is not None and fold.g2 is not None
+                            and A is None and acc is None and ctx.needs_input_grad[0]
+                            and tuple(fold.y.shape) == tuple(x.shape) and tuple(fold.g2.shape) == tuple(x.shape)):
+                        t3 = _tls.arena.take(3 * N * Cin, x.device).view(3, N, Cin)
+                        gAr = t3[2] if fold.res is not None else None
+                        fused = call_try('cfn_pwconv_bwd_fused_tail', gy, y, gs, gq, w2, x, gx, g64, N, Cin, Cout, T, H, W, gsc,
+                                         fold.g2, fold.y, t3[0], t3[1], fold.res, gAr)
+                        if fused:
+                            fold.out = (gx, fold.g2, t3[0], t3[1], gAr)
+                            fold.folded += 1
+                    if not fused:
+                        fused = call_try('cfn_pwconv_bwd_fused', gy, y, gs, gq, w2, x, A, B, act, gx, a64, b64, g64, N, Cin, Cout,
+                                         T, H, W, acc, acc_stride, gsc)
                 if not fused:
                     call('cfn_pwconv_bwd_data_acc', gy, y, gs, gq, w2, x, A, B, act, gx, a64, b64, N, Cin, Cout, T, H, W, stride,
                          acc, acc_stride, gsc)
@@ -277,7 +300,7 @@
             if not fused:
                 call('cfn_pwconv_bwd_weight', gy, y, gs, gq, x, A, B, act, g64, N, Cin, Cout, T, H, W, stride, gsc)
             gw = fin()
-        return gx, gA, gB, gw, None, None, None, None, None, None, None
+        return gx, gA, gB, gw, None, None, None, None, None, None, None, None
 
     @staticmethod
     def _backward_bf16(ctx, gy, gs, gq, gsc):
@@ -319,10 +342,10 @@
             g64, fin = _gw_buffers(ctx.wparam, Cout, Cin, x.device)
             call('cfn_pwconv_bwd_weight' + _sfx(gy), gy, y, gs, gq, xin, A, B, act, g64, N, Cin, Cout, T * Ho * Wo, gsc)
             gw = fin()
-        return gx, gA, gB, gw, None, None, None, None, None, None, None
-
-
-def pwconv(x, w, A=None, B=None, act=ACT_NONE, stride=1, stats=True, token=None, role=None, tail=None, tail_role=None):
+        return gx, gA, gB, gw, None, None, None, None, None, None, None, None
+
+
+def pwconv(x, w, A=None, B=None, act=ACT_NONE, stride=1, stats=True, token=None, role=None, tail=None, tail_role=None, fold=None):
     N, Cin, T, H, W = x.shape
     Ho, Wo = (H - 1) // stride + 1, (W - 1) // stride + 1
     es = x.element_size()
@@ -330,7 +353,7 @@
     span = max(Cin * H * W, w.shape[0] * H * W, w.shape[0] * Ho * Wo, Cin * Ho * Wo) * es
     needs_grad = torch.is_grad_enabled() and any(t is not None and t.requires_grad for t in (x, w, A, B))
     if span * T < lim or needs_grad or T == 1:
-        return _PwConv.apply(x, A, B, w, act, stride, stats, token, role, tail, tail_role)
+        return _PwConv.apply(x, A, B, w, act, stride, stats, token, role, tail, tail_role, fold)
     step = max((lim - 1) // span, 1)
     odd_plane = es == 2 and (Ho * Wo) % 2 == 1
     if odd_plane:
@@ -744,7 +767,7 @@
 class _BnAddRelu(Function):
 
     @staticmethod
-    def forward(ctx, y, A, B, res, Ar, Br, split, link):
+    def forward(ctx, y, A, B, res, Ar, Br, split, link, fold_out=None, fold_in=None):
         y, res = check(y).contiguous(), check(res).contiguous()
         N, C = y.shape[:2]
         vol = y[0, 0].numel()
@@ -760,6 +783,10 @@
                 mask = torch.empty(words, dtype=torch.int32, device=y.device)
         call('cfn_bn_add_relu_fwd' + sfx, y, A, B, res, Ar, Br, out, mask, N * C, vol)
         ctx.link, ctx.has_mask = link, mask is not None
+        ctx.fold_out = fold_out if (link is not None and not _bf(y)) else None
+        ctx.fold_in = fold_in if link is not None else None
+        if ctx.fold_out is not None:
+            ctx.fold_out.y, ctx.fold_out.res = y.detach(), (res.detach() if Ar is not None else None)
         ctx.save_for_backward(y, A, res, Ar, mask if mask is not None else out)
         if not split:
             return out
@@ -778,11 +805,24 @@
         if gout is None:
             gout = torch.zeros_like(y)
         gout2 = None if gout2 is None else gout2.contiguous()
+        link = ctx.link
+        fo, fi = ctx.fold_out, ctx.fold_in
+        if fo is not None:
+            done, fo.y, fo.res, fo.g2, fo.out = fo.out, None, None, None, None
+            if done is not None:
+                g, used2, gA, gB, gAr = done
+                if gout.data_ptr() != g.data_ptr() or (gout2 is not None and gout2.data_ptr() != used2.data_ptr()):
+                    raise RuntimeError('bn_add_relu: the folded block tail received other gradients than the ones its conv1 worked on '
+                                       '(the block output has consumers besides the next block: set ops.TAIL_FOLD = False)')
+                link.y_scale, link.res_scale, link.done = A.detach(), (None if Ar is None else Ar.detach()), True
+                if fi is not None:
+                    fi.g2 = g
+                g2 = torch.empty(0, dtype=g.dtype, device=g.device).set_(g.untyped_storage(), g.storage_offset(), g.shape, g.stride())
+                return g, gA, gB, g2, gAr, (gB if Ar is not None else None), None, None, None, None
         t3 = _tls.arena.take(3 * N * C, y.device).view(3, N, C)
         gA, gB = t3[0], t3[1]
         gAr = t3[2] if Ar is not None else None
         gBr = gB if Ar is not None else None
-        link = ctx.link
         if link is not None:
             g = torch.empty_like(y)
             mask = out if ctx.has_mask else None
@@ -790,21 +830,23 @@
                  res if Ar is not None else None, g, gA, gB, gAr, N * C, vol)
             link.y_scale, link.res_scale, link.done = A.detach(), (None if Ar is None else Ar.detach()), True
             g2 = torch.empty(0, dtype=g.dtype, device=g.device).set_(g.untyped_storage(), g.storage_offset(), g.shape, g.stride())
-            return g, gA, gB, g2, gAr, gBr, None, None
+            if fi is not None and not _bf(y) and Ar is None:
+                fi.g2 = g
+            return g, gA, gB, g2, gAr, gBr, None, None, None, None
         if _bf(y):
             g = torch.empty_like(y)
             call('cfn_bn_add_relu_bwd_g' + _sfx(y), gout.contiguous(), gout2, out, None, y, res if Ar is not None else None, g, gA, gB,
                  gAr, N * C, vol)
             shp = (N, C) + (1,) * (y.dim() - 2)
             gres = g if Ar is None else (g.float() * Ar.float().view(shp)).to(y.dtype)
-            return (g.float() * A.float().view(shp)).to(y.dtype), gA, gB, gres, gAr, gBr, None, None
+            return (g.float() * A.float().view(shp)).to(y.dtype), gA, gB, gres, gAr, gBr, None, None, None, None
         gy, gres = torch.empty_like(y), torch.empty_like(res)
         call('cfn_bn_add_relu_bwd', gout.contiguous(), gout2, out, y, A, res, Ar, gy, gres, gA, gB, gAr, N * C, vol)
-        return gy, gA, gB, gres, gAr, gBr, None, None
-
-
-def bn_add_relu(y, A, B, res, Ar=None, Br=None, split=False, link=None):
-    return _BnAddRelu.apply(y, A, B, res, Ar, Br, split, link)
+        return gy, gA, gB, gres, gAr, gBr, None, None, None, None
+
+
+def bn_add_relu(y, A, B, res, Ar=None, Br=None, split=False, link=None, fold_out=None, fold_in=None):
+    return _BnAddRelu.apply(y, A, B, res, Ar, Br, split, link, fold_out, fold_in)
 
 
 class _AffineAct(Function):
diff --git a/coarse-fine-networks_amd/csrc/pw_common.h b/coarse-fine-networks_amd/csrc/pw_common.h
--- a/coarse-fine-networks_amd/csrc/pw_common.h
+++ b/coarse-fine-networks_amd/csrc/pw_common.h
@@ -67,6 +67,9 @@
 int pwfs_try_launch(const float* gy, const float* y, const double* gsum, const double* gsumsq, const float* w, const float* x, const double* A,
                     const double* B, int act, float* gx, double* gA, double* gB, double* gw, int N, int Cin, int Cout, int T, int Hi, int Wi,
                     const float* acc, int acc_stride, const double* gscale, hipStream_t st);
+int pwfs_tail_try_launch(const float* gy, const float* y, const double* gsum, const double* gsumsq, const float* w, const float* x, float* gx, double* gw,
+                         int N, int Cin, int Cout, int T, int Hi, int Wi, const double* gscale, const float* g2, const float* ytail, double* gAt, double* gBt,
+                         const float* res, double* gAr, hipStream_t st);
 int salb_fwd_try_launch(const float* x, const double* A, const double* B, int act, const float* w, float* y, double* sum,
                         double* sumsq, int N, int Cin, int Cout, int T, int Hi, int Wi, const int* g, hipStream_t st);
 int sal_wgrad_try_launch(const float* gy, const float* y, const double* gs, const double* gq, const float* x, const double* A,
diff --git a/coarse-fine-networks_amd/csrc/pwfused.hip b/coarse-fine-networks_amd/csrc/pwfused.hip
--- a/coarse-fine-networks_amd/csrc/pwfused.hip
+++ b/coarse-fine-networks_amd/csrc/pwfused.hip
@@ -15,12 +15,16 @@
     float* gx; double* gA; double* gB; double* gw;
     const float* acc; int acc_s, acc_Ho, acc_Wo, Hi, Wi, T;
     int N, M, K, Q, nstrips, stages;
+    const float* g2; const float* yt; const float* res; double* gAt; double* gBt; double* gAr;
 };
 
+#define PF_TAIL (-2)
+
 template <int MTW, int NTW, int ACT>
-__global__ __launch_bounds__(256, ACT < 0 ? 3 : 2) void pw_bwd_fused_kernel(const PfArgs a) {
+__global__ __launch_bounds__(256, ACT == -1 ? 3 : 2) void pw_bwd_fused_kernel(const PfArgs a) {
     extern __shared__ __attribute__((aligned(16))) float smem[];
     constexpr bool EPI = ACT >= 0;
+    constexpr bool TAIL = ACT == PF_TAIL;
     constexpr int ACTV = EPI ? ACT : CFN_ACT_NONE;
     constexpr int BM = 32 * MTW, BN = 32 * NTW;
     constexpr int NG = BM / 16, NX = BN / 16;
@@ -77,6 +81,11 @@
     for (int t = 0; t < NT16; ++t)
 #pragma unroll
         for (int r = 0; r < 4; ++r) { sa[t][r] = 0.0f; sb[t][r] = 0.0f; }
+    float sr[NT16][4];
+#pragma unroll
+    for (int t = 0; t < NT16; ++t)
+#pragma unroll
+        for (int r = 0; r < 4; ++r) sr[t][r] = 0.0f;
     __syncthreads();
 
     const int lrow = tid >> 4, c4 = (tid & 15) * 4;
@@ -126,13 +135,35 @@
 
     const int qbeg = strip * a.stages * PF_PT;
     const int nst = min(a.stages, (Q - qbeg + PF_PT - 1) / PF_PT);
+    const int pbase = wave * (PF_PT / 4);
+    __amdgpu_buffer_rsrc_t rg2 = cfn_rsrc(const_cast<float*>(TAIL && a.g2 ? a.g2 + (long)n * K * Q : a.gy), TAIL && a.g2 ? (unsigned)((long)K * Q * 4) : 0u);
+    __amdgpu_buffer_rsrc_t ryt = cfn_rsrc(const_cast<float*>(TAIL ? a.yt + (long)n * K * Q : a.gy), TAIL ? (unsigned)((long)K * Q * 4) : 0u);
+    __amdgpu_buffer_rsrc_t rrs = cfn_rsrc(const_cast<float*>(TAIL && a.res ? a.res + (long)n * K * Q : a.gy), TAIL && a.res ? (unsigned)((long)K * Q * 4) : 0u);
+    float tg[NT16][4], ty[NT16][4], tr[NT16][4];
+#pragma unroll
+    for (int t = 0; t < NT16; ++t)
+#pragma unroll
+        for (int r = 0; r < 4; ++r) { tg[t][r] = 0.0f; ty[t][r] = 0.0f; tr[t][r] = 0.0f; }
+    auto tail_load = [&](int q0) {
+        const int tvo = (q0 + pbase + m16 < Q) ? (4 * kq * Q + pbase + m16) * 4 : OOB;
+#pragma unroll
+        for (int t = 0; t < NT16; ++t)
+#pragma unroll
+            for (int r = 0; r < 4; ++r) {
+                const int so = (q0 + (t * 16 + r) * Q) * 4;
+                const int vo = (t * 16 + 4 * kq + r) < K ? tvo : OOB;
+                tg[t][r] = __builtin_bit_cast(float, __builtin_amdgcn_raw_buffer_load_b32(rg2, vo, so, 0));
+                ty[t][r] = __builtin_bit_cast(float, __builtin_amdgcn_raw_buffer_load_b32(ryt, vo, so, 0));
+                if (a.res) tr[t][r] = __builtin_bit_cast(float, __builtin_amdgcn_raw_buffer_load_b32(rrs, vo, so, 0));
+            }
+    };
     if (nst > 0) {
         prefetch(qbeg);
         stage(qbeg, img0, img0 + BM * PF_PITCH);
+        if (TAIL) tail_load(qbeg);
         if (nst > 1) prefetch(qbeg + PF_PT);
     }
     __syncthreads();
-    const int pbase = wave * (PF_PT / 4);
     const int hw = a.Hi * a.Wi;
     const int acc_pitch4 = a.T * a.acc_Ho * a.acc_Wo * 4;
     __amdgpu_buffer_rsrc_t racc = cfn_rsrc(const_cast<float*>(a.acc ? a.acc + (long)n * K * (acc_pitch4 / 4) : a.gy), a.acc ? (unsigned)((long)K * acc_pitch4) : 0u);
@@ -208,24 +239,37 @@
                     sb[t][r] += dz;
                     v = dz * pa;
                 }
+                if (TAIL) {
+                    const float xr = sX[ci * PF_PITCH + pbase + m16];
+                    v = (ok && xr > 0.0f) ? v + tg[t][r] : 0.0f;
+                    sa[t][r] = fmaf(v, ty[t][r], sa[t][r]);
+                    sb[t][r] += v;
+                    sr[t][r] = fmaf(v, tr[t][r], sr[t][r]);
+                }
                 __builtin_amdgcn_raw_buffer_store_b32(__builtin_bit_cast(unsigned, v), rd, ok ? (ci * Q + pbase + m16) * 4 : OOB, q0 * 4, 0);
             }
         }
+        if (TAIL && st + 1 < nst) tail_load(q0 + PF_PT);
         __syncthreads();
     }
 
-    if (EPI) {
+    float* sSr = sSt + 8 * BN;
+    if (EPI || TAIL) {
 #pragma unroll
         for (int t = 0; t < NT16; ++t)
 #pragma unroll
             for (int r = 0; r < 4; ++r) {
-                float u = sa[t][r], v = sb[t][r];
-#pragma unroll
-                for (int o = 1; o < 16; o <<= 1) { u += __shfl_xor(u, o, 64); v += __shfl_xor(v, o, 64); }
+                float u = sa[t][r], v = sb[t][r], z = sr[t][r];
+#pragma unroll
+                for (int o = 1; o < 16; o <<= 1) {
+                    u += __shfl_xor(u, o, 64); v += __shfl_xor(v, o, 64);
+                    if (TAIL) z += __shfl_xor(z, o, 64);
+                }
                 if (m16 == 0) {
                     const int ci = t * 16 + 4 * kq + r;
                     sSt[(wave * BN + ci) * 2] = u;
                     sSt[(wave * BN + ci) * 2 + 1] = v;
+                    if (TAIL) sSr[wave * BN + ci] = z;
                 }
             }
     }
@@ -252,6 +296,16 @@
         const float v = (sSt[2 * tid + 1] + sSt[(BN + tid) * 2 + 1]) + (sSt[(2 * BN + tid) * 2 + 1] + sSt[(3 * BN + tid) * 2 + 1]);
         cfn_add64(&a.gA[(long)n * K + tid], (double)u);
         cfn_add64(&a.gB[(long)n * K + tid], (double)v);
+    }
+    if (TAIL && tid < K) {
+        const float u = (sSt[2 * tid] + sSt[(BN + tid) * 2]) + (sSt[(2 * BN + tid) * 2] + sSt[(3 * BN + tid) * 2]);
+        const float v = (sSt[2 * tid + 1] + sSt[(BN + tid) * 2 + 1]) + (sSt[(2 * BN + tid) * 2 + 1] + sSt[(3 * BN + tid) * 2 + 1]);
+        cfn_add64(&a.gAt[(long)n * K + tid], (double)u);
+        cfn_add64(&a.gBt[(long)n * K + tid], (double)v);
+        if (a.res) {
+            const float z = (sSr[tid] + sSr[BN + tid]) + (sSr[2 * BN + tid] + sSr[3 * BN + tid]);
+            cfn_add64(&a.gAr[(long)n * K + tid], (double)z);
+        }
     }
 }
 
@@ -271,8 +325,16 @@
     else if (act == CFN_ACT_RELU) CFN_PF_GO(CFN_ACT_RELU);
     else if (act == CFN_ACT_SWISH) CFN_PF_GO(CFN_ACT_SWISH);
     else CFN_PF_GO(CFN_ACT_NONE);
+    return cfn_check_launch("pwconv_bwd_fused");
+}
+
+static int pf_launch_tail(const PfArgs& a, unsigned blocks, hipStream_t st) {
+    constexpr int MTW = 2, NTW = 1, BM = 32 * MTW, BN = 32 * NTW;
+    const size_t lds = ((size_t)2 * (BM + BN) * PF_PITCH + 3 * BM + 14 * BN) * sizeof(float);
+    static_assert((size_t)4 * BM * (BN + 1) <= (size_t)2 * (BM + BN) * PF_PITCH, "the weight-gradient tiles fit over the images");
+    CFN_PF_GO(PF_TAIL);
 #undef CFN_PF_GO
-    return cfn_check_launch("pwconv_bwd_fused");
+    return cfn_check_launch("pwconv_bwd_fused_tail");
 }
 
 extern "C" int cfn_pwconv_bwd_fused(const float* gy, const float* y, const double* gsum, const double* gsumsq, const float* w,
@@ -314,3 +376,37 @@
     if (Cin > 32) return pf_launch<1, 2>(a, act, epi, blocks, st);
     return pf_launch<1, 1>(a, act, epi, blocks, st);
 }
+
+extern "C" int cfn_pwconv_bwd_fused_tail(const float* gy, const float* y, const double* gsum, const double* gsumsq, const float* w,
+                                         const float* x, float* gx, double* gw, int N, int Cin, int Cout, int T, int Hi, int Wi,
+                                         const double* gscale, const float* g2, const float* ytail, double* gAt, double* gBt,
+                                         const float* res, double* gAr, void* stream) {
+    CFN_REQUIRE(gy && w && x && gx && gw && ytail && gAt && gBt, "cfn_pwconv_bwd_fused_tail: null tensor");
+    CFN_REQUIRE(gsumsq == nullptr || y != nullptr, "cfn_pwconv_bwd_fused_tail: gsumsq needs y");
+    CFN_REQUIRE((res == nullptr) == (gAr == nullptr), "cfn_pwconv_bwd_fused_tail: res / gAr mismatch");
+    {
+        const int rs = pwfs_tail_try_launch(gy, y, gsum, gsumsq, w, x, gx, gw, N, Cin, Cout, T, Hi, Wi, gscale, g2, ytail, gAt, gBt, res, gAr, (hipStream_t)stream);
+        if (rs != -1) return rs;
+    }
+    const long Ql = (long)T * Hi * Wi;
+    if (Cin > 32 || Cout <= 32 || Cout > 64 || Ql % 4 != 0 || Ql >= (1L << 30)) return -1;
+    if ((long)Cout * Ql * 4 >= 0x7ffffff0L || (long)Cin * Ql * 4 >= 0x7ffffff0L) return -1;
+    if ((((uintptr_t)gy | (uintptr_t)x | (uintptr_t)(y ? y : gy)) & 15) != 0) return -1;
+    PfArgs a = {};
+    a.gy = gy; a.y = gsumsq ? y : nullptr; a.gs = gsum; a.gq = gsumsq; a.gsc = gscale; a.w = w; a.x = x;
+    a.gx = gx; a.gw = gw;
+    a.acc_s = 1; a.Hi = Hi; a.Wi = Wi; a.T = T; a.acc_Ho = Hi; a.acc_Wo = Wi;
+    a.N = N; a.M = Cout; a.K = Cin; a.Q = (int)Ql;
+    a.g2 = g2; a.yt = ytail; a.res = res; a.gAt = gAt; a.gBt = gBt; a.gAr = gAr;
+    const long nst = cfn_cdiv(Ql, PF_PT);
+    long want = 1024 / N;
+    if (want < 1) want = 1;
+    long stages = cfn_cdiv(nst, want);
+    if (stages < 4) stages = 4;
+    a.stages = (int)stages;
+    a.nstrips = (int)cfn_cdiv(nst, stages);
+    const unsigned blocks = (unsigned)((long)N * a.nstrips);
+    hipStream_t st = (hipStream_t)stream;
+    CfnProfScope prof(CFN_K_PWCONV_BWD, st, 4.0 * N * ((double)Cout * Ql * (a.y ? 2 : 1) + (double)Cin * Ql * (3 + (g2 ? 1 : 0) + (res ? 1 : 0))));
+    return pf_launch_tail(a, blocks, st);
+}
diff --git a/coarse-fine-networks_amd/csrc/pwfuseds.hip b/coarse-fine-networks_amd/csrc/pwfuseds.hip
--- a/coarse-fine-networks_amd/csrc/pwfuseds.hip
+++ b/coarse-fine-networks_amd/csrc/pwfuseds.hip
@@ -37,12 +37,16 @@
     const float* acc; int acc_s, acc_Ho, acc_Wo, Hi, Wi, T;
     int N, M, K, Q, nstrips, stages;
     int dbg;
+    const float* g2; const float* yt; double* gAt; double* gBt;
 };
+
+#define PFS_TAIL (-2)
 
 template <int MTW, int NTW, int ACT>
 __global__ __launch_bounds__(512, 1) void pw_bwd_fused_split_kernel(const PfsArgs a) {
     extern __shared__ __attribute__((aligned(16))) float smem[];
     constexpr bool EPI = ACT >= 0;
+    constexpr bool TAIL = ACT == PFS_TAIL;
     constexpr int ACTV = EPI ? ACT : CFN_ACT_NONE;
     constexpr int BM = 32 * MTW, BN = 32 * NTW;
     constexpr int NG = BM / 16, NX = BN / 16;
@@ -226,6 +230,25 @@
         const int hw = a.Hi * a.Wi;
         const int acc_pitch4 = a.T * a.acc_Ho * a.acc_Wo * 4;
         __amdgpu_buffer_rsrc_t racc = cfn_rsrc(const_cast<float*>(a.acc ? a.acc + (long)n * K * (acc_pitch4 / 4) : a.gy), a.acc ? (unsigned)((long)K * acc_pitch4) : 0u);
+        __amdgpu_buffer_rsrc_t rg2 = cfn_rsrc(const_cast<float*>(TAIL && a.g2 ? a.g2 + (long)n * K * Q : a.gy), TAIL && a.g2 ? (unsigned)((long)K * Q * 4) : 0u);
+        __amdgpu_buffer_rsrc_t ryt = cfn_rsrc(const_cast<float*>(TAIL ? a.yt + (long)n * K * Q : a.gy), TAIL ? (unsigned)((long)K * Q * 4) : 0u);
+        float tg[NT16][4], ty[NT16][4];
+#pragma unroll
+        for (int t = 0; t < NT16; ++t)
+#pragma unroll
+            for (int r = 0; r < 4; ++r) { tg[t][r] = 0.0f; ty[t][r] = 0.0f; }
+        auto tail_load = [&](int q0) {
+            const int tvo = (q0 + pbase + m16 < Q) ? (4 * kq * Q + pbase + m16) * 4 : OOB;
+#pragma unroll
+            for (int t = 0; t < NT16; ++t)
+#pragma unroll
+                for (int r = 0; r < 4; ++r) {
+                    const int so = (q0 + (t * 16 + r) * Q) * 4;
+                    const int vo = (t * 16 + 4 * kq + r) < K ? tvo : OOB;
+                    tg[t][r] = __builtin_bit_cast(float, __builtin_amdgcn_raw_buffer_load_b32(rg2, vo, so, 0));
+                    ty[t][r] = __builtin_bit_cast(float, __builtin_amdgcn_raw_buffer_load_b32(ryt, vo, so, 0));
+                }
+        };
         for (int st = 0; st < nst; ++st) {
             const int q0 = qbeg + st * PFS_PT;
             float* cur = img0 + (st & 1) * IMG;
@@ -258,11 +281,15 @@
                     if (NT16 > 4 && (t & 1)) __builtin_amdgcn_sched_barrier(0);
                 }
             }
+            if (TAIL) {
+                __builtin_amdgcn_sched_barrier(0);
+                tail_load(q0);
+            }
             const int q = q0 + pbase + m16;
             const bool qv = q < Q;
             const int gvo = (qv && !(a.dbg & 8)) ? (4 * kq * Q + pbase + m16) * 4 : OOB;
             int aoff = OOB;
-            if (a.acc && qv) {
+            if (!TAIL && a.acc && qv) {
                 const int tq = q / hw, rq = q - tq * hw;
                 const int hq = rq / a.Wi, wq_ = rq - hq * a.Wi;
                 if (hq % a.acc_s == 0 && wq_ % a.acc_s == 0) aoff = (((tq * a.acc_Ho + hq / a.acc_s) * a.acc_Wo + wq_ / a.acc_s)) * 4;
@@ -275,7 +302,7 @@
                 for (int t = 0; t < NT16; ++t)
 #pragma unroll
                     for (int r = 0; r < 4; ++r) av4[AV_UPFRONT ? t : 0][r] = 0.0f;
-                if (a.acc) {
+                if (!TAIL && a.acc) {
 #pragma unroll
                     for (int t = 0; t < NT16; ++t)
 #pragma unroll
@@ -291,7 +318,7 @@
                     const int ci = t * 16 + 4 * kq + r;
                     float v = da[t][r];
                     if (AV_UPFRONT) v += av4[AV_UPFRONT ? t : 0][r];
-                    else if (a.acc)
+                    else if (!TAIL && a.acc)
                         v += __builtin_bit_cast(float, __builtin_amdgcn_raw_buffer_load_b32(
                             racc, (int)(aoff == OOB ? (unsigned)OOB : arow + (unsigned)r * (unsigned)acc_pitch4), t * 16 * acc_pitch4, 0));
                     if (EPI && !(a.dbg & 4)) {
@@ -303,13 +330,19 @@
                         sb[t][r] += dz;
                         v = dz * pa;
                     }
+                    if (TAIL) {
+                        const float xr = sX[ci * PFS_PITCH + pbase + m16];
+                        v = xr > 0.0f ? v + tg[t][r] : 0.0f;
+                        sa[t][r] = fmaf(v, ty[t][r], sa[t][r]);
+                        sb[t][r] += v;
+                    }
                     __builtin_amdgcn_raw_buffer_store_b32(__builtin_bit_cast(unsigned, v), rd, gvo, (q0 + (t * 16 + r) * Q) * 4, 0);
                 }
                 if (NT16 > 4) __builtin_amdgcn_sched_barrier(0);
             }
             __syncthreads();
         }
-        if (EPI) {
+        if (EPI || TAIL) {
 #pragma unroll
             for (int t = 0; t < NT16; ++t)
 #pragma unroll
@@ -331,6 +364,12 @@
             const float v = (sSt[2 * t2 + 1] + sSt[(BN + t2) * 2 + 1]) + (sSt[(2 * BN + t2) * 2 + 1] + sSt[(3 * BN + t2) * 2 + 1]);
             cfn_add64(&a.gA[(long)n * K + t2], (double)u);
             cfn_add64(&a.gB[(long)n * K + t2], (double)v);
+        }
+        if (TAIL && t2 < K) {
+            const float u = (sSt[2 * t2] + sSt[(BN + t2) * 2]) + (sSt[(2 * BN + t2) * 2] + sSt[(3 * BN + t2) * 2]);
+            const float v = (sSt[2 * t2 + 1] + sSt[(BN + t2) * 2 + 1]) + (sSt[(2 * BN + t2) * 2 + 1] + sSt[(3 * BN + t2) * 2 + 1]);
+            cfn_add64(&a.gAt[(long)n * K + t2], (double)u);
+            cfn_add64(&a.gBt[(long)n * K + t2], (double)v);
         }
         __syncthreads();
     }
@@ -361,8 +400,16 @@
     else if (act == CFN_ACT_RELU) CFN_PFS_GO(CFN_ACT_RELU);
     else if (act == CFN_ACT_SWISH) CFN_PFS_GO(CFN_ACT_SWISH);
     else CFN_PFS_GO(CFN_ACT_NONE);
+    return cfn_check_launch("pwconv_bwd_fused (split bf16)");
+}
+
+static int pfs_launch_tail(const PfsArgs& a, unsigned blocks, hipStream_t st) {
+    constexpr int MTW = 4, NTW = 2, BM = 32 * MTW, BN = 32 * NTW, BMP = BM + 8;
+    const size_t lds = ((size_t)2 * (BM + BN) * PFS_PITCH + 3 * BM + 10 * BN) * sizeof(float) + (size_t)3 * BN * BMP * 2;
+    static_assert((size_t)4 * (MTW * NTW / 2) * 32 * 33 <= (size_t)2 * (BM + BN) * PFS_PITCH, "the weight-gradient tiles fit over the images");
+    CFN_PFS_GO(PFS_TAIL);
 #undef CFN_PFS_GO
-    return cfn_check_launch("pwconv_bwd_fused (split bf16)");
+    return cfn_check_launch("pwconv_bwd_fused_tail (split bf16)");
 }
 
 #define PF3_PT 32
@@ -1008,6 +1055,34 @@
     else CFN_PF3E_GO(CFN_ACT_NONE);
 #undef CFN_PF3E_GO
     return cfn_check_launch("pwconv_bwd_fused (split bf16, layer 3 conv3)");
+}
+
+int pwfs_tail_try_launch(const float* gy, const float* y, const double* gsum, const double* gsumsq, const float* w, const float* x, float* gx, double* gw,
+                         int N, int Cin, int Cout, int T, int Hi, int Wi, const double* gscale, const float* g2, const float* ytail, double* gAt, double* gBt,
+                         const float* res, double* gAr, hipStream_t st) {
+    const char* env_on = getenv("CFN_PWF_SPLIT");
+    if ((env_on && atoi(env_on) == 0) || pws_terms_now() != 6 || res != nullptr) return -1;
+    if (!(Cout > 64 && Cout <= 128 && Cin > 32 && Cin <= 64)) return -1;
+    const long Ql = (long)T * Hi * Wi;
+    if (Ql % 4 != 0 || Ql >= (1L << 30)) return -1;
+    if ((long)Cout * Ql * 4 >= 0x7ffffff0L || (long)Cin * Ql * 4 >= 0x7ffffff0L) return -1;
+    if ((((uintptr_t)gy | (uintptr_t)x | (uintptr_t)(y ? y : gy)) & 15) != 0) return -1;
+    PfsArgs a = {};
+    a.gy = gy; a.y = gsumsq ? y : nullptr; a.gs = gsum; a.gq = gsumsq; a.gsc = gscale; a.w = w; a.x = x;
+    a.gx = gx; a.gw = gw;
+    a.acc_s = 1; a.Hi = Hi; a.Wi = Wi; a.T = T; a.acc_Ho = Hi; a.acc_Wo = Wi;
+    a.N = N; a.M = Cout; a.K = Cin; a.Q = (int)Ql;
+    a.g2 = g2; a.yt = ytail; a.gAt = gAt; a.gBt = gBt;
+    const long nst = cfn_cdiv(Ql, PFS_PT);
+    long want = 512 / N;
+    if (want < 1) want = 1;
+    long stages = cfn_cdiv(nst, want);
+    if (stages < 4) stages = 4;
+    a.stages = (int)stages;
+    a.nstrips = (int)cfn_cdiv(nst, stages);
+    const unsigned blocks = (unsigned)((long)N * a.nstrips);
+    CfnProfScope prof(CFN_K_PWCONV_BWD, st, 4.0 * N * ((double)Cout * Ql * (a.y ? 2 : 1) + (double)Cin * Ql * (3 + (g2 ? 1 : 0))));
+    return pfs_launch_tail(a, blocks, st);
 }
 
 int pwfs_try_launch(const float* gy, const float* y, const double* gsum, const double* gsumsq, const float* w, const float* x, const double* A,
diff --git a/coarse-fine-networks_amd/x3d_fine.py b/coarse-fine-networks_amd/x3d_fine.py
--- a/coarse-fine-networks_amd/x3d_fine.py
+++ b/coarse-fine-networks_amd/x3d_fine.py
@@ -176,7 +176,11 @@
     def forward(self, x):
         if USE_TORCH_OPS:
             return self._forward_torch_ops(x)
-        x, x_res = x if isinstance(x, tuple) else (x, x)
+        fold_in = None
+        if isinstance(x, tuple) and len(x) == 3:
+            x, x_res, fold_in = x
+        else:
+            x, x_res = x if isinstance(x, tuple) else (x, x)
         xr, xa, xb, xact = _unpack(x)
         n = xr.shape[0]
         tr = self.training
@@ -184,7 +188,7 @@
 
         ts = self.t_stride
         tok = ops.ShortcutToken() if (isinstance(self.downsample, nn.Sequential) and self.stride > 1 and ts == 1) else None
-        y1, s1, q1 = ops.pwconv(xr, self.conv1.weight, xa, xb, xact, 1, stats=tr, token=tok, role='main')
+        y1, s1, q1 = ops.pwconv(xr, self.conv1.weight, xa, xb, xact, 1, stats=tr, token=tok, role='main', fold=fold_in)
         A1, B1 = self.bn1.fold(s1, q1, _count(y1), n)
         if ts == 1:
             y2, s2, q2 = ops.dwconv3d(y1, self.conv2.weight, A1, B1, ACT_RELU, self.stride, stats=tr or has_se)
@@ -197,6 +201,8 @@
         link = ops.TailLink() if torch.is_grad_enabled() else None
         y3, s3, q3 = ops.pwconv(y2, self.conv3.weight, A2, B2, ACT_SWISH, 1, stats=tr, tail=link, tail_role='y')
         A3, B3 = self.bn3.fold(s3, q3, _count(y3), n)
+        fold_out = ops.TailFold() if (self.split_out and link is not None and ops.TAIL_FOLD) else None
+        pack = (lambda o: o + (fold_out,)) if fold_out is not None else (lambda o: o)
 
         if self.downsample is not None:
             if not isinstance(self.downsample, nn.Sequential):
@@ -209,9 +215,9 @@
             yd, sd, qd = ops.pwconv(_every(xr, ts), self.downsample[0].weight, xa, xb, xact, self.stride, stats=tr, token=tok, role='short',
                                     tail=link, tail_role='res')
             Ad, Bd = self.downsample[1].fold(sd, qd, _count(yd), n)
-            return ops.bn_add_relu(y3, A3, B3, yd, Ad, Bd, split=self.split_out, link=link)
+            return pack(ops.bn_add_relu(y3, A3, B3, yd, Ad, Bd, split=self.split_out, link=link, fold_out=fold_out))
         res = x_res.materialize() if isinstance(x_res, Deferred) else x_res
-        return ops.bn_add_relu(y3, A3, B3, res, split=self.split_out, link=link)
+        return pack(ops.bn_add_relu(y3, A3, B3, res, split=self.split_out, link=link, fold_out=fold_out, fold_in=fold_in))
 
 
 class ResNet(nn.Module):
diff --git a/include/cfn_hip.h b/include/cfn_hip.h
--- a/include/cfn_hip.h
+++ b/include/cfn_hip.h
@@ -56,6 +56,11 @@
                          const float* x, const double* A, const double* B, int act, float* gx, double* gA, double* gB,
                          double* gw, int N, int Cin, int Cout, int T, int Hi, int Wi, const float* acc, int acc_stride,
                          const double* gscale, void* stream);
+
+int cfn_pwconv_bwd_fused_tail(const float* gy, const float* y, const double* gsum, const double* gsumsq, const float* w,
+                              const float* x, float* gx, double* gw, int N, int Cin, int Cout, int T, int Hi, int Wi,
+                              const double* gscale, const float* g2, const float* ytail, double* gAt, double* gBt,
+                              const float* res, double* gAr, void* stream);
 
 int cfn_pwconv_short_bwd(const float* gy, const float* y, const double* gsum, const double* gsumsq, const double* gscale,
                          const float* w, const float* x, const double* A, const double* B, int act, float* da, double* gw,
```
